# ru-wang/slam-plus-plus

Measured on AMD Instinct MI355X. Metric: Λ-solve block-nnz/sec + batch GN iters/sec, Venice BA, 1→8 MI355X, higher is better.
Workload: dtype f64; 1 GPU; venice871-shaped synthetic BA (871 cams, 530304 points, 2838740 observations, LM-damped); nnzb=3369915, n=1596138, mode=schur+dense, n_reduced=5226, schur_pairs=12875640, parallelism=single GPU

## Files before the change

### include/spp_hip.h

```cpp
#ifndef SPP_HIP_H
#define SPP_HIP_H

#include <stddef.h>
#include <stdint.h>

#ifdef __cplusplus
extern "C" {
#endif

#define SPP_OK            0
#define SPP_NOT_POSDEF    1
#define SPP_E_BADARG     -1
#define SPP_E_NOMEM      -2
#define SPP_E_HIP        -3
#define SPP_E_NO_DEVICE  -4
#define SPP_E_STATE      -5
#define SPP_E_UNSUPPORTED -6

#define SPP_MODE_AUTO     0
#define SPP_MODE_SPARSE   1
#define SPP_MODE_SCHUR    2
#define SPP_MODE_SCHUR_SPARSE 3

#define SPP_FLAG_PROFILE  1
#define SPP_FLAG_SCHUR_PARTIAL 2

typedef struct spp_ctx spp_ctx;

spp_ctx *spp_create(int device, int flags);
void spp_destroy(spp_ctx *ctx);
int spp_free_memory(spp_ctx *ctx);
int spp_last_error(const spp_ctx *ctx, char *buf, size_t buf_size);
double *spp_host_staging(spp_ctx *ctx, int64_t n_doubles);
int spp_set_stream(spp_ctx *ctx, void *hip_stream);
int spp_synchronize(spp_ctx *ctx);

int spp_analyze(spp_ctx *ctx, int64_t nb, const int64_t *h_col_ptr, const int64_t *h_row_idx,
	const int64_t *h_blk_off, const int32_t *h_dim, int mode);

int spp_set_shard(spp_ctx *ctx, int rank, int world_size);

#define SPP_MODE_SCHUR_MIS 4

#define SPP_INFO_MODE           0
#define SPP_INFO_N              1
#define SPP_INFO_NNZB           2
#define SPP_INFO_NVALS          3
#define SPP_INFO_FACTOR_NNZ     4
#define SPP_INFO_FACTOR_FLOPS   5
#define SPP_INFO_N_REDUCED      6
#define SPP_INFO_N_POSES        7
#define SPP_INFO_N_LANDMARKS    8
#define SPP_INFO_SCHUR_PAIRS    9
#define SPP_INFO_N_OBS          10
#define SPP_INFO_SOLVE_BYTES    11
#define SPP_INFO_N_SUPERNODES   12
#define SPP_INFO_N_LEVELS       13
#define SPP_INFO_S_LD           14
#define SPP_INFO_S_NNZB         15
#define SPP_INFO_DENSE_STREAMED 16
int spp_get_info(const spp_ctx *ctx, int what, int64_t *out);
int spp_get_ordering(const spp_ctx *ctx, int64_t *h_order);

#define SPP_ORDER_AMD 0
#define SPP_ORDER_ND  1
int spp_block_ordering(int64_t nb, const int64_t *col_ptr, const int64_t *row_idx, int method, int64_t *h_order);

int spp_schur_plan_host(int64_t nb, const int32_t *dim, const int64_t *col_ptr, const int64_t *row_idx, int shard_rank,
	int shard_world, int sparse_S, int64_t *out, double *seconds);

int spp_factor_solve(spp_ctx *ctx, const double *h_vals, double *h_rhs_inout);

int spp_factor_solve_device(spp_ctx *ctx, const double *d_vals, double *d_rhs_inout);

int spp_schur_buffer_size(const spp_ctx *ctx, int64_t *n_doubles);
int spp_schur_form(spp_ctx *ctx, const double *d_vals, const double *d_rhs, double *d_S_rhs);
int spp_schur_finish(spp_ctx *ctx, const double *d_vals, double *d_S_rhs, double *d_rhs_inout);
int spp_schur_packed_size(const spp_ctx *ctx, int64_t *n_doubles);
int spp_schur_pack(spp_ctx *ctx, const double *d_S_rhs, double *d_packed);
int spp_schur_unpack(spp_ctx *ctx, const double *d_packed, double *d_S_rhs);

int spp_assemble_analyze(spp_ctx *ctx, int64_t nv, const int32_t *h_dim,
	int64_t ne, const int64_t *h_v0, const int64_t *h_v1, int d0, int d1, int rd,
	int64_t unary_vertex);
int spp_assemble_get_structure(const spp_ctx *ctx, int64_t *h_col_ptr, int64_t *h_row_idx,
	int64_t *h_blk_off);
int spp_assemble_device(spp_ctx *ctx, const double *d_J0, const double *d_J1,
	const double *d_Omega, const double *d_r, double damping, double *d_vals_out, double *d_eta_out);
int spp_assemble_set_edge_weights(spp_ctx *ctx, const double *d_w);
int spp_edge_robust_weights_device(spp_ctx *ctx, int64_t n_edges, int rd, int kind, double scale, double param,
	const double *d_r, double *d_w_out);

int spp_se2_linearize_device(spp_ctx *ctx, int64_t n_edges, const int32_t *d_v0, const int32_t *d_v1,
	const double *d_poses, const double *d_measurements, double *d_J0, double *d_J1, double *d_r);
int spp_se2_update_device(spp_ctx *ctx, int64_t n_vertices, double *d_poses, const double *d_dx, int apply,
	double *h_dx_norm2);

int spp_se3_linearize_device(spp_ctx *ctx, int64_t n_edges, const int32_t *d_v0, const int32_t *d_v1,
	const double *d_poses, const double *d_measurements, double *d_J0, double *d_J1, double *d_r);
int spp_se3_update_device(spp_ctx *ctx, int64_t n_vertices, double *d_poses, const double *d_dx, int apply,
	double *h_dx_norm2);

int spp_ba_linearize_device(spp_ctx *ctx, int64_t n_obs, const int32_t *d_cam_of, const int32_t *d_pt_of,
	const double *d_cams, const double *d_intrinsics, const double *d_points, const double *d_measurements,
	double *d_J0, double *d_J1, double *d_r);
int spp_ba_update_device(spp_ctx *ctx, int64_t n_cams, double *d_cams, const int64_t *d_cam_dxoff,
	int64_t n_points, double *d_points, const int64_t *d_pt_dxoff, const double *d_dx, int64_t n_dx, int apply,
	double *h_dx_norm2);

int spp_edge_chi2_device(spp_ctx *ctx, int64_t n_edges, int rd, const double *d_r, const double *d_Omega, double *h_chi2);
int spp_edge_hessian_maxdiag_device(spp_ctx *ctx, int64_t n_edges, int rd, int d0, int d1, const double *d_J0,
	const double *d_J1, const double *d_Omega, double *h_max);
int spp_lm_gain_denominator_device(spp_ctx *ctx, int64_t n, const double *d_dx, const double *d_eta, double alpha,
	double *h_out);

int spp_device_malloc(spp_ctx *ctx, size_t bytes, void **d_ptr);
int spp_device_free(spp_ctx *ctx, void *d_ptr);
int spp_memcpy_h2d(spp_ctx *ctx, void *d_dst, const void *h_src, size_t bytes);
int spp_memcpy_d2h(spp_ctx *ctx, void *h_dst, const void *d_src, size_t bytes);
int spp_memcpy_d2d(spp_ctx *ctx, void *d_dst, const void *d_src, size_t bytes);

int spp_set_profiling(spp_ctx *ctx, int on);

#define SPP_PHASE_PERMUTE   0
#define SPP_PHASE_SCHUR_INV 1
#define SPP_PHASE_SCHUR_GEMM 2
#define SPP_PHASE_SCHUR_RHS 3
#define SPP_PHASE_FACTOR    4
#define SPP_PHASE_TRISOLVE  5
#define SPP_PHASE_BACKSUBST 6
#define SPP_PHASE_ASSEMBLE  7
#define SPP_PHASE_TOTAL     8
#define SPP_N_PHASES        9
int spp_get_phase_ms(spp_ctx *ctx, double *ms_out );
int spp_get_dominant_kernel(spp_ctx *ctx, double *ms_total, int64_t *n_launches, double *flops);

int spp_microbench_copy(spp_ctx *ctx, size_t bytes, int iters, double *gb_per_s);
int spp_microbench_mfma_f64(spp_ctx *ctx, int iters, double *tflops);
int spp_microbench_ctile(spp_ctx *ctx, int n, int iters, double *gb_per_s);
int spp_microbench_update(spp_ctx *ctx, int64_t m, int iters, double *ms_per_launch);

int spp_dense_potrf_upper(spp_ctx *ctx, double *d_A, int64_t n, int64_t ld);
int spp_dense_posv(spp_ctx *ctx, double *d_A, int64_t n, int64_t ld, double *d_b);
int spp_dense_gemm_tn_sub(spp_ctx *ctx, int64_t m, int64_t n, int64_t k,
	const double *d_A, int64_t lda, const double *d_B, int64_t ldb, double *d_C, int64_t ldc);
int spp_dense_gemm_tn_sub_upper(spp_ctx *ctx, int64_t m, int64_t n, int64_t k,
	const double *d_A, int64_t lda, const double *d_B, int64_t ldb, double *d_C, int64_t ldc);
int spp_dense_front_factor(spp_ctx *ctx, double *d_F, int64_t ld, int64_t w, int64_t h, double *d_image);

const char *spp_version(void);

#ifdef __cplusplus
}
#endif
#endif
```

### slam_plus_plus_amd/api.py

```python
import ctypes
import os

import numpy as np

_HERE = os.path.dirname(os.path.abspath(__file__))
LIB_PATH = os.environ.get("SPP_LIB") or os.path.join(_HERE, "libspp_hip.so")

SPP_OK, SPP_NOT_POSDEF = 0, 1
MODE_AUTO, MODE_SPARSE, MODE_SCHUR, MODE_SCHUR_SPARSE, MODE_SCHUR_MIS = 0, 1, 2, 3, 4
FLAG_PROFILE = 1
INFO = dict(MODE=0, N=1, NNZB=2, NVALS=3, FACTOR_NNZ=4, FACTOR_FLOPS=5, N_REDUCED=6, N_POSES=7,
            N_LANDMARKS=8, SCHUR_PAIRS=9, N_OBS=10, SOLVE_BYTES=11, N_SUPERNODES=12, N_LEVELS=13, S_LD=14, S_NNZB=15, DENSE_STREAMED=16)
PHASES = ["permute", "schur_inv", "schur_gemm", "schur_rhs", "factor", "trisolve", "backsubst", "assemble", "total"]

EXPORTS = [
    "spp_create", "spp_destroy", "spp_free_memory", "spp_last_error", "spp_host_staging", "spp_set_stream", "spp_synchronize",
    "spp_analyze", "spp_set_shard", "spp_get_info", "spp_get_ordering", "spp_factor_solve",
    "spp_factor_solve_device", "spp_schur_buffer_size", "spp_schur_form", "spp_schur_finish",
    "spp_schur_packed_size", "spp_schur_pack", "spp_schur_unpack",
    "spp_assemble_analyze", "spp_assemble_get_structure", "spp_assemble_device", "spp_assemble_set_edge_weights", "spp_device_malloc",
    "spp_device_free", "spp_memcpy_h2d", "spp_memcpy_d2h", "spp_memcpy_d2d", "spp_get_phase_ms", "spp_get_dominant_kernel",
    "spp_microbench_copy", "spp_microbench_mfma_f64", "spp_microbench_ctile", "spp_microbench_update", "spp_block_ordering", "spp_schur_plan_host", "spp_set_profiling", "spp_se2_linearize_device", "spp_se2_update_device", "spp_ba_linearize_device", "spp_ba_update_device", "spp_se3_linearize_device", "spp_se3_update_device", "spp_edge_chi2_device", "spp_edge_robust_weights_device", "spp_edge_hessian_maxdiag_device",
    "spp_lm_gain_denominator_device", "spp_dense_potrf_upper", "spp_dense_posv",
    "spp_dense_gemm_tn_sub", "spp_dense_gemm_tn_sub_upper", "spp_dense_front_factor", "spp_version",
]

_lib = None
_c_i64p = ctypes.POINTER(ctypes.c_int64)
_c_i32p = ctypes.POINTER(ctypes.c_int32)
_c_f64p = ctypes.POINTER(ctypes.c_double)


class SppError(RuntimeError):
    """std::runtime_error of the C++ adapter (reference LinearSolver_Schur_GPU.cpp:734-797)."""


def load_library():
    global _lib
    if _lib is not None:
        return _lib
    if not os.path.exists(LIB_PATH):
        raise SppError("libspp_hip.so is not built: run `python -m slam_plus_plus_amd.build` "
                       "(hipcc --offload-arch=gfx950); there is no CPU fallback")
    lib = ctypes.CDLL(LIB_PATH)
    vp, i64, i32, dbl, cint = ctypes.c_void_p, ctypes.c_int64, ctypes.c_int32, ctypes.c_double, ctypes.c_int
    sig = {
        "spp_create": (vp, [cint, cint]),
        "spp_destroy": (None, [vp]),
        "spp_free_memory": (cint, [vp]),
        "spp_last_error": (cint, [vp, ctypes.c_char_p, ctypes.c_size_t]),
        "spp_host_staging": (vp, [vp, i64]),
        "spp_set_stream": (cint, [vp, vp]),
        "spp_synchronize": (cint, [vp]),
        "spp_analyze": (cint, [vp, i64, vp, vp, vp, vp, cint]),
        "spp_set_shard": (cint, [vp, cint, cint]),
        "spp_get_info": (cint, [vp, cint, _c_i64p]),
        "spp_get_ordering": (cint, [vp, vp]),
        "spp_factor_solve": (cint, [vp, vp, vp]),
        "spp_factor_solve_device": (cint, [vp, vp, vp]),
        "spp_schur_buffer_size": (cint, [vp, _c_i64p]),
        "spp_schur_form": (cint, [vp, vp, vp, vp]),
        "spp_schur_finish": (cint, [vp, vp, vp, vp]),
        "spp_schur_packed_size": (cint, [vp, _c_i64p]),
        "spp_schur_pack": (cint, [vp, vp, vp]),
        "spp_schur_unpack": (cint, [vp, vp, vp]),
        "spp_assemble_analyze": (cint, [vp, i64, vp, i64, vp, vp, cint, cint, cint, i64]),
        "spp_assemble_get_structure": (cint, [vp, vp, vp, vp]),
        "spp_assemble_device": (cint, [vp, vp, vp, vp, vp, dbl, vp, vp]),
        "spp_assemble_set_edge_weights": (cint, [vp, vp]),
        "spp_device_malloc": (cint, [vp, ctypes.c_size_t, ctypes.POINTER(vp)]),
        "spp_device_free": (cint, [vp, vp]),
        "spp_memcpy_h2d": (cint, [vp, vp, vp, ctypes.c_size_t]),
        "spp_memcpy_d2h": (cint, [vp, vp, vp, ctypes.c_size_t]),
        "spp_memcpy_d2d": (cint, [vp, vp, vp, ctypes.c_size_t]),
        "spp_get_phase_ms": (cint, [vp, _c_f64p]),
        "spp_get_dominant_kernel": (cint, [vp, _c_f64p, _c_i64p, _c_f64p]),
        "spp_microbench_copy": (cint, [vp, ctypes.c_size_t, cint, _c_f64p]),
        "spp_microbench_mfma_f64": (cint, [vp, cint, _c_f64p]),
        "spp_microbench_ctile": (cint, [vp, cint, cint, _c_f64p]),
        "spp_microbench_update": (cint, [vp, ctypes.c_int64, cint, _c_f64p]),
        "spp_block_ordering": (cint, [ctypes.c_int64, vp, vp, cint, vp]),
        "spp_schur_plan_host": (cint, [ctypes.c_int64, vp, vp, vp, cint, cint, cint, vp, vp]),
        "spp_set_profiling": (cint, [vp, cint]),
        "spp_se2_linearize_device": (cint, [vp, ctypes.c_int64, vp, vp, vp, vp, vp, vp, vp]),
        "spp_se2_update_device": (cint, [vp, ctypes.c_int64, vp, vp, cint, _c_f64p]),
        "spp_se3_linearize_device": (cint, [vp, ctypes.c_int64, vp, vp, vp, vp, vp, vp, vp]),
        "spp_se3_update_device": (cint, [vp, ctypes.c_int64, vp, vp, cint, _c_f64p]),
        "spp_edge_chi2_device": (cint, [vp, ctypes.c_int64, cint, vp, vp, _c_f64p]),
        "spp_edge_robust_weights_device": (cint, [vp, ctypes.c_int64, cint, cint, dbl, dbl, vp, vp]),
        "spp_edge_hessian_maxdiag_device": (cint, [vp, ctypes.c_int64, cint, cint, cint, vp, vp, vp, _c_f64p]),
        "spp_lm_gain_denominator_device": (cint, [vp, ctypes.c_int64, vp, vp, ctypes.c_double, _c_f64p]),
        "spp_ba_linearize_device": (cint, [vp, ctypes.c_int64, vp, vp, vp, vp, vp, vp, vp, vp, vp]),
        "spp_ba_update_device": (cint, [vp, ctypes.c_int64, vp, vp, ctypes.c_int64, vp, vp, vp, ctypes.c_int64, cint, _c_f64p]),
        "spp_dense_potrf_upper": (cint, [vp, vp, i64, i64]),
        "spp_dense_posv": (cint, [vp, vp, i64, i64, vp]),
        "spp_dense_gemm_tn_sub": (cint, [vp, i64, i64, i64, vp, i64, vp, i64, vp, i64]),
        "spp_dense_gemm_tn_sub_upper": (cint, [vp, i64, i64, i64, vp, i64, vp, i64, vp, i64]),
        "spp_dense_front_factor": (cint, [vp, vp, i64, i64, i64, vp]),
        "spp_version": (ctypes.c_char_p, []),
    }
    for name, (res, args) in sig.items():
        fn = getattr(lib, name)
        fn.restype = res
        fn.argtypes = args
    _lib = lib
    return lib


def _ptr(a):
    return a.ctypes.data_as(ctypes.c_void_p)


ORDER_AMD, ORDER_ND = 0, 1


def block_ordering(lam, method=ORDER_AMD):
    lib = load_library()
    col_ptr = np.ascontiguousarray(lam.col_ptr, dtype=np.int64)
    row_idx = np.ascontiguousarray(lam.row_idx, dtype=np.int64)
    out = np.empty(lam.nb, dtype=np.int64)
    code = lib.spp_block_ordering(lam.nb, _ptr(col_ptr), _ptr(row_idx), method, _ptr(out))
    if code != 0:
        raise SppError("spp_block_ordering failed: %d" % code)
    return out


def schur_plan_host(lam, shard_rank=0, shard_world=1, sparse_S=False, mis=False):
    lib = load_library()
    col_ptr = np.ascontiguousarray(lam.col_ptr, dtype=np.int64)
    row_idx = np.ascontiguousarray(lam.row_idx, dtype=np.int64)
    dim = np.ascontiguousarray(lam.dim, dtype=np.int32)
    out = np.zeros(8, dtype=np.int64)
    sec = ctypes.c_double(0.0)
    code = lib.spp_schur_plan_host(lam.nb, _ptr(dim), _ptr(col_ptr), _ptr(row_idx), shard_rank, shard_world,
                                   (1 if sparse_S else 0) | (2 if mis else 0), _ptr(out), ctypes.byref(sec))
    if code != 0:
        raise SppError("spp_schur_plan_host failed: %d" % code)
    keys = ("nc", "nl", "no", "n_pairs", "n_sblk", "n_items", "n_multi", "checksum")
    d = dict(zip(keys, (int(v) for v in out)))
    d["seconds"] = sec.value
    return d


class DeviceArray:

    def __init__(self, ctx, n, dtype=np.float64):
        self.ctx, self.n, self.dtype = ctx, int(n), np.dtype(dtype)
        p = ctypes.c_void_p()
        ctx._check(ctx.lib.spp_device_malloc(ctx.h, self.n * self.dtype.itemsize, ctypes.byref(p)))
        self.ptr = p.value

    @classmethod
    def from_host(cls, ctx, arr):
        arr = np.ascontiguousarray(arr)
        d = cls(ctx, arr.size, arr.dtype)
        d.upload(arr)
        return d

    def upload(self, arr):
        arr = np.ascontiguousarray(arr, dtype=self.dtype)
        assert arr.size == self.n
        self.ctx._check(self.ctx.lib.spp_memcpy_h2d(self.ctx.h, self.ptr, _ptr(arr), arr.nbytes))

    def download(self):
        out = np.empty(self.n, dtype=self.dtype)
        self.ctx._check(self.ctx.lib.spp_memcpy_d2h(self.ctx.h, _ptr(out), self.ptr, out.nbytes))
        return out

    def copy_from(self, other):
        assert other.n * other.dtype.itemsize <= self.n * self.dtype.itemsize
        self.ctx._check(self.ctx.lib.spp_memcpy_d2d(self.ctx.h, self.ptr, other.ptr, other.n * other.dtype.itemsize))

    def free(self):
        if self.ptr:
            self.ctx.lib.spp_device_free(self.ctx.h, self.ptr)
            self.ptr = None


class Context:

    def __init__(self, device=0, flags=0):
        self.lib = load_library()
        self.h = self.lib.spp_create(int(device), int(flags))
        if not self.h:
            raise SppError("spp_create failed: no usable HIP device %d (the solver has no CPU fallback)" % device)

    def close(self):
        if getattr(self, "h", None):
            self.lib.spp_destroy(self.h)
            self.h = None

    def __del__(self):
        try:
            self.close()
        except Exception:
            pass

    def last_error(self):
        buf = ctypes.create_string_buffer(1024)
        self.lib.spp_last_error(self.h, buf, 1024)
        return buf.value.decode(errors="replace")

    def _check(self, code):
        if code < 0:
            if code == -2:
                raise MemoryError(self.last_error())
            raise SppError("spp error %d: %s" % (code, self.last_error()))
        return code

    def analyze(self, bcsc, mode=MODE_AUTO):
        self._keep = bcsc
        return self._check(self.lib.spp_analyze(self.h, bcsc.nb, _ptr(bcsc.col_ptr), _ptr(bcsc.row_idx),
                                                 _ptr(bcsc.blk_off), _ptr(bcsc.dim), mode))

    def set_shard(self, rank, world):
        return self._check(self.lib.spp_set_shard(self.h, rank, world))

    def info(self, key):
        out = ctypes.c_int64()
        self._check(self.lib.spp_get_info(self.h, INFO[key], ctypes.byref(out)))
        return out.value

    def ordering(self, nb):
        out = np.empty(nb, dtype=np.int64)
        self._check(self.lib.spp_get_ordering(self.h, _ptr(out)))
        return out

    def se2_linearize_device(self, n_edges, d_v0, d_v1, d_poses, d_meas, d_J0, d_J1, d_r):
        return self._check(self.lib.spp_se2_linearize_device(self.h, n_edges, d_v0, d_v1, d_poses, d_meas, d_J0, d_J1, d_r))

    def se2_update_device(self, n_vertices, d_poses, d_dx, apply=True):
        out = ctypes.c_double()
        self._check(self.lib.spp_se2_update_device(self.h, n_vertices, d_poses, d_dx, 1 if apply else 0, ctypes.byref(out)))
        return out.value ** 0.5

    def se3_linearize_device(self, n_edges, d_v0, d_v1, d_poses, d_meas, d_J0, d_J1, d_r):
        return self._check(self.lib.spp_se3_linearize_device(self.h, n_edges, d_v0, d_v1, d_poses, d_meas, d_J0, d_J1, d_r))

    def se3_update_device(self, n_vertices, d_poses, d_dx, apply=True):
        out = ctypes.c_double()
        self._check(self.lib.spp_se3_update_device(self.h, n_vertices, d_poses, d_dx, 1 if apply else 0, ctypes.byref(out)))
        return out.value ** 0.5

    def edge_robust_weights_device(self, n_edges, rd, d_r, d_w, scale, param=1.345, kind=0):
        return self._check(self.lib.spp_edge_robust_weights_device(self.h, n_edges, rd, kind, float(scale), float(param), d_r, d_w))

    def edge_chi2_device(self, n_edges, rd, d_r, d_Om):
        out = ctypes.c_double()
        self._check(self.lib.spp_edge_chi2_device(self.h, n_edges, rd, d_r, d_Om, ctypes.byref(out)))
        return out.value

    def edge_hessian_maxdiag_device(self, n_edges, rd, d0, d1, d_J0, d_J1, d_Om):
        out = ctypes.c_double()
        self._check(self.lib.spp_edge_hessian_maxdiag_device(self.h, n_edges, rd, d0, d1, d_J0, d_J1, d_Om, ctypes.byref(out)))
        return out.value

    def lm_gain_denominator_device(self, n, d_dx, d_eta, alpha):
        out = ctypes.c_double()
        self._check(self.lib.spp_lm_gain_denominator_device(self.h, n, d_dx, d_eta, float(alpha), ctypes.byref(out)))
        return out.value

    def ba_linearize_device(self, n_obs, d_cam_of, d_pt_of, d_cams, d_intr, d_points, d_meas, d_J0, d_J1, d_r):
        return self._check(self.lib.spp_ba_linearize_device(self.h, n_obs, d_cam_of, d_pt_of, d_cams, d_intr, d_points,
                                                            d_meas, d_J0, d_J1, d_r))

    def ba_update_device(self, n_cams, d_cams, d_cam_dxoff, n_points, d_points, d_pt_dxoff, d_dx, n_dx, apply=True):
        out = ctypes.c_double()
        self._check(self.lib.spp_ba_update_device(self.h, n_cams, d_cams, d_cam_dxoff, n_points, d_points, d_pt_dxoff,
                                                  d_dx, n_dx, 1 if apply else 0, ctypes.byref(out)))
        return out.value ** 0.5

    def set_profiling(self, on):
        return self._check(self.lib.spp_set_profiling(self.h, 1 if on else 0))

    def set_stream(self, stream_handle):
        return self._check(self.lib.spp_set_stream(self.h, ctypes.c_void_p(stream_handle)))

    def synchronize(self):
        return self._check(self.lib.spp_synchronize(self.h))

    def host_staging(self, n):
        p = self.lib.spp_host_staging(self.h, int(n))
        if not p:
            raise MemoryError(self.last_error())
        return np.ctypeslib.as_array(ctypes.cast(p, ctypes.POINTER(ctypes.c_double)), shape=(int(n),))

    def factor_solve(self, vals, rhs):
        vals = np.ascontiguousarray(vals, dtype=np.float64)
        x = np.array(rhs, dtype=np.float64, copy=True)
        code = self._check(self.lib.spp_factor_solve(self.h, _ptr(vals), _ptr(x)))
        return code, x

    def factor_solve_device(self, d_vals, d_rhs):
        return self._check(self.lib.spp_factor_solve_device(self.h, d_vals, d_rhs))

    def schur_buffer_size(self):
# ... 127 lines not shown
```

### slam_plus_plus_amd/csrc/spp_api.cpp

```cpp

#include "spp_internal.h"
#include <string.h>
#include <new>

using namespace spp;

namespace spp {

void phases_reset(spp_ctx *ctx)
{
	if(!(ctx->flags & SPP_FLAG_PROFILE))
		return;
	if(!ctx->timer.created) {
		for(int i = 0; i < 2 * SPP_N_PHASES; ++ i)
			SPP_HIP_CHECK(hipEventCreate(&ctx->timer.ev[i]));
		ctx->timer.created = true;
	}
	for(int i = 0; i < SPP_N_PHASES; ++ i) {
		ctx->timer.used[i] = false;
		ctx->phase_ms[i] = 0;
	}
	ctx->dom_used = 0;
	ctx->dom_flops = 0;
}

void phase_begin(spp_ctx *ctx, int phase)
{
	if(!(ctx->flags & SPP_FLAG_PROFILE) || !ctx->timer.created)
		return;
	SPP_HIP_CHECK(hipEventRecord(ctx->timer.ev[2 * phase], ctx->stream));
}

void phase_end(spp_ctx *ctx, int phase)
{
	if(!(ctx->flags & SPP_FLAG_PROFILE) || !ctx->timer.created)
		return;
	SPP_HIP_CHECK(hipEventRecord(ctx->timer.ev[2 * phase + 1], ctx->stream));
	ctx->timer.used[phase] = true;
}

void phases_collect(spp_ctx *ctx)
{
	if(!(ctx->flags & SPP_FLAG_PROFILE) || !ctx->timer.created)
		return;
	SPP_HIP_CHECK(hipStreamSynchronize(ctx->stream));
	for(int i = 0; i < SPP_N_PHASES; ++ i) {
		if(!ctx->timer.used[i])
			continue;
		float ms = 0;
		if(hipEventElapsedTime(&ms, ctx->timer.ev[2 * i], ctx->timer.ev[2 * i + 1]) == hipSuccess)
			ctx->phase_ms[i] = ms;
	}
}

void dom_begin(spp_ctx *ctx)
{
	if(!(ctx->flags & SPP_FLAG_PROFILE))
		return;
	if(ctx->dom_used + 2 > ctx->dom_events.size()) {
		size_t old = ctx->dom_events.size();
		ctx->dom_events.resize(old + 64);
		for(size_t i = old; i < ctx->dom_events.size(); ++ i)
			SPP_HIP_CHECK(hipEventCreate(&ctx->dom_events[i]));
	}
	SPP_HIP_CHECK(hipEventRecord(ctx->dom_events[ctx->dom_used], ctx->stream));
}

void dom_end(spp_ctx *ctx, double flops)
{
	if(!(ctx->flags & SPP_FLAG_PROFILE))
		return;
	SPP_HIP_CHECK(hipEventRecord(ctx->dom_events[ctx->dom_used + 1], ctx->stream));
	ctx->dom_used += 2;
	ctx->dom_flops += flops;
}

}

#define SPP_TRY(ctx) try {
#define SPP_CATCH(ctx) } catch(const spp::Error &e) { if(ctx) (ctx)->last_error = e.what(); return e.code; } \
	catch(const std::bad_alloc &) { if(ctx) (ctx)->last_error = "host allocation failed"; return SPP_E_NOMEM; } \
	catch(const std::exception &e) { if(ctx) (ctx)->last_error = e.what(); return SPP_E_HIP; }

extern "C" {

const char *spp_version(void)
{
	return "slam_plus_plus_amd 0.1 (gfx950, fp64)";
}

spp_ctx *spp_create(int device, int flags)
{
	int count = 0;
	if(hipGetDeviceCount(&count) != hipSuccess || count <= 0 || device < 0 || device >= count)
		return nullptr;
	if(hipSetDevice(device) != hipSuccess)
		return nullptr;
	spp_ctx *ctx = new(std::nothrow) spp_ctx;
	if(!ctx)
		return nullptr;
	ctx->device = device;
	ctx->flags = flags;
	if(hipStreamCreateWithFlags(&ctx->stream, hipStreamNonBlocking) != hipSuccess) {
		delete ctx;
		return nullptr;
	}
	ctx->own_stream = true;
	return ctx;
}

int spp_free_memory(spp_ctx *ctx)
{
	if(!ctx)
		return SPP_E_BADARG;
	SPP_TRY(ctx)
	(void)hipSetDevice(ctx->device);
	(void)hipStreamSynchronize(ctx->stream);
	ctx->schur.release_all();
	sparse_release(ctx);
	assemble_release(ctx);
	ctx->dense.tinv.release();
	ctx->dense.tinv_all.release();
	ctx->dense.xtmp.release();
	ctx->dense.la_cnt.release();
	ctx->dense.la_trace.release();
	ctx->geom_partial.release();
	ctx->dense.flags.release();
	ctx->dense.trsv_pay.release();
	ctx->dense.trsv_m.release();
	ctx->dense.tail_pub.release();
	ctx->dense.tail_order.release();
	ctx->dense.tail_order_tr = ctx->dense.tail_order_tc = 0;
	ctx->dense.tail_dinv.release();
	ctx->dense.tail_epoch = 0;
	ctx->dense.epoch = 0;
	ctx->dense.sync.release();
	ctx->dense.fuse_cnt.release();
	ctx->dense.fuse_expect.clear();
	ctx->dense.sync_epoch = 0;
	ctx->d_vals.release();
	ctx->d_rhs.release();
	ctx->mode = -1;
	return SPP_OK;
	SPP_CATCH(ctx)
}

void spp_destroy(spp_ctx *ctx)
{
	if(!ctx)
		return;
	if(ctx->plan_trash.joinable())
		ctx->plan_trash.join();
	spp_free_memory(ctx);
	ctx->dense.info.release();
	if(ctx->dense.aux) {
		dense_aux_park(ctx->device, ctx->dense.aux);
		(void)hipEventDestroy(ctx->dense.ev[0]);
		(void)hipEventDestroy(ctx->dense.ev[1]);
	}
	if(ctx->dense.chain) {
		(void)hipStreamDestroy(ctx->dense.chain);
		if(ctx->dense.ev_chain)
			(void)hipEventDestroy(ctx->dense.ev_chain);
	}
	if(ctx->dense.h_chain_err)
		(void)hipHostFree(ctx->dense.h_chain_err);
	if(ctx->h_staging)
		(void)hipHostFree(ctx->h_staging);
	if(ctx->timer.created)
		for(int i = 0; i < 2 * SPP_N_PHASES; ++ i)
			(void)hipEventDestroy(ctx->timer.ev[i]);
	for(size_t i = 0; i < ctx->dom_events.size(); ++ i)
		(void)hipEventDestroy(ctx->dom_events[i]);
	if(ctx->own_stream && ctx->stream)
		(void)hipStreamDestroy(ctx->stream);
	delete ctx;
}

int spp_last_error(const spp_ctx *ctx, char *buf, size_t buf_size)
{
	if(!ctx || !buf || !buf_size)
		return SPP_E_BADARG;
	strncpy(buf, ctx->last_error.c_str(), buf_size - 1);
	buf[buf_size - 1] = 0;
	return SPP_OK;
}

double *spp_host_staging(spp_ctx *ctx, int64_t n_doubles)
{
	if(!ctx || n_doubles < 0)
		return nullptr;
	if((size_t)n_doubles <= ctx->h_staging_cap && ctx->h_staging)
		return ctx->h_staging;
	(void)hipSetDevice(ctx->device);
	(void)hipStreamSynchronize(ctx->stream);
	if(ctx->h_staging) {
		(void)hipHostFree(ctx->h_staging);
		ctx->h_staging = nullptr;
		ctx->h_staging_cap = 0;
	}
	const size_t want = (size_t)(n_doubles > 0 ? n_doubles : 1);
	if(hipHostMalloc((void**)&ctx->h_staging, want * sizeof(double), hipHostMallocDefault) != hipSuccess) {
		(void)hipGetLastError();
		ctx->h_staging = nullptr;
		ctx->last_error = "hipHostMalloc of the staging buffer failed";
		return nullptr;
	}
	ctx->h_staging_cap = want;
	return ctx->h_staging;
}

int spp_set_stream(spp_ctx *ctx, void *hip_stream)
{
	if(!ctx)
		return SPP_E_BADARG;
	(void)hipStreamSynchronize(ctx->stream);
	if(ctx->own_stream && ctx->stream)
		(void)hipStreamDestroy(ctx->stream);
	ctx->stream = (hipStream_t)hip_stream;
	ctx->own_stream = false;
	return SPP_OK;
}

int spp_synchronize(spp_ctx *ctx)
{
	if(!ctx)
		return SPP_E_BADARG;
	SPP_TRY(ctx)
	SPP_HIP_CHECK(hipStreamSynchronize(ctx->stream));
	dense_chain_check(ctx);
	return SPP_OK;
	SPP_CATCH(ctx)
}

int spp_set_profiling(spp_ctx *ctx, int on)
{
	if(!ctx)
		return SPP_E_BADARG;
	ctx->flags = on ? (ctx->flags | SPP_FLAG_PROFILE) : (ctx->flags & ~SPP_FLAG_PROFILE);
	return SPP_OK;
}

int spp_set_shard(spp_ctx *ctx, int rank, int world_size)
{
	if(!ctx || world_size < 1 || rank < 0 || rank >= world_size)
		return SPP_E_BADARG;
	ctx->shard_rank = rank;
	ctx->shard_world = world_size;
	return SPP_OK;
}

int spp_analyze(spp_ctx *ctx, int64_t nb, const int64_t *col_ptr, const int64_t *row_idx,
	const int64_t *blk_off, const int32_t *dim, int mode)
{
	if(!ctx)
		return SPP_E_BADARG;
	SPP_TRY(ctx)
	SPP_REQUIRE(nb > 0 && col_ptr && row_idx && blk_off && dim, SPP_E_BADARG, "spp_analyze: null or empty structure");
	SPP_REQUIRE(col_ptr[0] == 0 && col_ptr[nb] >= nb, SPP_E_BADARG, "spp_analyze: column pointers must start at 0 and hold every diagonal block");
	SPP_HIP_CHECK(hipSetDevice(ctx->device));
	ctx->mode = -1;
	VClock clk("spp_analyze");
	Structure st;
	st.nb = nb;
	st.nnzb = col_ptr[nb];
	st.col_ptr.assign(col_ptr, col_ptr + nb + 1);
	SPP_REQUIRE(st.nnzb >= nb, SPP_E_BADARG, "spp_analyze: fewer blocks than block columns");
	for(int64_t j = 0; j < nb; ++ j)
		SPP_REQUIRE(col_ptr[j + 1] > col_ptr[j], SPP_E_BADARG, "every block column needs its diagonal block");
	st.dim.assign(dim, dim + nb);
	st.base.resize(nb + 1);
	st.base[0] = 0;
	for(int64_t j = 0; j < nb; ++ j) {
		SPP_REQUIRE(dim[j] > 0 && dim[j] <= 8, SPP_E_BADARG, "block widths must be in 1..8");
		st.base[j + 1] = st.base[j] + dim[j];
	}
	st.n = st.base[nb];
	st.row_idx.resize(st.nnzb);
	st.blk_off.resize(st.nnzb);
	{
		const int nt = plan_threads(st.nnzb);
		std::vector<int64_t> jcut, nvals_t(nt, 0);
		balanced_cuts(st.col_ptr, nt, jcut);
		run_threads(nt, [&](int t) {
			const int64_t p0 = col_ptr[jcut[t]], p1 = col_ptr[jcut[t + 1]];
			if(p1 > p0) {
				memcpy(st.row_idx.data() + p0, row_idx + p0, (size_t)(p1 - p0) * sizeof(int64_t));
				memcpy(st.blk_off.data() + p0, blk_off + p0, (size_t)(p1 - p0) * sizeof(int64_t));
			}
			int64_t nv = 0;
			for(int64_t j = jcut[t]; j < jcut[t + 1]; ++ j) {
				for(int64_t p = col_ptr[j]; p < col_ptr[j + 1]; ++ p) {
					const int64_t i = row_idx[p];
					SPP_REQUIRE(i >= 0 && i <= j, SPP_E_BADARG, "only the upper triangle may be stored");
					SPP_REQUIRE(p == col_ptr[j] || row_idx[p - 1] < i, SPP_E_BADARG, "rows must ascend within a column");
					SPP_REQUIRE(blk_off[p] >= 0, SPP_E_BADARG, "negative block offset");
					nv = std::max<int64_t>(nv, blk_off[p] + (int64_t)dim[i] * dim[j]);
				}
				SPP_REQUIRE(row_idx[col_ptr[j + 1] - 1] == j, SPP_E_BADARG, "diagonal block missing (must be last in its column)");
			}
			nvals_t[t] = nv;
		});
		st.nvals = 0;
		for(int t = 0; t < nt; ++ t)
			st.nvals = std::max(st.nvals, nvals_t[t]);
	}
	ctx->st = std::move(st);
	Structure &st_ref = ctx->st;
	clk.lap("structure copied + validated");
	ctx->schur.release_all();
	sparse_release(ctx);
	clk.lap("old plans released");
	int dp, dl;
	int chosen = mode;
	if(mode == SPP_MODE_AUTO) {
		chosen = SPP_MODE_SPARSE;
		if(schur_applicable(st_ref, &dp, &dl)) {
			int64_t n_red = 0;
			for(int64_t j = 0; j < nb; ++ j)
				n_red += (dim[j] == dp) ? dp : 0;
			chosen = (n_red <= 16384) ? SPP_MODE_SCHUR : SPP_MODE_SCHUR_SPARSE;
		}
	}
	SPP_REQUIRE(chosen == SPP_MODE_SCHUR || chosen == SPP_MODE_SPARSE || chosen == SPP_MODE_SCHUR_SPARSE ||
		chosen == SPP_MODE_SCHUR_MIS, SPP_E_BADARG, "unknown mode");
	SPP_REQUIRE((chosen != SPP_MODE_SPARSE && chosen != SPP_MODE_SCHUR_MIS) || ctx->shard_world == 1, SPP_E_UNSUPPORTED,
		"only the Schur modes shard (over landmarks); pose graphs run as replicas (DESIGN.md, multi-GPU)");
	ctx->mode = -1;
	if(chosen == SPP_MODE_SCHUR || chosen == SPP_MODE_SCHUR_SPARSE || chosen == SPP_MODE_SCHUR_MIS) {
		const bool mis = chosen == SPP_MODE_SCHUR_MIS;
		const bool sparse_S = chosen != SPP_MODE_SCHUR;
		build_schur_plan(ctx, sparse_S, mis);
		clk.lap("schur plan (all of it)");
		ctx->schur.mis = mis;
		ctx->order.clear();
		ctx->order.reserve((size_t)st_ref.nb);
		if(sparse_S) {
			sparse_analyze(ctx, ctx->schur.s_st);
			std::vector<int64_t> red = ctx->order;
			ctx->order.clear();
			for(size_t i = 0; i < red.size(); ++ i)
				ctx->order.push_back(ctx->schur.pose_block[red[i]]);
			chosen = SPP_MODE_SCHUR;
		} else
		for(size_t i = 0; i < ctx->schur.pose_block.size(); ++ i)
			ctx->order.push_back(ctx->schur.pose_block[i]);
		for(int64_t j = 0; j < st_ref.nb; ++ j)
			if(ctx->schur.is_lm[j])
				ctx->order.push_back(j);
	} else
		sparse_analyze(ctx, ctx->st);
	ctx->mode = chosen;
	clk.lap("plan + ordering");
	return SPP_OK;
	SPP_CATCH(ctx)
}

int spp_get_info(const spp_ctx *ctx, int what, int64_t *out)
{
	if(!ctx || !out)
		return SPP_E_BADARG;
	if(ctx->mode < 0 && what != SPP_INFO_NNZB && what != SPP_INFO_NVALS && what != SPP_INFO_N && what != SPP_INFO_DENSE_STREAMED)
		return SPP_E_STATE;
	switch(what) {
	case SPP_INFO_MODE: *out = (ctx->mode != SPP_MODE_SCHUR) ? ctx->mode : ctx->schur.mis ? SPP_MODE_SCHUR_MIS :
		ctx->schur.sparse_S ? SPP_MODE_SCHUR_SPARSE : SPP_MODE_SCHUR; break;
	case SPP_INFO_N: *out = ctx->st.n; break;
	case SPP_INFO_NNZB: *out = ctx->st.nnzb; break;
	case SPP_INFO_NVALS: *out = ctx->st.nvals; break;
	case SPP_INFO_FACTOR_NNZ: *out = ctx->factor_nnz; break;
	case SPP_INFO_FACTOR_FLOPS: *out = ctx->factor_flops; break;
	case SPP_INFO_N_REDUCED: *out = (ctx->mode == SPP_MODE_SCHUR) ? ctx->schur.n_red : 0; break;
	case SPP_INFO_N_POSES: *out = (ctx->mode == SPP_MODE_SCHUR) ? ctx->schur.nc : ctx->st.nb; break;
	case SPP_INFO_N_LANDMARKS: *out = (ctx->mode == SPP_MODE_SCHUR) ? ctx->schur.nl : 0; break;
	case SPP_INFO_SCHUR_PAIRS: *out = (ctx->mode == SPP_MODE_SCHUR) ? ctx->schur.n_pairs : 0; break;
	case SPP_INFO_N_OBS: *out = (ctx->mode == SPP_MODE_SCHUR) ? ctx->schur.no : 0; break;
	case SPP_INFO_SOLVE_BYTES: *out = ctx->solve_bytes; break;
	case SPP_INFO_N_SUPERNODES: *out = ctx->sparse ? sparse_info(ctx, what) : 0; break;
	case SPP_INFO_N_LEVELS: *out = ctx->sparse ? sparse_info(ctx, what) : 0; break;
	case SPP_INFO_S_LD: *out = (ctx->mode == SPP_MODE_SCHUR && !ctx->schur.sparse_S) ? ctx->schur.ld : 0; break;
	case SPP_INFO_S_NNZB: *out = (ctx->mode == SPP_MODE_SCHUR) ? ctx->schur.n_sblk : 0; break;
	case SPP_INFO_DENSE_STREAMED: *out = ctx->dense.tail_rows_last; break;
	default: return SPP_E_BADARG;
	}
	return SPP_OK;
}

int spp_get_ordering(const spp_ctx *ctx, int64_t *h_order)
{
	if(!ctx || !h_order)
		return SPP_E_BADARG;
	if(ctx->mode < 0)
		return SPP_E_STATE;
	for(size_t i = 0; i < ctx->order.size(); ++ i)
		h_order[i] = ctx->order[i];
	return SPP_OK;
}

int spp_block_ordering(int64_t nb, const int64_t *col_ptr, const int64_t *row_idx, int method, int64_t *h_order)
{
	if(nb <= 0 || !col_ptr || !row_idx || !h_order || (method != SPP_ORDER_AMD && method != SPP_ORDER_ND))
		return SPP_E_BADARG;
	try {
		for(int64_t j = 0; j < nb; ++ j)
			for(int64_t p = col_ptr[j]; p < col_ptr[j + 1]; ++ p)
				if(row_idx[p] < 0 || row_idx[p] > j)
					return SPP_E_BADARG;
		std::vector<int64_t> order;
		if(method == SPP_ORDER_AMD)
			min_degree_order(nb, col_ptr, row_idx, order);
		else
			nested_dissection_order(nb, col_ptr, row_idx, order);
		for(int64_t k = 0; k < nb; ++ k)
			h_order[k] = order[k];
		return SPP_OK;
	} catch(const std::bad_alloc &) {
		return SPP_E_NOMEM;
	} catch(...) {
		return SPP_E_HIP;
	}
}

int spp_schur_plan_host(int64_t nb, const int32_t *dim, const int64_t *col_ptr, const int64_t *row_idx, int shard_rank,
	int shard_world, int sparse_S, int64_t *out, double *seconds)
{
	if(nb <= 0 || !dim || !col_ptr || !row_idx || !out || shard_world < 1 || shard_rank < 0 || shard_rank >= shard_world)
		return SPP_E_BADARG;
	try {
		Structure st;
		st.nb = nb;
		st.nnzb = col_ptr[nb];
		st.col_ptr.assign(col_ptr, col_ptr + nb + 1);
		st.row_idx.assign(row_idx, row_idx + st.nnzb);
		st.dim.assign(dim, dim + nb);
		st.base.resize(nb + 1);
		st.base[0] = 0;
		for(int64_t j = 0; j < nb; ++ j)
			st.base[j + 1] = st.base[j] + dim[j];
		st.n = st.base[nb];
		st.blk_off.resize(st.nnzb);
		int64_t off = 0;
		for(int64_t j = 0; j < nb; ++ j)
			for(int64_t p = col_ptr[j]; p < col_ptr[j + 1]; ++ p) {
				if(row_idx[p] < 0 || row_idx[p] > j)
					return SPP_E_BADARG;
				st.blk_off[p] = off;
				off += (int64_t)dim[row_idx[p]] * dim[j];
			}
		st.nvals = off;
		const double sec = schur_plan_host_probe(st, shard_rank, shard_world, (sparse_S & 1) != 0, (sparse_S & 2) != 0, out);
		if(seconds)
			*seconds = sec;
		return SPP_OK;
	} catch(const Error &e) {
		return e.code;
	} catch(const std::bad_alloc &) {
		return SPP_E_NOMEM;
	} catch(...) {
		return SPP_E_HIP;
	}
}

int spp_schur_buffer_size(const spp_ctx *ctx, int64_t *n_doubles)
{
	if(!ctx || !n_doubles)
		return SPP_E_BADARG;
	if(ctx->mode != SPP_MODE_SCHUR)
		return SPP_E_STATE;
	*n_doubles = schur_buffer_doubles(ctx);
	return SPP_OK;
}

int spp_schur_form(spp_ctx *ctx, const double *d_vals, const double *d_rhs, double *d_S_rhs)
{
	if(!ctx || !d_vals || !d_rhs || !d_S_rhs)
		return SPP_E_BADARG;
	SPP_TRY(ctx)
	SPP_REQUIRE(ctx->mode == SPP_MODE_SCHUR, SPP_E_STATE, "spp_schur_form: analyze in Schur mode first");
	SPP_HIP_CHECK(hipSetDevice(ctx->device));
	phases_reset(ctx);
	phase_begin(ctx, SPP_PHASE_TOTAL);
	schur_form(ctx, d_vals, d_rhs, d_S_rhs);
	return SPP_OK;
	SPP_CATCH(ctx)
}

int spp_schur_packed_size(const spp_ctx *ctx, int64_t *n_doubles)
{
	if(!ctx || !n_doubles)
		return SPP_E_BADARG;
	if(ctx->mode != SPP_MODE_SCHUR)
		return SPP_E_STATE;
	if(ctx->schur.sparse_S) {
		*n_doubles = schur_buffer_doubles(ctx);
		return SPP_OK;
	}
	const int64_t nblk = ctx->schur.ld / DENSE_NB;
	*n_doubles = (int64_t)DENSE_NB * DENSE_NB * (nblk * (nblk + 1) / 2);
	return SPP_OK;
}

int spp_schur_pack(spp_ctx *ctx, const double *d_S_rhs, double *d_packed)
{
	if(!ctx || !d_S_rhs || !d_packed)
		return SPP_E_BADARG;
	SPP_TRY(ctx)
	SPP_REQUIRE(ctx->mode == SPP_MODE_SCHUR, SPP_E_STATE, "spp_schur_pack: analyze in Schur mode first");
	SPP_HIP_CHECK(hipSetDevice(ctx->device));
	if(ctx->schur.sparse_S)
		SPP_HIP_CHECK(hipMemcpyAsync(d_packed, d_S_rhs, (size_t)schur_buffer_doubles(ctx) * sizeof(double),
			hipMemcpyDeviceToDevice, ctx->stream));
	else
		schur_pack(ctx, const_cast<double*>(d_S_rhs), d_packed, true);
	return SPP_OK;
	SPP_CATCH(ctx)
}

int spp_schur_unpack(spp_ctx *ctx, const double *d_packed, double *d_S_rhs)
{
	if(!ctx || !d_S_rhs || !d_packed)
		return SPP_E_BADARG;
	SPP_TRY(ctx)
	SPP_REQUIRE(ctx->mode == SPP_MODE_SCHUR, SPP_E_STATE, "spp_schur_unpack: analyze in Schur mode first");
	SPP_HIP_CHECK(hipSetDevice(ctx->device));
	if(ctx->schur.sparse_S)
		SPP_HIP_CHECK(hipMemcpyAsync(d_S_rhs, d_packed, (size_t)schur_buffer_doubles(ctx) * sizeof(double),
			hipMemcpyDeviceToDevice, ctx->stream));
	else
		schur_pack(ctx, d_S_rhs, const_cast<double*>(d_packed), false);
	return SPP_OK;
	SPP_CATCH(ctx)
}

int spp_schur_finish(spp_ctx *ctx, const double *d_vals, double *d_S_rhs, double *d_rhs_inout)
{
	if(!ctx || !d_vals || !d_rhs_inout || !d_S_rhs)
		return SPP_E_BADARG;
	SPP_TRY(ctx)
	SPP_REQUIRE(ctx->mode == SPP_MODE_SCHUR, SPP_E_STATE, "spp_schur_finish: analyze in Schur mode first");
	SPP_HIP_CHECK(hipSetDevice(ctx->device));
	int ret = schur_finish(ctx, d_vals, d_S_rhs, d_rhs_inout);
	phase_end(ctx, SPP_PHASE_TOTAL);
	phases_collect(ctx);
	dense_chain_check(ctx);
	return ret;
	SPP_CATCH(ctx)
}

int spp_factor_solve_device(spp_ctx *ctx, const double *d_vals, double *d_rhs)
{
	if(!ctx || !d_vals || !d_rhs)
		return SPP_E_BADARG;
	SPP_TRY(ctx)
	SPP_REQUIRE(ctx->mode >= 0, SPP_E_STATE, "spp_factor_solve: call spp_analyze first");
	SPP_HIP_CHECK(hipSetDevice(ctx->device));
	phases_reset(ctx);
	phase_begin(ctx, SPP_PHASE_TOTAL);
	int ret;
	if(ctx->mode == SPP_MODE_SCHUR) {
		SPP_REQUIRE(ctx->shard_world == 1, SPP_E_STATE,
			"sharded ctx: use spp_schur_form / all-reduce / spp_schur_finish");
		ctx->schur.S.reserve((size_t)schur_buffer_doubles(ctx));
		schur_form(ctx, d_vals, d_rhs, ctx->schur.S.p);
		ret = schur_finish(ctx, d_vals, ctx->schur.S.p, d_rhs);
	} else
		ret = sparse_factor_solve(ctx, d_vals, d_rhs);
	phase_end(ctx, SPP_PHASE_TOTAL);
	phases_collect(ctx);
	SPP_HIP_CHECK(hipStreamSynchronize(ctx->stream));
	dense_chain_check(ctx);
	return ret;
	SPP_CATCH(ctx)
}

int spp_factor_solve(spp_ctx *ctx, const double *h_vals, double *h_rhs)
{
	if(!ctx || !h_vals || !h_rhs)
		return SPP_E_BADARG;
	SPP_TRY(ctx)
	SPP_REQUIRE(ctx->mode >= 0, SPP_E_STATE, "spp_factor_solve: call spp_analyze first");
	SPP_HIP_CHECK(hipSetDevice(ctx->device));
	ctx->d_vals.reserve((size_t)ctx->st.nvals);
	ctx->d_rhs.reserve((size_t)ctx->st.n);
	SPP_HIP_CHECK(hipMemcpyAsync(ctx->d_vals.p, h_vals, ctx->st.nvals * sizeof(double), hipMemcpyHostToDevice, ctx->stream));
	SPP_HIP_CHECK(hipMemcpyAsync(ctx->d_rhs.p, h_rhs, ctx->st.n * sizeof(double), hipMemcpyHostToDevice, ctx->stream));
	int ret = spp_factor_solve_device(ctx, ctx->d_vals.p, ctx->d_rhs.p);
	if(ret != SPP_OK)
		return ret;
	SPP_HIP_CHECK(hipMemcpyAsync(h_rhs, ctx->d_rhs.p, ctx->st.n * sizeof(double), hipMemcpyDeviceToHost, ctx->stream));
	SPP_HIP_CHECK(hipStreamSynchronize(ctx->stream));
	return SPP_OK;
	SPP_CATCH(ctx)
}

int spp_assemble_analyze(spp_ctx *ctx, int64_t nv, const int32_t *h_dim, int64_t ne, const int64_t *h_v0,
	const int64_t *h_v1, int d0, int d1, int rd, int64_t unary_vertex)
{
	if(!ctx || !h_dim || !h_v0 || !h_v1 || nv <= 0 || ne <= 0)
		return SPP_E_BADARG;
	SPP_TRY(ctx)
	SPP_HIP_CHECK(hipSetDevice(ctx->device));
	assemble_analyze(ctx, nv, h_dim, ne, h_v0, h_v1, d0, d1, rd, unary_vertex);
	return SPP_OK;
	SPP_CATCH(ctx)
}

// ... 163 lines not shown
}

int spp_device_malloc(spp_ctx *ctx, size_t bytes, void **d_ptr)
{
	if(!ctx || !d_ptr)
		return SPP_E_BADARG;
	(void)hipSetDevice(ctx->device);
	if(hipMalloc(d_ptr, bytes ? bytes : 8) != hipSuccess) {
		ctx->last_error = "hipMalloc failed";
		return SPP_E_NOMEM;
	}
	return SPP_OK;
}

int spp_device_free(spp_ctx *ctx, void *d_ptr)
{
	if(!ctx)
		return SPP_E_BADARG;
	(void)hipSetDevice(ctx->device);
	(void)hipStreamSynchronize(ctx->stream);
	return hipFree(d_ptr) == hipSuccess ? SPP_OK : SPP_E_HIP;
}

int spp_memcpy_h2d(spp_ctx *ctx, void *d_dst, const void *h_src, size_t bytes)
{
	if(!ctx)
		return SPP_E_BADARG;
	SPP_TRY(ctx)
	SPP_HIP_CHECK(hipSetDevice(ctx->device));
	SPP_HIP_CHECK(hipMemcpyAsync(d_dst, h_src, bytes, hipMemcpyHostToDevice, ctx->stream));
	SPP_HIP_CHECK(hipStreamSynchronize(ctx->stream));
	return SPP_OK;
	SPP_CATCH(ctx)
}

int spp_memcpy_d2h(spp_ctx *ctx, void *h_dst, const void *d_src, size_t bytes)
{
	if(!ctx)
		return SPP_E_BADARG;
	SPP_TRY(ctx)
	SPP_HIP_CHECK(hipSetDevice(ctx->device));
	SPP_HIP_CHECK(hipMemcpyAsync(h_dst, d_src, bytes, hipMemcpyDeviceToHost, ctx->stream));
	SPP_HIP_CHECK(hipStreamSynchronize(ctx->stream));
	return SPP_OK;
	SPP_CATCH(ctx)
}

int spp_memcpy_d2d(spp_ctx *ctx, void *d_dst, const void *d_src, size_t bytes)
{
	if(!ctx)
		return SPP_E_BADARG;
	SPP_TRY(ctx)
	SPP_HIP_CHECK(hipSetDevice(ctx->device));
	SPP_HIP_CHECK(hipMemcpyAsync(d_dst, d_src, bytes, hipMemcpyDeviceToDevice, ctx->stream));
	return SPP_OK;
	SPP_CATCH(ctx)
}

int spp_get_phase_ms(spp_ctx *ctx, double *ms_out)
{
	if(!ctx || !ms_out)
		return SPP_E_BADARG;
	for(int i = 0; i < SPP_N_PHASES; ++ i)
		ms_out[i] = ctx->phase_ms[i];
	return SPP_OK;
}

int spp_get_dominant_kernel(spp_ctx *ctx, double *ms_total, int64_t *n_launches, double *flops)
{
	if(!ctx || !ms_total || !n_launches || !flops)
		return SPP_E_BADARG;
	SPP_TRY(ctx)
	SPP_HIP_CHECK(hipStreamSynchronize(ctx->stream));
	double total = 0;
	for(size_t i = 0; i + 1 < ctx->dom_used; i += 2) {
		float ms = 0;
		SPP_HIP_CHECK(hipEventElapsedTime(&ms, ctx->dom_events[i], ctx->dom_events[i + 1]));
		total += ms;
	}
	*ms_total = total;
	*n_launches = (int64_t)(ctx->dom_used / 2);
	*flops = ctx->dom_flops;
	return SPP_OK;
	SPP_CATCH(ctx)
}

int spp_microbench_copy(spp_ctx *ctx, size_t bytes, int iters, double *gb_per_s)
{
	if(!ctx || !gb_per_s)
		return SPP_E_BADARG;
	SPP_TRY(ctx)
	SPP_HIP_CHECK(hipSetDevice(ctx->device));
	*gb_per_s = microbench_copy(ctx, bytes, iters);
	return SPP_OK;
	SPP_CATCH(ctx)
}

int spp_microbench_ctile(spp_ctx *ctx, int n, int iters, double *gb_per_s)
{
	if(!ctx || !gb_per_s)
		return SPP_E_BADARG;
	SPP_TRY(ctx)
	SPP_HIP_CHECK(hipSetDevice(ctx->device));
	*gb_per_s = microbench_ctile(ctx, n, iters);
	return SPP_OK;
	SPP_CATCH(ctx)
}

int spp_microbench_update(spp_ctx *ctx, int64_t m, int iters, double *ms_per_launch)
{
	if(!ctx || !ms_per_launch || m < 128 || iters < 1)
		return SPP_E_BADARG;
	SPP_TRY(ctx)
	SPP_HIP_CHECK(hipSetDevice(ctx->device));
	*ms_per_launch = microbench_update(ctx, m, iters);
	return SPP_OK;
	SPP_CATCH(ctx)
}

int spp_microbench_mfma_f64(spp_ctx *ctx, int iters, double *tflops)
{
	if(!ctx || !tflops)
		return SPP_E_BADARG;
	SPP_TRY(ctx)
	SPP_HIP_CHECK(hipSetDevice(ctx->device));
	*tflops = microbench_mfma_f64(ctx, iters);
	return SPP_OK;
	SPP_CATCH(ctx)
}

int spp_dense_potrf_upper(spp_ctx *ctx, double *d_A, int64_t n, int64_t ld)
{
	if(!ctx || !d_A || n <= 0 || ld < n)
		return SPP_E_BADARG;
	SPP_TRY(ctx)
	SPP_HIP_CHECK(hipSetDevice(ctx->device));
	const int64_t ldp = ((n + 1 + DENSE_NB - 1) / DENSE_NB) * DENSE_NB;
	DevBuf<double> tmp;
	tmp.reserve((size_t)ldp * ldp);
	SPP_HIP_CHECK(hipMemsetAsync(tmp.p, 0, (size_t)ldp * ldp * sizeof(double), ctx->stream));
	SPP_HIP_CHECK(hipMemcpy2DAsync(tmp.p, ldp * sizeof(double), d_A, ld * sizeof(double), n * sizeof(double), n,
		hipMemcpyDeviceToDevice, ctx->stream));
	dense_set_padding(ctx, tmp.p, ldp, n);
	int ret = dense_potrf_upper(ctx, tmp.p, n, ldp, true);
	SPP_HIP_CHECK(hipMemcpy2DAsync(d_A, ld * sizeof(double), tmp.p, ldp * sizeof(double), n * sizeof(double), n,
		hipMemcpyDeviceToDevice, ctx->stream));
	SPP_HIP_CHECK(hipStreamSynchronize(ctx->stream));
	return ret;
	SPP_CATCH(ctx)
}

int spp_dense_posv(spp_ctx *ctx, double *d_A, int64_t n, int64_t ld, double *d_b)
{
	if(!ctx || !d_A || !d_b || n <= 0 || ld < n)
		return SPP_E_BADARG;
	SPP_TRY(ctx)
	SPP_HIP_CHECK(hipSetDevice(ctx->device));
	const int64_t ldp = ((n + 1 + DENSE_NB - 1) / DENSE_NB) * DENSE_NB;
	DevBuf<double> tmp;
	tmp.reserve((size_t)ldp * ldp);
	SPP_HIP_CHECK(hipMemsetAsync(tmp.p, 0, (size_t)ldp * ldp * sizeof(double), ctx->stream));
	SPP_HIP_CHECK(hipMemcpy2DAsync(tmp.p, ldp * sizeof(double), d_A, ld * sizeof(double), n * sizeof(double), n,
		hipMemcpyDeviceToDevice, ctx->stream));
	dense_set_padding(ctx, tmp.p, ldp, n);
	SPP_HIP_CHECK(hipMemcpyAsync(tmp.p + n * ldp, d_b, n * sizeof(double), hipMemcpyDeviceToDevice, ctx->stream));
	int ret = dense_potrf_upper(ctx, tmp.p, n, ldp, true);
	if(ret == SPP_OK) {
		dense_potrs_upper(ctx, tmp.p, n, ldp, tmp.p + n * ldp);
		SPP_HIP_CHECK(hipMemcpyAsync(d_b, tmp.p + n * ldp, n * sizeof(double), hipMemcpyDeviceToDevice, ctx->stream));
		SPP_HIP_CHECK(hipMemcpy2DAsync(d_A, ld * sizeof(double), tmp.p, ldp * sizeof(double), n * sizeof(double), n,
			hipMemcpyDeviceToDevice, ctx->stream));
	}
	SPP_HIP_CHECK(hipStreamSynchronize(ctx->stream));
	dense_chain_check(ctx);
	return ret;
	SPP_CATCH(ctx)
}

int spp_dense_gemm_tn_sub(spp_ctx *ctx, int64_t m, int64_t n, int64_t k, const double *d_A, int64_t lda,
	const double *d_B, int64_t ldb, double *d_C, int64_t ldc)
{
	if(!ctx || !d_A || !d_B || !d_C)
		return SPP_E_BADARG;
	SPP_TRY(ctx)
	SPP_REQUIRE((lda % 2) == 0 && (ldb % 2) == 0, SPP_E_BADARG, "gemm_tn_sub: lda/ldb must be even (16-byte loads)");
	SPP_HIP_CHECK(hipSetDevice(ctx->device));
	dense_gemm_tn_sub(ctx, m, n, k, d_A, lda, d_B, ldb, d_C, ldc, false);
	SPP_HIP_CHECK(hipStreamSynchronize(ctx->stream));
	return SPP_OK;
	SPP_CATCH(ctx)
}

int spp_dense_gemm_tn_sub_upper(spp_ctx *ctx, int64_t m, int64_t n, int64_t k, const double *d_A, int64_t lda,
	const double *d_B, int64_t ldb, double *d_C, int64_t ldc)
{
	if(!ctx || !d_A || !d_B || !d_C)
		return SPP_E_BADARG;
	SPP_TRY(ctx)
	SPP_REQUIRE((lda % 2) == 0 && (ldb % 2) == 0, SPP_E_BADARG, "gemm_tn_sub: lda/ldb must be even (16-byte loads)");
	SPP_HIP_CHECK(hipSetDevice(ctx->device));
	dense_gemm_tn_sub(ctx, m, n, k, d_A, lda, d_B, ldb, d_C, ldc, true);
	SPP_HIP_CHECK(hipStreamSynchronize(ctx->stream));
	return SPP_OK;
	SPP_CATCH(ctx)
}

int spp_dense_front_factor(spp_ctx *ctx, double *d_F, int64_t ld, int64_t w, int64_t h, double *d_image)
{
	if(!ctx || !d_F)
		return SPP_E_BADARG;
	SPP_TRY(ctx)
	SPP_HIP_CHECK(hipSetDevice(ctx->device));
	return dense_front_factor(ctx, d_F, ld, w, h, d_image);
	SPP_CATCH(ctx)
}

}
```

### slam_plus_plus_amd/csrc/spp_dense.hip

```cpp

#include "spp_internal.h"
#include "spp_tiles.h"
#include "spp_dense_dev.h"
#include <stdio.h>
#include <stdlib.h>
#include <string.h>
#include <algorithm>
#include <vector>
#include <mutex>

namespace spp {


constexpr int BK = 16;
constexpr int LDS_STRIDE = 18;

template <int BM, int BN, int WM, int WN, int MODE, int DEPTH, int BKT, int SC1 = 0>
__device__ __forceinline__ void gemm_tn_tile(const int64_t m0, const int64_t n0, int64_t M, int64_t N, int K,
	const double *__restrict__ A, int64_t lda, const double *B, int64_t ldb, double *C, int64_t ldc, double *gemm_lds)
{
	constexpr int NWM = BM / WM, NWN = BN / WN, NT = NWM * NWN * 64;
	constexpr int TA = WM / 16, TB = WN / 16;
	constexpr int PPC = BKT / 2, LSTR = BKT + 2;
	constexpr int PA = (BM * PPC) / NT, PB = (BN * PPC) / NT;
// ... 1148 lines not shown
		dw.la_trace.reserve(nw);
		std::vector<long long> init(nw, 0);
		for(int64_t k = 0; k < nsteps; ++ k)
			init[8 * nsteps + 8 + 4 * k] = (long long)((~0ull) >> 1);
		SPP_HIP_CHECK(hipMemcpyAsync(dw.la_trace.p, init.data(), nw * sizeof(long long), hipMemcpyHostToDevice, s));
		SPP_HIP_CHECK(hipStreamSynchronize(s));
		a.trace = dw.la_trace.p;
	}
	SPP_HIP_CHECK(hipMemsetAsync(a.cnt, 0, nints * sizeof(int), s));
	SPP_HIP_CHECK(hipEventRecord(dw.ev[0], s));
	SPP_HIP_CHECK(hipStreamWaitEvent(sc, dw.ev[0], 0));
	SPP_HIP_CHECK(hipStreamWaitEvent(sb, dw.ev[0], 0));
	hipLaunchKernelGGL(la_chain_kernel, dim3((unsigned)(1 + LA_G1 + a.g2)), dim3(LA_THREADS), LA_LDS_DOUBLES * sizeof(double), sc, a);
	const int64_t slots = slots_env > 0 ? slots_env : 512;
	for(int k = 0; k < a.nsteps; ++ k) {
		const int64_t c1 = (int64_t)NB * (k + 1);
		if(c1 >= ncols || rows - c1 <= 0)
			break;
		const int nr = (int)((rows - c1 + NB - 1) / NB), nc = (int)((ncols - c1 + NB - 1) / NB);
		const int npri = (nc > 2) ? (nc - 2) + std::min(2, nr - 1) : 0;
		const int64_t ntr = nr - 1, ntc = nc - 1;
		const int64_t T = ntr > 0 ? ntr * (ntr + 1) / 2 + (ntc - ntr) * ntr : 0;
		const int64_t n128 = (T / slots) * slots;
		const int64_t grid = 4 * (int64_t)npri + n128 + 4 * (T - n128);
		if(grid > 0)
			hipLaunchKernelGGL(la_bulk_kernel, dim3((unsigned)grid), dim3(1024), LA_BULK_LDS_DOUBLES * sizeof(double), sb,
				a, k, nr, nc, npri, n128);
	}
	SPP_HIP_CHECK(hipEventRecord(dw.ev[1], sb));
	SPP_HIP_CHECK(hipEventRecord(dw.ev_chain, sc));
	SPP_HIP_CHECK(hipStreamWaitEvent(s, dw.ev[1], 0));
	SPP_HIP_CHECK(hipStreamWaitEvent(s, dw.ev_chain, 0));
	SPP_HIP_CHECK(hipGetLastError());
	if(tracing) {
		std::vector<long long> h((size_t)12 * nsteps + 16);
		SPP_HIP_CHECK(hipMemcpyAsync(h.data(), dw.la_trace.p, h.size() * sizeof(long long), hipMemcpyDeviceToHost, s));
		SPP_HIP_CHECK(hipStreamSynchronize(s));
		fprintf(stderr, "[spp] lookahead factorization, %d steps: potrf start / duration / gap to the next start (us)\n", a.nsteps);
		for(int k = 0; k < a.nsteps; ++ k)
			fprintf(stderr, "  k %2d  start %8.1f  potrf %5.1f  publish %4.1f | b1 seen +%4.1f  done +%4.1f | c1 seen +%4.1f  done +%4.1f | step %5.1f\n", k,
				(h[8 * k] - h[0]) * 0.01, (h[8 * k + 2] - h[8 * k]) * 0.01, (h[8 * k + 1] - h[8 * k + 2]) * 0.01,
				(h[8 * k + 3] - h[8 * k + 1]) * 0.01, (h[8 * k + 4] - h[8 * k + 1]) * 0.01, (h[8 * k + 5] - h[8 * k + 1]) * 0.01,
				(h[8 * k + 6] - h[8 * k + 1]) * 0.01, k + 1 < a.nsteps ? (h[8 * (k + 1)] - h[8 * k]) * 0.01 : 0.0);
		fprintf(stderr, "[spp] per step: panel (rest) done / bulk launch: first tile starts, priority tiles done, last tile done, busy workgroup-us (all relative to potrf(0) start)\n");
		for(int k = 0; k < a.nsteps; ++ k) {
			const long long *b = h.data() + 8 * nsteps + 8 + 4 * k;
			fprintf(stderr, "  k %2d  panel done %8.1f | bulk start %8.1f  pri done %8.1f  end %8.1f  busy %9.1f\n", k, h[8 * k + 7] ? (h[8 * k + 7] - h[0]) * 0.01 : 0.0,
				b[1] ? (b[0] - h[0]) * 0.01 : 0.0, b[3] ? (b[3] - h[0]) * 0.01 : 0.0, b[1] ? (b[1] - h[0]) * 0.01 : 0.0, b[2] * 0.01);
		}
	}
}

void dense_factor_steps(spp_ctx *ctx, double *d_A, int64_t ld, int64_t n, int64_t rows, int64_t ncols,
	int64_t nsteps, bool has_rhs)
{
	ensure_dense_work(ctx, nsteps);
	ctx->dense.tail_rows_last = 0;
	hipStreamCaptureStatus cs = hipStreamCaptureStatusNone;
	const bool capturing = hipStreamIsCapturing(ctx->stream, &cs) != hipSuccess || cs != hipStreamCaptureStatusNone;
	if(!capturing && la_usable(ctx, nsteps)) {
		dense_factor_lookahead(ctx, d_A, ld, n, rows, ncols, nsteps, has_rhs);
		ctx->dense.tinv_half = 0;
		return;
	}
	ctx->dense.tinv_half = nsteps;
	const bool flags = !capturing && nsteps >= 4 && flag_schedule_usable(ctx);
	dense_factor_steps_enqueue(ctx, d_A, ld, n, rows, ncols, nsteps, has_rhs, flags, !capturing);
}

static void flag_signal(hipStream_t st, int *flag, int value)
{
	hipLaunchKernelGGL(flag_signal_kernel, dim3(1), dim3(64), 0, st, flag, value);
}

static FlagWait make_flag_wait(spp_ctx *ctx, const int *flag, int value, double timeout_ms = 500.0)
{
	return FlagWait{flag, value, ctx->dense.info.p + 2, (long long)(timeout_ms * 1e5)};
}

static void flag_wait(spp_ctx *ctx, hipStream_t st, const int *flag, int value, double timeout_ms)
{
	hipLaunchKernelGGL(flag_wait_kernel, dim3(1), dim3(64), 0, st, make_flag_wait(ctx, flag, value, timeout_ms));
}

static bool flag_schedule_selftest(spp_ctx *ctx)
{
	DenseWork &dw = ctx->dense;
	hipStream_t st[2] = {ctx->stream, dw.aux};
	dw.sync.reserve(16);
	SPP_HIP_CHECK(hipMemsetAsync(dw.sync.p, 0, 16 * sizeof(int), ctx->stream));
	SPP_HIP_CHECK(hipStreamSynchronize(ctx->stream));
	for(int p = 0; p < 2; ++ p) {
		flag_wait(ctx, st[p], dw.sync.p + p, 1, 20.0);
		flag_signal(st[1 - p], dw.sync.p + p, 1);
	}
	for(int i = 0; i < 2; ++ i)
		SPP_HIP_CHECK(hipStreamSynchronize(st[i]));
	int h_abort = 0;
	SPP_HIP_CHECK(hipMemcpy(&h_abort, dw.info.p + 2, sizeof(int), hipMemcpyDeviceToHost));
	if(h_abort) {
		SPP_HIP_CHECK(hipMemset(dw.info.p + 2, 0, sizeof(int)));
		return false;
	}
	return true;
}

static bool flag_schedule_usable(spp_ctx *ctx)
{
	static int sched = -1;
	if(sched < 0) {
		const char *e = getenv("SPP_DENSE_SCHED");
		sched = e ? atoi(e) : 1;
	}
	if(!sched)
		return false;
	DenseWork &dw = ctx->dense;
	if(dw.sync_state == 0 || dw.sync_stream != ctx->stream) {
		hipStreamCaptureStatus cs = hipStreamCaptureStatusNone;
		if(hipStreamIsCapturing(ctx->stream, &cs) != hipSuccess || cs != hipStreamCaptureStatusNone)
			return false;
		dw.sync_state = flag_schedule_selftest(ctx) ? 1 : -1;
		dw.sync_stream = ctx->stream;
	}
	return dw.sync_state == 1;
}

static int dense_tail_rows()
{
	static int v = -1;
	if(v < 0) {
		const char *e = getenv("SPP_TAIL_ROWS"), *on = getenv("SPP_DENSE_TAIL");
		v = (on && !atoi(on)) ? 0 : (e ? atoi(e) : 44);
	}
	return v;
}

static bool dense_tail_applies(spp_ctx *ctx, int64_t rows, int64_t nsteps)
{
	return !ctx->dense.tail_disabled && nsteps * NB >= rows && !(ctx->dense.ident_from >= 0 && ctx->dense.ident_from < rows);
}

static bool launch_dense_tail(spp_ctx *ctx, double *d_A, int64_t ld, int64_t rows, int64_t ncols, int64_t nsteps, int64_t k, bool has_rhs)
{
	static int enabled = -1;
	if(enabled < 0) {
		const char *e = getenv("SPP_DENSE_TAIL");
		enabled = e ? atoi(e) : 1;
	}
	DenseWork &dw = ctx->dense;
	const int64_t c1 = (k + 1) * NB;
	if(!enabled || dw.tail_disabled || k + 1 >= nsteps || nsteps * NB < rows || (dw.ident_from >= 0 && dw.ident_from < rows))
		return false;
	const int Tr = (int)(nsteps - (k + 1)), Tc = (int)((ncols - c1 + NB - 1) / NB);
	if(Tr < 1 || Tc < Tr || Tc > Tr + 1)
		return false;
	const int ntile = Tr * Tc - Tr * (Tr - 1) / 2;
	static int max_rows = -1;
	if(max_rows < 0) {
		const char *e = getenv("SPP_TAIL_ROWS");
		max_rows = e ? atoi(e) : 44;
	}
	if(Tr > max_rows)
		return false;
	hipStream_t s = ctx->stream;
	static uint64_t attr_seen = 0;
	if(first_on_this_device(attr_seen))
		SPP_HIP_CHECK(hipFuncSetAttribute((const void*)dense_tail_kernel, hipFuncAttributeMaxDynamicSharedMemorySize,
			TAIL_LDS_DOUBLES * (int)sizeof(double)));
	if(dw.tail_pub.cap < (size_t)Tr * Tc) {
		dw.tail_pub.reserve(std::max<size_t>((size_t)Tr * Tc, 24 * 25));
		SPP_HIP_CHECK(hipMemsetAsync(dw.tail_pub.p, 0, dw.tail_pub.cap * sizeof(int), s));
		dw.tail_epoch = 0;
	}
	if(dw.tail_dinv.cap < (size_t)Tr * 8 * 256)
		dw.tail_dinv.reserve(std::max<size_t>((size_t)Tr * 8 * 256, (size_t)24 * 8 * 256));
	if(++ dw.tail_epoch >= (1 << 26)) {
		SPP_HIP_CHECK(hipMemsetAsync(dw.tail_pub.p, 0, dw.tail_pub.cap * sizeof(int), s));
		dw.tail_epoch = 1;
	}
	if(dw.tail_order_tr != Tr || dw.tail_order_tc != Tc) {
		static double beta = -1;
		if(beta < 0) {
			const char *e = getenv("SPP_TAIL_ORDER_BETA");
			beta = e ? atof(e) : 0.0;
		}
		std::vector<std::pair<double, int> > key;
		for(int i = 0; i < Tr; ++ i)
			for(int j = i; j < Tc; ++ j)
				key.push_back(std::make_pair((double)i + beta * (double)j, (i << 16) | j));
		std::stable_sort(key.begin(), key.end(), [](const std::pair<double, int> &x, const std::pair<double, int> &y) { return x.first < y.first; });
		std::vector<int> &order = dw.tail_order_host;
		order.resize(key.size());
		for(size_t q = 0; q < key.size(); ++ q)
			order[q] = key[q].second;
		dw.tail_order.upload(order, s);
		dw.tail_order_tr = Tr;
		dw.tail_order_tc = Tc;
	}
	TailArgs a;
	a.order = dw.tail_order.p;
	a.A = d_A;
	a.ld = ld;
	a.rows = rows;
	a.ncols = ncols;
	a.c0 = c1;
	a.have_pre = (k >= 0) ? 1 : 0;
	a.Tr = Tr;
	a.Tc = Tc;
	a.has_rhs = has_rhs ? 1 : 0;
	a.tinv = dw.tinv_all.p + (size_t)(k + 1) * NB * NB;
	a.dbuf = dw.tail_dinv.p;
	a.pub = dw.tail_pub.p;
	a.epoch = dw.tail_epoch;
	a.info = dw.info.p;
	a.abort = dw.info.p + 2;
	static long long tail_timeout = -1;
	if(tail_timeout < 0) {
		const char *e = getenv("SPP_TAIL_TIMEOUT_TICKS");
		tail_timeout = e ? atoll(e) : (long long)(500.0 * 1e5);
	}
	a.timeout_ticks = tail_timeout;
	static int trace_env = -1;
	if(trace_env < 0) {
		const char *e = getenv("SPP_TAIL_TRACE");
		trace_env = e ? atoi(e) : 0;
	}
	static int launches = 0;
	DevBuf<long long> trace;
	a.trace = nullptr;
	if(trace_env && ++ launches == trace_env) {
		trace.reserve((size_t)Tr * 8);
		SPP_HIP_CHECK(hipMemsetAsync(trace.p, 0, (size_t)Tr * 8 * sizeof(long long), s));
		a.trace = trace.p;
	}
	dom_begin(ctx);
	hipLaunchKernelGGL(dense_tail_kernel, dim3((unsigned)ntile), dim3(POTRF_THREADS), TAIL_LDS_DOUBLES * sizeof(double), s, a);
	{
		const double m = (double)(rows - c1);
		dom_end(ctx, m * m * m / 3.0 + (a.have_pre ? (double)NB * m * (m + 1.0) : 0.0) + 2.0 * m * m);
	}
	dw.tail_rows_last = Tr;
	SPP_HIP_CHECK(hipGetLastError());
	if(a.trace) {
		std::vector<long long> h((size_t)Tr * 8);
		SPP_HIP_CHECK(hipStreamSynchronize(s));
		SPP_HIP_CHECK(hipMemcpy(h.data(), trace.p, h.size() * sizeof(long long), hipMemcpyDeviceToHost));
		fprintf(stderr, "[spp] streamed tail, %d tile rows (us from the launch's first stamp): diagonal tile: updates complete / factored+inverted | first panel tile: first row tile seen / last seen / last published\n", Tr);
		const long long t0 = h[0];
		for(int i = 0; i < Tr; ++ i)
			fprintf(stderr, "  row %2d  start %7.1f  updated %7.1f  done %7.1f | %7.1f %7.1f %7.1f\n", i, (h[8 * i] - t0) * 0.01, (h[8 * i + 1] - t0) * 0.01,
				(h[8 * i + 2] - t0) * 0.01, h[8 * i + 3] ? (h[8 * i + 3] - t0) * 0.01 : 0.0, h[8 * i + 4] ? (h[8 * i + 4] - t0) * 0.01 : 0.0, h[8 * i + 5] ? (h[8 * i + 5] - t0) * 0.01 : 0.0);
	}
	return true;
}

static void dense_factor_steps_enqueue(spp_ctx *ctx, double *d_A, int64_t ld, int64_t n, int64_t rows, int64_t ncols,
	int64_t nsteps, bool has_rhs, bool use_flags, bool allow_fused)
{
	hipStream_t s = ctx->stream, s2 = ctx->dense.aux;
	hipEvent_t evA = ctx->dense.ev[0], evB = ctx->dense.ev[1];
	DenseWork &dw = ctx->dense;
	const int64_t n_id = (dw.ident_from >= 0 && dw.ident_from < n) ? dw.ident_from : n;
	int ep = 0;
	int64_t step_a = -1, step_b = -1;
	int64_t need_wait_b = -1;
	if(use_flags) {
		if(dw.sync.cap < (size_t)(2 * nsteps + 16)) {
			dw.sync.reserve((size_t)(2 * nsteps + 16));
			SPP_HIP_CHECK(hipMemsetAsync(dw.sync.p, 0, dw.sync.cap * sizeof(int), s));
			dw.sync_epoch = 1;
		}
		ep = ++ dw.sync_epoch;
		SPP_HIP_CHECK(hipEventRecord(evA, s));
		SPP_HIP_CHECK(hipStreamWaitEvent(s2, evA, 0));
	}
	int64_t pend_sig = -1;
	auto record_a = [&](int64_t k) {
		step_a = k;
		if(use_flags)
			pend_sig = k;
		else
			SPP_HIP_CHECK(hipEventRecord(evA, s));
	};
	int64_t pend_sig_b = -1;
	auto wait_a_on_bulk = [&]() {
		if(use_flags && pend_sig_b >= 0) {
			hipLaunchKernelGGL(flag_signal_wait_kernel, dim3(1), dim3(64), 0, s2, dw.sync.p + 2 * pend_sig_b + 1, ep,
				make_flag_wait(ctx, dw.sync.p + 2 * step_a, ep));
			pend_sig_b = -1;
		} else if(use_flags)
			flag_wait(ctx, s2, dw.sync.p + 2 * step_a, ep);
		else
			SPP_HIP_CHECK(hipStreamWaitEvent(s2, evA, 0));
	};
	auto flush_sig_b = [&]() {
		if(pend_sig_b >= 0)
			flag_signal(s2, dw.sync.p + 2 * pend_sig_b + 1, ep);
		pend_sig_b = -1;
	};
	auto record_b = [&](int64_t k) {
		step_b = k;
		if(use_flags)
			pend_sig_b = k;
		else
			SPP_HIP_CHECK(hipEventRecord(evB, s2));
	};
	auto wait_b_now = [&]() {
		if(use_flags && pend_sig_b == step_b)
			flush_sig_b();
		if(use_flags && pend_sig >= 0) {
			flag_signal(s, dw.sync.p + 2 * pend_sig, ep);
			pend_sig = -1;
		}
		if(use_flags)
			flag_wait(ctx, s, dw.sync.p + 2 * step_b + 1, ep);
		else
			SPP_HIP_CHECK(hipStreamWaitEvent(s, evB, 0));
	};
	auto wait_b_deferred = [&]() {
		if(use_flags)
			need_wait_b = step_b;
		else
			SPP_HIP_CHECK(hipStreamWaitEvent(s, evB, 0));
	};
	auto flush_wait_b = [&]() {
		if(need_wait_b >= 0 && pend_sig_b == need_wait_b)
			flush_sig_b();
		if(need_wait_b >= 0 && pend_sig >= 0)
			hipLaunchKernelGGL(flag_signal_wait_kernel, dim3(1), dim3(64), 0, s, dw.sync.p + 2 * pend_sig, ep,
				make_flag_wait(ctx, dw.sync.p + 2 * need_wait_b + 1, ep));
		else if(need_wait_b >= 0)
			flag_wait(ctx, s, dw.sync.p + 2 * need_wait_b + 1, ep);
		else if(pend_sig >= 0)
			flag_signal(s, dw.sync.p + 2 * pend_sig, ep);
		need_wait_b = pend_sig = -1;
	};
	bool bulk_pending = false;
	static int fused_env = -1;
	if(fused_env < 0) {
		const char *e = getenv("SPP_FUSED");
		fused_env = e ? atoi(e) : 1;
	}
	const int fused = allow_fused ? fused_env : 0;
	if(fused) {
		static uint64_t fattr_seen = 0;
		if(first_on_this_device(fattr_seen)) {
			SPP_HIP_CHECK(hipFuncSetAttribute((const void*)update_potrf_kernel, hipFuncAttributeMaxDynamicSharedMemorySize,
				POTRF_LDS_DOUBLES * (int)sizeof(double)));
		}
		if(dw.fuse_cnt.cap < (size_t)(nsteps + 2) || dw.fuse_dirty) {
			dw.fuse_cnt.reserve(std::max<size_t>((size_t)(nsteps + 2), 64));
			SPP_HIP_CHECK(hipMemsetAsync(dw.fuse_cnt.p, 0, dw.fuse_cnt.cap * sizeof(int), s));
			dw.fuse_expect.assign(dw.fuse_cnt.cap, 0);
			dw.fuse_dirty = false;
		}
	}
	static_assert(POTRF_LDS_DOUBLES >= (64 + 64) * FS_STRIDE, "the fused kernel's LDS is sized by the factorization");
	auto fused_update_potrf = [&](int64_t r0, int64_t m, int64_t kp0, int64_t kn) {
		const int64_t N = ncols - r0;
		if(m <= 0 || N <= 0)
			return false;
		const int64_t md = std::min<int64_t>(NB, m), nd = std::min<int64_t>(NB, N);
		const int ti = (int)((md + 31) / 32), tj = (int)((nd + 31) / 32);
		int nA = 0;
		for(int j = 0; j < tj; ++ j)
			nA += std::min(j, ti - 1) + 1;
		const int64_t nbi = (m + 63) / 64, nbj = (N + 63) / 64;
		const int do_potrf = kn >= 0 ? 1 : 0;
		const int64_t kn0 = (kn >= 0 ? kn : 0) * NB;
		const int n_valid = (int)std::max<int64_t>(0, std::min<int64_t>(NB, n_id - kn0));
		const size_t slot = (size_t)(kn >= 0 ? kn : nsteps + 1);
		dw.fuse_expect[slot] += nA;
		hipLaunchKernelGGL(update_potrf_kernel, dim3((unsigned)(nA + do_potrf + nbi * nbj)), dim3(POTRF_THREADS),
			POTRF_LDS_DOUBLES * sizeof(double), s, m, N, d_A + kp0 + r0 * ld, ld, d_A + r0 + r0 * ld, nA, dw.fuse_expect[slot], do_potrf,
			n_valid, (has_rhs && n_valid < NB) ? 1 : 0, dw.tinv_all.p + (size_t)(kn >= 0 ? kn : 0) * NB * NB, dw.info.p, kn0,
			dw.fuse_cnt.p + slot, dw.info.p + 2, (long long)(500.0 * 1e5));
		return true;
	};
	auto potrf_and_panel = [&](int64_t k, bool potrf_done = false) {
		const int64_t k0 = k * NB;
		const int n_valid = (int)std::max<int64_t>(0, std::min<int64_t>(NB, n_id - k0));
		double *tinv = ctx->dense.tinv_all.p + (size_t)k * NB * NB;
		if(!potrf_done)
			hipLaunchKernelGGL(potrf_diag_kernel, dim3(1), dim3(POTRF_THREADS), POTRF_LDS_DOUBLES * sizeof(double), s,
				d_A + k0 + k0 * ld, ld, n_valid, (has_rhs && n_valid < NB) ? 1 : 0, tinv, ctx->dense.info.p, k0);
		const int64_t c1 = k0 + NB;
		if(c1 < ncols)
			launch_panel_solve(s, ncols - c1, tinv, d_A + k0 + c1 * ld, ld);
	};
	auto tile_row = [&](int64_t r0, int64_t kp0) {
		const int64_t m = std::min<int64_t>(NB, rows - r0);
		if(m <= 0 || r0 >= ncols)
			return;
		const double *P = d_A + kp0 + r0 * ld;
		flush_wait_b();
		launch_gemm_staged<32, 32, 16, 16, 0>(s, m, ncols - r0, NB, P, ld, P, ld, d_A + r0 + r0 * ld, ld, true);
	};
	if(allow_fused && nsteps >= 2 && dense_tail_rows() * NB >= rows && dense_tail_applies(ctx, rows, nsteps) &&
		launch_dense_tail(ctx, d_A, ld, rows, ncols, nsteps, -1, has_rhs)) {
		dw.tinv_half = 0;
// ... 435 lines not shown
```

### slam_plus_plus_amd/csrc/spp_dense_tail.h

```cpp
#pragma once
#include "spp_dense_dev.h"

namespace spp {

struct TailArgs {
	double *A;
	int64_t ld;
	int64_t rows;
	int64_t ncols;
	int64_t c0;
	int have_pre;
	int Tr, Tc;
	int has_rhs;
	double *tinv;
	double *dbuf;
	int *pub;
	int epoch;
	int *info, *abort;
	long long timeout_ticks;
	long long *trace;
	const int *order;
};

constexpr int TAIL_ABORT_TIMEOUT = 2;

constexpr int TAIL_LDS_DOUBLES = POTRF_LDS_DOUBLES_INV2 + 16;

#ifndef SPP_TAIL_PLAIN_LD
#define SPP_TAIL_PLAIN_LD 0
#endif
__device__ __forceinline__ double tail_ld(const double *p)
{
#if SPP_TAIL_PLAIN_LD
	return __hip_atomic_load(p, __ATOMIC_RELAXED, __HIP_MEMORY_SCOPE_WORKGROUP);
#else
	return __hip_atomic_load(p, __ATOMIC_RELAXED, __HIP_MEMORY_SCOPE_AGENT);
#endif
}

__device__ __noinline__ void tail_first_tile(double *sm, const v4f64 t00, const int lane, int *info, const int64_t k0)
{
	const int l15 = lane & 15, l4 = lane >> 4;
#pragma unroll
	for(int r = 0; r < 4; ++ r)
		sm[(l4 + 4 * r) + l15 * TS] = t00[r];
	if(lane == 0)
		potrf_lds2_fail(sm)[0] = 0;
	__builtin_amdgcn_fence(__ATOMIC_ACQ_REL, "wavefront");
	__builtin_amdgcn_wave_barrier();
	diag_tile_factor<TS>(sm, potrf_lds2_dv(sm), potrf_lds2_gd0(sm), potrf_lds2_dinv(sm), 0, lane, potrf_lds2_fail(sm), info, k0);
}

__global__ __launch_bounds__(POTRF_THREADS)
void dense_tail_kernel(const TailArgs a)
{
	extern __shared__ double sm[];
	const int tid = threadIdx.x, lane = tid & 63, wave = __builtin_amdgcn_readfirstlane(tid >> 6);
	const int l15 = lane & 15, l4 = lane >> 4;
	int *st = (int*)(sm + POTRF_LDS_DOUBLES_INV2);
	const int ord = a.order[blockIdx.x];
	const int ti = ord >> 16, tj = ord & 0xffff;
	const bool diag = ti == tj;
	const int64_t i0 = a.c0 + (int64_t)NB * ti, j0 = a.c0 + (int64_t)NB * tj;
	const int tag = a.epoch << 4;
	auto stamp = [&](int slot) { if(a.trace && tid == 0) a.trace[ti * 8 + slot] = wall_clock64(); };
	if(diag) stamp(0);
	auto pub_count = [&](const int v, const int w) -> int {
		const int cv = ((v >> 4) == a.epoch) ? (v & 15) : 0, cw = ((w >> 4) == a.epoch) ? (w & 15) : 0;
		return cv < cw ? cv : cw;
	};
	auto wait_pub = [&](const int *p, const int *q, const int need) -> int {
		if(tid == 0) {
			const long long t0 = wall_clock64();
			int got = -1;
			for(;;) {
				const int v = __hip_atomic_load(p, __ATOMIC_RELAXED, __HIP_MEMORY_SCOPE_AGENT);
				const int w = q ? __hip_atomic_load(q, __ATOMIC_RELAXED, __HIP_MEMORY_SCOPE_AGENT) : v;
				const int cv = ((v >> 4) == a.epoch) ? (v & 15) : 0, cw = ((w >> 4) == a.epoch) ? (w & 15) : 0;
				const int c = cv < cw ? cv : cw;
				if(c >= need) {
					got = c;
					break;
				}
				if(__hip_atomic_load(a.abort, __ATOMIC_RELAXED, __HIP_MEMORY_SCOPE_AGENT))
					break;
				if(wall_clock64() - t0 > a.timeout_ticks) {
					__hip_atomic_store(a.abort, TAIL_ABORT_TIMEOUT, __ATOMIC_RELAXED, __HIP_MEMORY_SCOPE_AGENT);
					break;
				}
				__builtin_amdgcn_s_sleep(1);
			}
			st[1] = got;
		}
		lds_barrier();
		const int got = st[1];
		lds_barrier();
		return got;
	};
	int ra[4], cb[4];
#pragma unroll
	for(int u = 0; u < 4; ++ u) {
		if(!diag) {
			ra[u] = wave & 7;
			cb[u] = 4 * (wave >> 3) + u;
		} else {
			int q = (wave == 0) ? (u == 0 ? 0 : 36) : wave + 15 * u, c = 0;
			if(q >= 36)
				ra[u] = cb[u] = -1;
			else {
				while(q > c) {
					q -= c + 1;
					++ c;
				}
				ra[u] = q;
				cb[u] = c;
			}
		}
	}
	v4f64 acc[4];
	{
		double *img = sm;
#pragma unroll 4
		for(int q = 0; q < NB * NB / POTRF_THREADS; ++ q) {
			const int e = tid + q * POTRF_THREADS, r = e & (NB - 1), c = e >> 7;
			const int64_t row = i0 + r, col = j0 + c;
			img[r + c * TS] = (col < a.ncols) ? a.A[row + col * a.ld] : ((diag && row == col) ? 1.0 : 0.0);
		}
		lds_barrier();
#pragma unroll
		for(int u = 0; u < 4; ++ u)
#pragma unroll
			for(int r = 0; r < 4; ++ r)
				acc[u][r] = (ra[u] < 0) ? 0.0 : img[(16 * ra[u] + l4 + 4 * r) + (16 * cb[u] + l15) * TS];
		lds_barrier();
	}
	bool pre_first = false;
	{
		const int ek = tid & 15, ec = tid >> 4;
		constexpr int PS = 18;
		const int ekp = 4 * (ek & 3) + (ek >> 2);
		const int kfirst = a.have_pre ? -1 : 0, nst = 8 * (ti - kfirst);
		double va[2], vb[2];
		auto fetch = [&](const int sidx) {
			const int k = kfirst + (sidx >> 3), J = sidx & 7;
			const double *rowp = a.A + (a.c0 + (int64_t)NB * k) + 16 * J + ek;
#pragma unroll
			for(int h = 0; h < 2; ++ h) {
				const int64_t ca = i0 + ec + 64 * h, cb = j0 + ec + 64 * h;
				va[h] = (ca < (diag ? a.ncols : a.rows)) ? tail_ld(rowp + ca * a.ld) : 0.0;
				vb[h] = (!diag && cb < a.ncols) ? tail_ld(rowp + cb * a.ld) : 0.0;
			}
		};
		int avail = a.have_pre ? 8 : 0;
		pre_first = diag && nst > 0 && (nst & 1) == 0 && a.rows - i0 >= 16;
		bool inflight = false;
		for(int sidx = 0; sidx < nst; ++ sidx) {
			const int k = kfirst + (sidx >> 3), J = sidx & 7;
			if(J == 0 && k >= 0)
				avail = 0;
			if(!inflight) {
				if(J >= avail) {
					avail = wait_pub(a.pub + k * a.Tc + ti, a.pub + k * a.Tc + tj, J + 1);
					if(avail < 0)
						return;
				}
				fetch(sidx);
			}
			int pk = -1;
			if(tid == 0 && k >= 0 && J + 1 < 8 && J + 1 >= avail)
				pk = pub_count(__hip_atomic_load(a.pub + k * a.Tc + ti, __ATOMIC_RELAXED, __HIP_MEMORY_SCOPE_AGENT),
					__hip_atomic_load(a.pub + k * a.Tc + tj, __ATOMIC_RELAXED, __HIP_MEMORY_SCOPE_AGENT));
			double *sa = sm + (sidx & 1) * 2 * NB * PS, *sb = diag ? sa : sa + NB * PS;
#pragma unroll
			for(int h = 0; h < 2; ++ h) {
				sa[ekp + (ec + 64 * h) * PS] = va[h];
				if(!diag)
					sb[ekp + (ec + 64 * h) * PS] = vb[h];
			}
			if(tid == 0)
				st[2 + (sidx & 1)] = pk;
			lds_barrier();
			{
				const int seen = st[2 + (sidx & 1)];
				if(seen > avail)
					avail = seen;
			}
			inflight = (sidx + 1 < nst) && (J + 1 < 8) && (J + 1 < avail);
			if(inflight)
				fetch(sidx + 1);
			double fa[4];
#pragma unroll
			for(int u = 0; u < 4; ++ u) {
				if(ra[u] < 0)
					continue;
				double fb[4];
				if(u == 0 || diag) {
					const bool row_live = i0 + 16 * ra[u] + l15 < a.rows;
					const double2 a01 = *(const double2*)(sa + 4 * l4 + (16 * ra[u] + l15) * PS), a23 = *(const double2*)(sa + 4 * l4 + 2 + (16 * ra[u] + l15) * PS);
					fa[0] = row_live ? -a01.x : 0.0;
					fa[1] = row_live ? -a01.y : 0.0;
					fa[2] = row_live ? -a23.x : 0.0;
					fa[3] = row_live ? -a23.y : 0.0;
				}
				{
					const double2 b01 = *(const double2*)(sb + 4 * l4 + (16 * cb[u] + l15) * PS), b23 = *(const double2*)(sb + 4 * l4 + 2 + (16 * cb[u] + l15) * PS);
					fb[0] = b01.x;
					fb[1] = b01.y;
					fb[2] = b23.x;
					fb[3] = b23.y;
				}
#pragma unroll
				for(int kk = 0; kk < 4; ++ kk)
					acc[u] = __builtin_amdgcn_mfma_f64_16x16x4f64(fa[kk], fb[kk], acc[u], 0, 0, 0);
				if(u == 0 && pre_first && sidx == nst - 1 && wave == 0) {
					tail_first_tile(sm, acc[0], lane, a.info, i0);
				}
			}
		}
		lds_barrier();
	}
	if(diag) stamp(1);
	double *T = sm;
#pragma unroll
	for(int u = 0; u < 4; ++ u)
#pragma unroll
		for(int r = 0; r < 4; ++ r)
			if(ra[u] >= 0 && !(pre_first && wave == 0 && u == 0))
				T[(16 * ra[u] + l4 + 4 * r) + (16 * cb[u] + l15) * TS] = acc[u][r];
	lds_barrier();
	if(diag) {
		const int64_t nv = a.rows - i0;
		const int n_valid = (int)(nv < 0 ? 0 : (nv > NB ? NB : nv));
		PotrfPub pb;
		pb.flag = a.pub + ti * a.Tc + ti;
		pb.base = tag;
		pb.dbuf = a.dbuf + (size_t)ti * 8 * 256;
		pb.abort = a.abort;
		potrf_diag_body<false, 1, 2, true>(a.A + i0 + i0 * a.ld, a.ld, n_valid, (a.has_rhs && n_valid < NB) ? 1 : 0,
			a.tinv + (size_t)ti * NB * NB, a.info, i0, sm, pb, pre_first ? 1 : 0);
		stamp(2);
		return;
	}
	double *Dv = T + NB * TS;
	double *Rr = Dv + 16 * PT;
	const double *Rii = a.A + i0 + i0 * a.ld;
	int avail = 0;
	bool inflight = false;
	double dvr = 0, rr[2] = {0, 0};
	auto fetch_panel = [&](const int J) {
		if(tid < 256)
			dvr = tail_ld(a.dbuf + ((size_t)ti * 8 + J) * 256 + tid);
#pragma unroll
		for(int h = 0; h < 2; ++ h) {
			const int e = tid + POTRF_THREADS * h, k = e & 15, c = e >> 4;
			if(e < 16 * (NB - 16 * (J + 1)))
				rr[h] = tail_ld(Rii + (16 * J + k) + (int64_t)(16 * (J + 1) + c) * a.ld);
		}
	};
	for(int J = 0; J < 8; ++ J) {
		if(!inflight) {
			if(J >= avail) {
				avail = wait_pub(a.pub + ti * a.Tc + ti, nullptr, J + 1);
				if(avail < 0)
					return;
			}
			fetch_panel(J);
		}
		if(tj == ti + 1 && J == 0) stamp(3);
		if(tj == ti + 1 && J == 7) stamp(4);
		int pk = -1;
		if(tid == 0 && J + 1 < 8 && J + 1 >= avail) {
			const int v = __hip_atomic_load(a.pub + ti * a.Tc + ti, __ATOMIC_RELAXED, __HIP_MEMORY_SCOPE_AGENT);
			pk = pub_count(v, v);
		}
		if(tid < 256)
			Dv[(tid & 15) + (tid >> 4) * PT] = dvr;
#pragma unroll
		for(int h = 0; h < 2; ++ h) {
			const int e = tid + POTRF_THREADS * h;
			if(e < 16 * (NB - 16 * (J + 1)))
				Rr[(e & 15) + (e >> 4) * PT] = rr[h];
		}
		if(tid == 0)
			st[2 + (J & 1)] = pk;
		lds_barrier();
		{
			const int seen = st[2 + (J & 1)];
			if(seen > avail)
				avail = seen;
		}
		inflight = (J + 1 < 8) && (J + 1 < avail);
		if(inflight)
			fetch_panel(J + 1);
		if(wave < 8) {
			double *Y = T + 16 * J + (16 * wave) * TS;
			const v4f64 x = tile_atb(Dv, 1, PT, Y, 1, TS, lane);
			__builtin_amdgcn_fence(__ATOMIC_ACQ_REL, "wavefront");
			__builtin_amdgcn_wave_barrier();
			const int64_t col = j0 + 16 * wave + l15;
#pragma unroll
			for(int r = 0; r < 4; ++ r) {
				Y[(l4 + 4 * r) + l15 * TS] = x[r];
				if(col < a.ncols)
					__hip_atomic_store(&a.A[(i0 + 16 * J + l4 + 4 * r) + col * a.ld], x[r], __ATOMIC_RELAXED, __HIP_MEMORY_SCOPE_AGENT);
			}
		}
		lds_barrier();
		{
			const int b = wave & 7;
			double xb[4];
#pragma unroll
			for(int kk = 0; kk < 4; ++ kk)
				xb[kk] = T[16 * J + (4 * kk + l4) + (16 * b + l15) * TS];
			auto row_update = [&](const int I) {
				const double *Ra = Rr + 16 * (I - J - 1) * PT;
				v4f64 d = (v4f64){0, 0, 0, 0};
#pragma unroll
				for(int kk = 0; kk < 4; ++ kk)
					d = __builtin_amdgcn_mfma_f64_16x16x4f64(Ra[(4 * kk + l4) + l15 * PT], xb[kk], d, 0, 0, 0);
				double *D = T + 16 * I + (16 * b) * TS;
#pragma unroll
				for(int r = 0; r < 4; ++ r)
					D[(l4 + 4 * r) + l15 * TS] -= d[r];
			};
			{
				const int I = J + 1 + (wave >> 3);
				if(I < 8)
					row_update(I);
			}
			if(wave < 8)
				asm volatile("s_waitcnt vmcnt(0)" ::: "memory");
			lds_barrier();
			if(tid == 0)
				__hip_atomic_store(a.pub + ti * a.Tc + tj, tag | (J + 1), __ATOMIC_RELAXED, __HIP_MEMORY_SCOPE_AGENT);
			for(int I = J + 3 + (wave >> 3); I < 8; I += 2)
				row_update(I);
			lds_barrier();
		}
		if(tj == ti + 1 && J == 7) stamp(5);
	}
}

// ... 2 lines not shown
```

### slam_plus_plus_amd/csrc/spp_internal.h

```cpp
#pragma once

#include <hip/hip_runtime.h>
#include <stdint.h>
#include <string>
#include <vector>
#include <sys/mman.h>
#include <utility>
#include <new>
#include <exception>
#include <thread>
#include <stdexcept>
#include <algorithm>
#include <string.h>
#include <chrono>
#include <stdio.h>
#include <stdlib.h>
#include "../../include/spp_hip.h"

namespace spp {

struct Error : std::runtime_error {
	int code;
	Error(int c, const std::string &what) : std::runtime_error(what), code(c) {}
};
// ... 23 lines not shown
		if(!on)
			return;
		const std::chrono::steady_clock::time_point n = std::chrono::steady_clock::now();
		fprintf(stderr, "[spp] %s: %-34s %8.2f ms\n", who, what, std::chrono::duration<double>(n - t).count() * 1e3);
		t = n;
	}
};

template <class T>
struct HugeAlloc {
	typedef T value_type;
	HugeAlloc() {}
	template <class U> HugeAlloc(const HugeAlloc<U>&) {}
	T *allocate(size_t n)
	{
		const size_t bytes = n * sizeof(T), huge = (size_t)2 << 20;
		void *q = nullptr;
		if(bytes >= ((size_t)4 << 20)) {
			if(posix_memalign(&q, huge, (bytes + huge - 1) & ~(huge - 1)) != 0)
				q = nullptr;
#ifdef MADV_HUGEPAGE
			if(q)
				madvise(q, bytes, MADV_HUGEPAGE);
#endif
		}
		if(!q)
			q = malloc(bytes ? bytes : 1);
		if(!q)
			throw std::bad_alloc();
		return (T*)q;
	}
	void deallocate(T *p, size_t) { free(p); }
	template <class U> void construct(U *p) { ::new((void*)p) U; }
	template <class U, class A0, class... A> void construct(U *p, A0 &&a0, A &&... a) { ::new((void*)p) U(std::forward<A0>(a0), std::forward<A>(a)...); }
	template <class U> bool operator==(const HugeAlloc<U>&) const { return true; }
	template <class U> bool operator!=(const HugeAlloc<U>&) const { return false; }
};
template <class T> using HVec = std::vector<T, HugeAlloc<T> >;

template <class T>
struct DevBuf {
	T *p = nullptr;
	size_t cap = 0;
	bool owned = true;
	DevBuf() {}
	DevBuf(const DevBuf&) = delete;
	DevBuf &operator=(const DevBuf&) = delete;
	~DevBuf() { release(); }
	void release()
	{
		if(p && owned)
			(void)hipFree(p);
		p = nullptr;
		cap = 0;
		owned = true;
	}
	void view(T *ptr, size_t n)
	{
		release();
		p = ptr;
		cap = n;
		owned = false;
	}
	void reserve(size_t n)
	{
		if(n <= cap && owned)
			return;
		release();
		size_t want = n;
		hipError_t e = hipMalloc((void**)&p, want * sizeof(T));
		if(e != hipSuccess) {
			p = nullptr;
			throw Error(SPP_E_NOMEM, "hipMalloc of " + std::to_string(want * sizeof(T)) + " bytes failed");
		}
		cap = want;
	}
	template <class A>
	void upload(const std::vector<T, A> &h, hipStream_t s)
	{
		reserve(h.size() ? h.size() : 1);
		if(!h.empty())
			SPP_HIP_CHECK(hipMemcpyAsync(p, h.data(), h.size() * sizeof(T), hipMemcpyHostToDevice, s));
	}
};

struct UploadArena {
	hipStream_t stream;
	std::vector<unsigned char> host;
	struct Item { void **pp; size_t *pcap; bool *powned; size_t off, n; };
	std::vector<Item> items;
	explicit UploadArena(hipStream_t s) : stream(s) { host.reserve(size_t(1) << 20); }
	template <class T, class A>
	void add(DevBuf<T> &b, const std::vector<T, A> &v)
	{
		if(v.size() * sizeof(T) > (size_t(256) << 10)) {
			b.upload(v, stream);
			return;
		}
		b.release();
		const size_t off = (host.size() + 255) & ~(size_t)255, bytes = std::max<size_t>(v.size(), 1) * sizeof(T);
		host.resize(off + bytes);
		if(!v.empty())
			memcpy(host.data() + off, v.data(), v.size() * sizeof(T));
		Item it = {(void**)&b.p, &b.cap, &b.owned, off, std::max<size_t>(v.size(), 1)};
		items.push_back(it);
	}
	void commit(DevBuf<unsigned char> &store)
	{
		store.release();
		store.reserve(std::max<size_t>(host.size(), 256));
		if(!host.empty())
			SPP_HIP_CHECK(hipMemcpyAsync(store.p, host.data(), host.size(), hipMemcpyHostToDevice, stream));
		for(size_t i = 0; i < items.size(); ++ i) {
			*items[i].pp = store.p + items[i].off;
			*items[i].pcap = items[i].n;
			*items[i].powned = false;
		}
	}
};

struct Structure {
	int64_t nb = 0, n = 0, nnzb = 0, nvals = 0;
	HVec<int64_t> col_ptr, row_idx, blk_off, base;
	HVec<int32_t> dim;
};

struct SaccItem {
	int32_t beg, end;
	int32_t kind;
	int32_t pad;
	int64_t dst;
	int64_t aoff;
};

struct SchurPlan {
	int dp = 0, dl = 0;
	int64_t nc = 0, nl = 0;
	int64_t nl_total = 0;
	int64_t no = 0;
	int64_t n_red = 0, ld = 0;
	int64_t n_sblk = 0;
	int64_t n_pairs = 0;
	int64_t n_items = 0, n_multi = 0;
	bool add_A = true;
	bool u_landmark_major = true;
	bool factored = true;
	bool sparse_S = false;
	bool mis = false;
	Structure s_st;
	DevBuf<int64_t> sblk_voff;
	std::vector<int64_t> pose_block;
	std::vector<int64_t> lm_block;
	std::vector<uint8_t> is_lm;
	DevBuf<int32_t> lm_ptr;
	DevBuf<int32_t> bs_ptr;
	int64_t n_bs = 0;
	DevBuf<int64_t> lm_coff;
	DevBuf<int64_t> lm_rbase;
	DevBuf<int32_t> obs_pose;
	DevBuf<int32_t> obs_lm;
	DevBuf<int64_t> obs_off;
	DevBuf<int64_t> pose_rbase;
	DevBuf<int32_t> cam_ptr;
	DevBuf<int32_t> cam_obs;
	DevBuf<int32_t> obs_wpos;
	DevBuf<SaccItem> items;
	DevBuf<int32_t> xcd_beg;
	int32_t xcd_max_items = 0;
	DevBuf<int32_t> sblk_i1, sblk_i2;
	DevBuf<int64_t> sblk_aoff;
	DevBuf<int32_t> pair_a, pair_b;
	DevBuf<int32_t> multi_blk;
	DevBuf<int32_t> multi_ptr;
	DevBuf<double> cinv;
	DevBuf<double> lfac;
	DevBuf<double> W;
	DevBuf<double> Up;
	DevBuf<double> xw;
	DevBuf<double> partial;
	DevBuf<double> S;
	void release_all();
};

struct DenseWork {
	DevBuf<double> tinv;
	DevBuf<int> info;
	DevBuf<double> tinv_all;
	int64_t tinv_half = 0;
	DevBuf<double> xtmp;
	DevBuf<int> flags;
	DevBuf<int> tail_pub;
	DevBuf<double> tail_dinv;
	int tail_epoch = 0;
	DevBuf<int> tail_order;
	std::vector<int> tail_order_host;
	int tail_order_tr = 0, tail_order_tc = 0;
	int tail_rows_last = 0;
	bool tail_disabled = false;
	DevBuf<double> trsv_m;
	DevBuf<double> trsv_pay;
	uint64_t epoch = 0;
	int *h_chain_err = nullptr;
	hipStream_t aux = nullptr;
	hipEvent_t ev[2] = {nullptr, nullptr};
	DevBuf<int> sync;
	DevBuf<int> fuse_cnt;
	std::vector<int> fuse_expect;
	bool fuse_dirty = false;
	int64_t ident_from = -1;
	hipStream_t chain = nullptr;
	hipEvent_t ev_chain = nullptr;
	DevBuf<int> la_cnt;
	DevBuf<long long> la_trace;
	int la_state = 0;
	int la_reserve = 0;
	int la_ncu = 0;
	int sync_epoch = 0;
	int sync_state = 0;
	hipStream_t sync_stream = nullptr;
};

struct SparsePlan;

struct AssemblePlan;

struct PhaseTimer {
	hipEvent_t ev[2 * SPP_N_PHASES];
	bool used[SPP_N_PHASES];
	bool created = false;
};

}

struct spp_ctx {
	int device = 0;
	int flags = 0;
	hipStream_t stream = nullptr;
	bool own_stream = false;
	std::string last_error;
	int mode = -1;
	int shard_rank = 0, shard_world = 1;
	spp::Structure st;
	std::vector<int64_t> order;
	std::thread plan_trash;
	spp::SchurPlan schur;
	spp::DenseWork dense;
	spp::SparsePlan *sparse = nullptr;
	spp::AssemblePlan *assemble = nullptr;
	spp::DevBuf<double> d_vals, d_rhs;
	double *h_staging = nullptr;
	size_t h_staging_cap = 0;
	spp::DevBuf<double> geom_partial;
	spp::PhaseTimer timer;
	double phase_ms[SPP_N_PHASES] = {0};
	std::vector<hipEvent_t> dom_events;
	size_t dom_used = 0;
	double dom_flops = 0;
	int64_t factor_flops = 0, solve_bytes = 0, factor_nnz = 0;
};

namespace spp {

void se2_linearize(spp_ctx *ctx, int64_t ne, const int32_t *d_v0, const int32_t *d_v1, const double *d_poses,
	const double *d_meas, double *d_J0, double *d_J1, double *d_r);
double se2_update(spp_ctx *ctx, int64_t nv, double *d_poses, const double *d_dx, bool apply);
double edge_chi2(spp_ctx *ctx, int64_t ne, int rd, const double *d_r, const double *d_Om);
void edge_robust_weights(spp_ctx *ctx, int64_t ne, int rd, int kind, double scale, double param, const double *d_r, double *d_w);
double edge_hessian_maxdiag(spp_ctx *ctx, int64_t ne, int rd, int d0, int d1, const double *d_J0, const double *d_J1,
	const double *d_Om);
double lm_gain_denominator(spp_ctx *ctx, int64_t n, const double *d_dx, const double *d_rhs, double alpha);
void se3_linearize(spp_ctx *ctx, int64_t ne, const int32_t *d_v0, const int32_t *d_v1, const double *d_poses,
	const double *d_meas, double *d_J0, double *d_J1, double *d_r);
double se3_update(spp_ctx *ctx, int64_t nv, double *d_poses, const double *d_dx, bool apply);
void ba_linearize(spp_ctx *ctx, int64_t no, const int32_t *d_cam_of, const int32_t *d_pt_of, const double *d_cams,
	const double *d_intr, const double *d_pts, const double *d_meas, double *d_J0, double *d_J1, double *d_r);
double ba_update(spp_ctx *ctx, int64_t nc, double *d_cams, const int64_t *d_cam_dxoff, int64_t np, double *d_pts,
	const int64_t *d_pt_dxoff, const double *d_dx, int64_t n_dx, bool apply);

void min_degree_order(int64_t nb, const int64_t *col_ptr, const int64_t *row_idx, std::vector<int64_t> &order);
void nested_dissection_order(int64_t nb, const int64_t *col_ptr, const int64_t *row_idx, std::vector<int64_t> &order);
void build_schur_plan(spp_ctx *ctx, bool sparse_S, bool mis = false);
int64_t schur_buffer_doubles(const spp_ctx *ctx);
bool schur_applicable(const Structure &st, int *dp, int *dl);
double schur_plan_host_probe(const Structure &st, int shard_rank, int shard_world, bool sparse_S, bool mis, int64_t *out);

void sparse_analyze(spp_ctx *ctx, const Structure &st);
int sparse_factor_solve(spp_ctx *ctx, const double *d_vals, double *d_rhs);
void sparse_release(spp_ctx *ctx);
void sparse_dag_disable(spp_ctx *ctx);
int64_t sparse_info(const spp_ctx *ctx, int what);

void schur_form(spp_ctx *ctx, const double *d_vals, const double *d_rhs, double *d_S_rhs);
int schur_finish(spp_ctx *ctx, const double *d_vals, double *d_S_rhs, double *d_rhs);
void schur_pack(spp_ctx *ctx, double *S, double *packed, bool pack);

constexpr int DENSE_NB = 128;
int dense_potrf_upper(spp_ctx *ctx, double *d_A, int64_t n, int64_t ld, bool keep_inverses);
void dense_potrf_upper_enqueue(spp_ctx *ctx, double *d_A, int64_t n, int64_t ld);
int dense_info_fetch(spp_ctx *ctx, bool *dag_aborted = nullptr);
void dense_potrs_upper(spp_ctx *ctx, const double *d_R, int64_t n, int64_t ld, double *d_b);
void dense_aux_park(int device, hipStream_t s);
void dense_factor_steps(spp_ctx *ctx, double *d_A, int64_t ld, int64_t n, int64_t rows, int64_t ncols,
	int64_t nsteps, bool has_rhs);
void dense_info_reset(spp_ctx *ctx);
void dense_reserve(spp_ctx *ctx, int64_t nblk);

void dense_chain_check(spp_ctx *ctx);
void dense_set_padding(spp_ctx *ctx, double *d_A, int64_t ld, int64_t n);
int dense_front_factor(spp_ctx *ctx, double *d_F, int64_t ld, int64_t w, int64_t h, double *d_image);
bool dense_gemm_tn_sub(spp_ctx *ctx, int64_t m, int64_t n, int64_t k, const double *A, int64_t lda,
	const double *B, int64_t ldb, double *C, int64_t ldc, bool upper_only);
double microbench_copy(spp_ctx *ctx, size_t bytes, int iters);
double microbench_mfma_f64(spp_ctx *ctx, int iters);
double microbench_ctile(spp_ctx *ctx, int n, int iters);
double microbench_update(spp_ctx *ctx, int64_t m, int iters);

void assemble_analyze(spp_ctx *ctx, int64_t nv, const int32_t *dim, int64_t ne, const int64_t *v0,
	const int64_t *v1, int d0, int d1, int rd, int64_t unary_vertex);
void assemble_run(spp_ctx *ctx, const double *J0, const double *J1, const double *Om, const double *r,
	double damping, double *vals, double *eta);
void assemble_set_edge_weights(spp_ctx *ctx, const double *d_w);
void assemble_release(spp_ctx *ctx);
void assemble_get_structure(const spp_ctx *ctx, int64_t *col_ptr, int64_t *row_idx, int64_t *blk_off);

void phase_begin(spp_ctx *ctx, int phase);
void phase_end(spp_ctx *ctx, int phase);
void phases_reset(spp_ctx *ctx);
void phases_collect(spp_ctx *ctx);
void dom_begin(spp_ctx *ctx);
void dom_end(spp_ctx *ctx, double flops);

template <class F>
inline void run_threads(int nt, F fn)
{
	if(nt <= 1) {
		fn(0);
		return;
	}
	std::vector<std::thread> th;
	std::exception_ptr err[64];
	for(int t = 1; t < nt; ++ t)
		th.emplace_back([&, t]() { try { fn(t); } catch(...) { err[t] = std::current_exception(); } });
	try { fn(0); } catch(...) { err[0] = std::current_exception(); }
	for(size_t t = 0; t < th.size(); ++ t)
		th[t].join();
	for(int t = 0; t < nt; ++ t)
		if(err[t])
			std::rethrow_exception(err[t]);
}

inline int plan_threads(int64_t work)
{
	static int env = -1;
	if(env < 0) {
		const char *e = getenv("SPP_PLAN_THREADS");
		env = e ? std::max(1, atoi(e)) : 0;
	}
	static int64_t min_work = -1;
	if(min_work < 0) {
		const char *e = getenv("SPP_PLAN_MIN_WORK");
		min_work = e ? std::max<int64_t>(1, atoll(e)) : (int64_t(1) << 18);
	}
	int nt = env ? env : (int)std::min<unsigned>(16u, std::max(1u, std::thread::hardware_concurrency()));
	if(work < min_work)
		nt = 1;
	return std::min(nt, 64);
}

template <class V>
inline void balanced_cuts(const V &w_prefix, int nt, std::vector<int64_t> &cut)
{
	const int64_t n = (int64_t)w_prefix.size() - 1, total = w_prefix[n];
	cut.assign(nt + 1, n);
	cut[0] = 0;
	for(int t = 1; t < nt; ++ t)
		cut[t] = std::lower_bound(w_prefix.begin(), w_prefix.end(), total * t / nt) - w_prefix.begin();
	for(int t = 1; t <= nt; ++ t)
		cut[t] = std::max(cut[t], cut[t - 1]);
	cut[nt] = n;
}


}
```

### slam_plus_plus_amd/csrc/spp_schur.hip

```cpp

#include "spp_internal.h"

namespace spp {

template <int DL>
__device__ __forceinline__ void cinv_block(const double *__restrict__ m, double *o)
{
	if(DL == 3) {
#define M_(i, j) m[(i) + 3 * (j)]
#define COF_(i, j) (M_(((i) + 1) % 3, ((j) + 1) % 3) * M_(((i) + 2) % 3, ((j) + 2) % 3) - \
	M_(((i) + 1) % 3, ((j) + 2) % 3) * M_(((i) + 2) % 3, ((j) + 1) % 3))
		const double c00 = COF_(0, 0), c10 = COF_(1, 0), c20 = COF_(2, 0);
		const double det = c00 * M_(0, 0) + c10 * M_(1, 0) + c20 * M_(2, 0);
		const double id = -1.0 / det;
		o[0] = c00 * id; o[3] = c10 * id; o[6] = c20 * id;
		o[1] = COF_(0, 1) * id; o[4] = COF_(1, 1) * id; o[7] = COF_(2, 1) * id;
		o[2] = COF_(0, 2) * id; o[5] = COF_(1, 2) * id; o[8] = COF_(2, 2) * id;
#undef COF_
#undef M_
	} else if(DL == 2) {
		const double det = m[0] * m[3] - m[2] * m[1];
		const double id = -1.0 / det;
		o[0] = m[3] * id; o[2] = -m[2] * id;
		o[1] = -m[1] * id; o[3] = m[0] * id;
// ... 684 lines not shown
#pragma unroll
	for(int q = 0; q < DL; ++ q) {
		double sum = 0;
#pragma unroll
		for(int u = 0; u < DL; ++ u)
			sum += Ci[q + DL * u] * t[u];
		rhs[rb + q] = sum;
	}
}

template <int DP, int DL>
__global__ __launch_bounds__(256)
void backsubst_fused_kernel(const int32_t *__restrict__ bs_ptr, const int32_t *__restrict__ lm_ptr, const int32_t *__restrict__ obs_pose,
	const int64_t *__restrict__ obs_off, const int64_t *__restrict__ lm_rbase, const double *__restrict__ cinv,
	const int64_t *__restrict__ lm_coff, const double *__restrict__ vals, const double *__restrict__ dx, double *__restrict__ rhs)
{
	__shared__ double tq[256 * DL];
	const int32_t l0 = bs_ptr[blockIdx.x], l1 = bs_ptr[blockIdx.x + 1];
	const int32_t a0 = lm_ptr[l0], na = lm_ptr[l1] - a0;
	const int t = threadIdx.x;
	if(t < na) {
		const int64_t a = (int64_t)a0 + t;
		double u[DP * DL];
		load_U<DP, DL>(vals, obs_off[a], u);
		double dv[DP];
		const double *d = dx + (int64_t)obs_pose[a] * DP;
#pragma unroll
		for(int r = 0; r < DP; ++ r)
			dv[r] = d[r];
#pragma unroll
		for(int q = 0; q < DL; ++ q) {
			double sum = 0;
#pragma unroll
			for(int r = 0; r < DP; ++ r)
				sum += dv[r] * u[r + DP * q];
			tq[t * DL + q] = sum;
		}
	}
	__syncthreads();
	if(t >= l1 - l0)
		return;
	const int64_t l = (int64_t)l0 + t;
	double tv[DL];
	const int64_t rb = lm_rbase[l];
#pragma unroll
	for(int q = 0; q < DL; ++ q)
		tv[q] = -rhs[rb + q];
	for(int32_t a = lm_ptr[l] - a0, e = lm_ptr[l + 1] - a0; a < e; ++ a) {
#pragma unroll
		for(int q = 0; q < DL; ++ q)
			tv[q] += tq[a * DL + q];
	}
	double Ci[DL * DL];
	if(cinv) {
#pragma unroll
		for(int e = 0; e < DL * DL; ++ e)
			Ci[e] = cinv[l * DL * DL + e];
	} else
		cinv_block<DL>(vals + lm_coff[l], Ci);
#pragma unroll
	for(int q = 0; q < DL; ++ q) {
		double sum = 0;
#pragma unroll
		for(int u = 0; u < DL; ++ u)
			sum += Ci[q + DL * u] * tv[u];
		rhs[rb + q] = sum;
	}
}

template <int DP>
__global__ __launch_bounds__(256)
void scatter_dx_kernel(int64_t nc, const int64_t *__restrict__ pose_rbase, const double *__restrict__ dx,
	double *__restrict__ rhs)
{
	const int64_t e = (int64_t)blockIdx.x * blockDim.x + threadIdx.x;
	if(e >= nc * DP)
		return;
	rhs[pose_rbase[e / DP] + e % DP] = dx[e];
}

template <int DP, int DL>
static void schur_form_t(spp_ctx *ctx, const double *d_vals, const double *d_rhs, double *S)
{
	SchurPlan &sp = ctx->schur;
	hipStream_t s = ctx->stream;
	const int64_t ld = sp.ld;
	const int64_t *voff = sp.sparse_S ? sp.sblk_voff.p : nullptr;
	double *xcol = sp.sparse_S ? S + sp.s_st.nvals : S + sp.n_red * ld;
	phase_begin(ctx, SPP_PHASE_SCHUR_INV);
	if(S == sp.S.p && !sp.sparse_S && ctx->shard_world == 1 && sp.n_sblk == sp.nc * (sp.nc + 1) / 2 && sp.n_red == sp.nc * DP)
		SPP_HIP_CHECK(hipMemsetAsync(S + sp.n_red * ld, 0, (size_t)(schur_buffer_doubles(ctx) - sp.n_red * ld) * sizeof(double), s));
	else
		SPP_HIP_CHECK(hipMemsetAsync(S, 0, (size_t)schur_buffer_doubles(ctx) * sizeof(double), s));
	constexpr int VIL = VSplit<DP * DL>::IL;
	double *Vm = sp.W.p, *Vs = sp.W.p + sp.no * VIL;
	const bool onfly = sp.factored && DL <= 3;
	if(sp.nl && !onfly)
		hipLaunchKernelGGL((cinv_kernel<DL>), dim3((unsigned)((sp.nl + 255) / 256)), dim3(256), 0, s,
			sp.nl, sp.lm_coff.p, d_vals, sp.cinv.p, sp.factored ? sp.lfac.p : nullptr);
	if(sp.no && sp.factored)
		hipLaunchKernelGGL((obs_fact_kernel<DP, DL>), dim3((unsigned)((sp.no + 255) / 256)), dim3(256), 0, s,
			sp.no, sp.obs_lm.p, sp.obs_off.p, sp.lm_rbase.p, d_vals, d_rhs, onfly ? (const double*)nullptr : (const double*)sp.lfac.p, sp.lm_coff.p,
			sp.obs_wpos.p, Vm, Vs, sp.xw.p);
	else if(sp.no)
		hipLaunchKernelGGL((obs_kernel<DP, DL>), dim3((unsigned)((sp.no + 255) / 256)), dim3(256), 0, s,
			sp.no, sp.obs_lm.p, sp.obs_off.p, sp.lm_rbase.p, d_vals, d_rhs, sp.cinv.p, sp.obs_wpos.p, sp.W.p, sp.Up.p, sp.xw.p, sp.u_landmark_major ? 1 : 0);
	phase_end(ctx, SPP_PHASE_SCHUR_INV);
	phase_begin(ctx, SPP_PHASE_SCHUR_GEMM);
	if(sp.n_items) {
		static int chunk_env = -1;
		if(chunk_env < 0) {
			const char *e = getenv("SPP_SACC_CHUNK");
			chunk_env = e ? atoi(e) : 1;
		}
		int chunk = chunk_env;
		if(chunk <= 0)
			chunk = (int)((sp.xcd_max_items + SACC_WAVES * 64 - 1) / (SACC_WAVES * 64));
		const int64_t per = (int64_t)SACC_WAVES * chunk;
		if(sp.factored)
			hipLaunchKernelGGL((s_accum_kernel<DP, DL, true>), dim3((unsigned)(8 * ((sp.xcd_max_items + per - 1) / per))), dim3(SACC_WAVES * 64), 0, s,
				sp.items.p, sp.xcd_beg.p, chunk, sp.pair_a.p, sp.pair_b.p, Vm, Vs, d_vals, S, ld, sp.partial.p);
		else
			hipLaunchKernelGGL((s_accum_kernel<DP, DL, false>), dim3((unsigned)(8 * ((sp.xcd_max_items + per - 1) / per))), dim3(SACC_WAVES * 64), 0, s,
				sp.items.p, sp.xcd_beg.p, chunk, sp.pair_a.p, sp.pair_b.p, sp.W.p, sp.Up.p, d_vals, S, ld, sp.partial.p);
	}
	if(sp.n_multi)
		hipLaunchKernelGGL((s_multi_kernel<DP>), dim3((unsigned)((sp.n_multi + 3) / 4)), dim3(256), 0, s,
			sp.n_multi, sp.multi_blk.p, sp.multi_ptr.p, sp.sblk_i1.p, sp.sblk_i2.p, sp.sblk_aoff.p,
			sp.partial.p, d_vals, sp.add_A ? 1 : 0, S, ld, voff);
	phase_end(ctx, SPP_PHASE_SCHUR_GEMM);
	phase_begin(ctx, SPP_PHASE_SCHUR_RHS);
	if(sp.nc)
		hipLaunchKernelGGL((rhs_kernel<DP>), dim3((unsigned)((sp.nc + 3) / 4)), dim3(256), 0, s,
			sp.nc, sp.cam_ptr.p, sp.cam_obs.p, sp.pose_rbase.p, sp.xw.p, d_rhs, sp.add_A ? 1 : 0, xcol);
	phase_end(ctx, SPP_PHASE_SCHUR_RHS);
	SPP_HIP_CHECK(hipGetLastError());
}

template <int DP, int DL>
static int schur_finish_t(spp_ctx *ctx, const double *d_vals, double *S, double *d_rhs)
{
	SchurPlan &sp = ctx->schur;
	hipStream_t s = ctx->stream;
	const int64_t ld = sp.ld;
	double *xcol;
	if(sp.sparse_S) {
		xcol = S + sp.s_st.nvals;
		const int ret = sparse_factor_solve(ctx, S, xcol);
		if(ret != SPP_OK)
			return ret;
	} else {
		phase_begin(ctx, SPP_PHASE_FACTOR);
		dense_set_padding(ctx, S, ld, sp.n_red);
		dense_potrf_upper_enqueue(ctx, S, sp.n_red, ld);
		phase_end(ctx, SPP_PHASE_FACTOR);
		xcol = S + sp.n_red * ld;
		phase_begin(ctx, SPP_PHASE_TRISOLVE);
		dense_potrs_upper(ctx, S, sp.n_red, ld, xcol);
		phase_end(ctx, SPP_PHASE_TRISOLVE);
	}
	phase_begin(ctx, SPP_PHASE_BACKSUBST);
	static_assert(DL <= DP, "the products U^T dx reuse the W l buffer (DP doubles per observation)");
	static int bs_fused = -1;
	if(bs_fused < 0) {
		const char *e = getenv("SPP_BACKSUBST_FUSED");
		bs_fused = e ? atoi(e) : 1;
	}
	const double *cinv_arg = (sp.factored && DL <= 3) ? (const double*)nullptr : (const double*)sp.cinv.p;
	if(bs_fused && sp.n_bs > 0)
		hipLaunchKernelGGL((backsubst_fused_kernel<DP, DL>), dim3((unsigned)sp.n_bs), dim3(256), 0, s,
			sp.bs_ptr.p, sp.lm_ptr.p, sp.obs_pose.p, sp.obs_off.p, sp.lm_rbase.p, cinv_arg, sp.lm_coff.p, d_vals, xcol, d_rhs);
	else {
		if(sp.no)
			hipLaunchKernelGGL((backsubst_obs_kernel<DP, DL>), dim3((unsigned)((sp.no + 255) / 256)), dim3(256), 0, s,
				sp.no, sp.obs_pose.p, sp.obs_off.p, d_vals, xcol, sp.xw.p);
		if(sp.nl)
			hipLaunchKernelGGL((backsubst_lm_kernel<DL>), dim3((unsigned)((sp.nl + 255) / 256)), dim3(256), 0, s,
				sp.nl, sp.lm_ptr.p, sp.lm_rbase.p, sp.xw.p, cinv_arg, sp.lm_coff.p, d_vals, d_rhs);
	}
	if(sp.nc)
		hipLaunchKernelGGL((scatter_dx_kernel<DP>), dim3((unsigned)((sp.nc * DP + 255) / 256)), dim3(256), 0, s,
			sp.nc, sp.pose_rbase.p, xcol, d_rhs);
	phase_end(ctx, SPP_PHASE_BACKSUBST);
	SPP_HIP_CHECK(hipGetLastError());
	if(!sp.sparse_S && dense_info_fetch(ctx))
		return SPP_NOT_POSDEF;
	return SPP_OK;
}

template <bool PACK>
__global__ __launch_bounds__(256)
void schur_pack_kernel(double *__restrict__ S, int64_t ld, double *__restrict__ packed)
{
	const int64_t k = blockIdx.y;
	const int64_t rows = 128 * (k + 1);
	const int64_t e = (int64_t)blockIdx.x * 256 + threadIdx.x;
	if(e >= rows * 128)
		return;
	const int64_t r = e % rows, c = e / rows;
	double *ps = S + r + (128 * k + c) * ld;
	double *pp = packed + 128 * 128 * (k * (k + 1) / 2) + e;
	if(PACK)
		*pp = *ps;
	else
		*ps = *pp;
}

void schur_pack(spp_ctx *ctx, double *S, double *packed, bool pack)
{
	const int64_t ld = ctx->schur.ld, nblk = ld / 128;
	dim3 grid((unsigned)((ld * 128 + 255) / 256), (unsigned)nblk);
	if(pack)
		hipLaunchKernelGGL((schur_pack_kernel<true>), grid, dim3(256), 0, ctx->stream, S, ld, packed);
	else
		hipLaunchKernelGGL((schur_pack_kernel<false>), grid, dim3(256), 0, ctx->stream, S, ld, packed);
	SPP_HIP_CHECK(hipGetLastError());
}

void schur_form(spp_ctx *ctx, const double *d_vals, const double *d_rhs, double *d_S_rhs)
{
	const int dp = ctx->schur.dp, dl = ctx->schur.dl;
	if(dp == 6 && dl == 3) schur_form_t<6, 3>(ctx, d_vals, d_rhs, d_S_rhs);
	else if(dp == 3 && dl == 2) schur_form_t<3, 2>(ctx, d_vals, d_rhs, d_S_rhs);
	else if(dp == 3 && dl == 3) schur_form_t<3, 3>(ctx, d_vals, d_rhs, d_S_rhs);
	else if(dp == 6 && dl == 6) schur_form_t<6, 6>(ctx, d_vals, d_rhs, d_S_rhs);
	else throw Error(SPP_E_UNSUPPORTED, "Schur kernels: block widths not instantiated");
}

int schur_finish(spp_ctx *ctx, const double *d_vals, double *d_S_rhs, double *d_rhs)
{
	const int dp = ctx->schur.dp, dl = ctx->schur.dl;
	if(dp == 6 && dl == 3) return schur_finish_t<6, 3>(ctx, d_vals, d_S_rhs, d_rhs);
	if(dp == 3 && dl == 2) return schur_finish_t<3, 2>(ctx, d_vals, d_S_rhs, d_rhs);
	if(dp == 3 && dl == 3) return schur_finish_t<3, 3>(ctx, d_vals, d_S_rhs, d_rhs);
	if(dp == 6 && dl == 6) return schur_finish_t<6, 6>(ctx, d_vals, d_S_rhs, d_rhs);
	throw Error(SPP_E_UNSUPPORTED, "Schur kernels: block widths not instantiated");
}

}
```

### slam_plus_plus_amd/csrc/spp_symbolic.cpp

```cpp

#include "spp_internal.h"
#include <sys/mman.h>
#include <stdlib.h>
#include <algorithm>
#include <numeric>
#include <string.h>
#include <stdlib.h>
#include <stdio.h>
#include <thread>
#include <memory>
#include <chrono>
#include <exception>

namespace spp {

void SchurPlan::release_all()
{
	lm_ptr.release(); bs_ptr.release(); n_bs = 0; lm_coff.release(); lm_rbase.release(); obs_pose.release(); obs_lm.release();
	obs_off.release(); pose_rbase.release(); cam_ptr.release(); cam_obs.release(); items.release();
	obs_wpos.release(); xcd_beg.release(); sblk_i1.release(); sblk_i2.release(); sblk_aoff.release();
	sblk_voff.release(); s_st = Structure(); sparse_S = false; mis = false;
	pair_a.release(); pair_b.release(); multi_blk.release(); multi_ptr.release(); cinv.release(); lfac.release();
	W.release(); Up.release(); xw.release(); partial.release(); S.release();
	pose_block.clear(); lm_block.clear(); is_lm.clear();
}

bool schur_applicable(const Structure &st, int *dp_out, int *dl_out)
{
	int d_a = -1, d_b = -1;
	for(int64_t j = 0; j < st.nb; ++ j) {
		int d = st.dim[j];
		if(d_a < 0 || d == d_a) d_a = d;
		else if(d_b < 0 || d == d_b) d_b = d;
		else return false;
	}
	if(d_a < 0 || d_b < 0)
		return false;
	int dp = std::max(d_a, d_b), dl = std::min(d_a, d_b);
	if(!((dp == 6 && dl == 3) || (dp == 3 && dl == 2)))
		return false;
	int64_t n_lm = 0;
	for(int64_t j = 0; j < st.nb; ++ j) {
		if(st.dim[j] == dl)
			++ n_lm;
		for(int64_t p = st.col_ptr[j]; p < st.col_ptr[j + 1]; ++ p) {
			int64_t i = st.row_idx[p];
			if(i != j && st.dim[i] == dl && st.dim[j] == dl)
				return false;
		}
	}
	if(n_lm == 0)
		return false;
	*dp_out = dp;
	*dl_out = dl;
	return true;
}

static const int PAIR_CHUNK = 2048;

int64_t schur_buffer_doubles(const spp_ctx *ctx)
{
	const SchurPlan &sp = ctx->schur;
	return sp.sparse_S ? sp.s_st.nvals + sp.n_red : sp.ld * sp.ld;
}

static bool mis_partition(const Structure &st, std::vector<uint8_t> &is_lm, int *d_out)
{
	const int d = st.dim[0];
	for(int64_t j = 0; j < st.nb; ++ j)
		if(st.dim[j] != d)
			return false;
	if(d != 3 && d != 6)
		return false;
	std::vector<std::vector<int32_t> > adj(st.nb);
	for(int64_t j = 0; j < st.nb; ++ j)
		for(int64_t p = st.col_ptr[j]; p < st.col_ptr[j + 1]; ++ p) {
			const int64_t i = st.row_idx[p];
			if(i != j) {
				adj[i].push_back((int32_t)j);
				adj[j].push_back((int32_t)i);
			}
		}
	std::vector<int32_t> order(st.nb);
	for(int64_t j = 0; j < st.nb; ++ j)
		order[j] = (int32_t)j;
	std::stable_sort(order.begin(), order.end(), [&](int32_t a, int32_t b) { return adj[a].size() < adj[b].size(); });
	is_lm.assign(st.nb, 0);
	std::vector<uint8_t> blocked(st.nb, 0);
	int64_t n_lm = 0;
	for(int64_t q = 0; q < st.nb; ++ q) {
		const int32_t v = order[q];
		if(blocked[v])
			continue;
		is_lm[v] = 1;
		++ n_lm;
		for(size_t e = 0; e < adj[v].size(); ++ e)
			blocked[adj[v][e]] = 1;
	}
	*d_out = d;
	return n_lm > 0 && n_lm < st.nb;
}

template <class T>
struct RawBuf {
	T *p = nullptr;
	size_t n = 0;
	RawBuf() {}
	RawBuf(const RawBuf&) = delete;
	RawBuf &operator=(const RawBuf&) = delete;
	~RawBuf() { free(p); }
	void resize(size_t m)
	{
		free(p);
		p = nullptr;
		if(m) {
			const size_t bytes = m * sizeof(T);
			if(bytes >= ((size_t)8 << 20)) {
				void *q = nullptr;
				if(posix_memalign(&q, (size_t)2 << 20, (bytes + (((size_t)2 << 20) - 1)) & ~(((size_t)2 << 20) - 1)) == 0) {
					p = (T*)q;
#ifdef MADV_HUGEPAGE
					madvise(q, bytes, MADV_HUGEPAGE);
#endif
				}
			}
			if(!p)
				p = (T*)malloc(bytes);
			if(!p)
				throw std::bad_alloc();
		}
		n = m;
	}
	size_t size() const { return n; }
	T &operator[](size_t i) { return p[i]; }
	const T &operator[](size_t i) const { return p[i]; }
};

struct SchurPlanHost {
	int dp = 0, dl = 0;
	int64_t nc = 0, nl = 0, nl_total = 0, no = 0, n_red = 0, ld = 0, n_sblk = 0, n_pairs = 0, n_items = 0, n_multi = 0, n_ablk = 0;
	int32_t n_slots = 0, xcd_max_items = 0;
	bool u_landmark_major = true, factored = true;
	std::vector<int64_t> pose_block, lm_block;
	std::vector<uint8_t> is_lm;
	HVec<int32_t> lm_ptr, obs_pose, obs_lm, cam_obs, wpos;
	std::vector<int32_t> bs_ptr;
	std::vector<int32_t> cam_ptr, sblk_i1, sblk_i2, multi_blk, multi_ptr, xb;
	RawBuf<int32_t> pair_a, pair_b;
	HVec<int64_t> lm_coff, obs_off, lm_rbase;
	std::vector<int64_t> sblk_aoff, sblk_voff, pose_rbase;
	std::vector<SaccItem> recs;
	Structure s_st;
};

static void schur_plan_host(const Structure &st, int shard_rank, int shard_world, bool sparse_S, bool mis, SchurPlanHost &h)
{
	VClock clk("schur plan");
	int dp, dl;
	std::vector<uint8_t> &is_lm = h.is_lm;
	if(mis) {
		SPP_REQUIRE(mis_partition(st, is_lm, &dp), SPP_E_UNSUPPORTED,
			"MIS Schur mode needs a graph of one block width (3 or 6) with at least one edge");
		dl = dp;
	} else {
		SPP_REQUIRE(schur_applicable(st, &dp, &dl), SPP_E_UNSUPPORTED,
			"Schur mode needs exactly two block widths ({6,3} or {3,2}) and a block-diagonal landmark part");
		is_lm.assign(st.nb, 0);
		for(int64_t j = 0; j < st.nb; ++ j)
			is_lm[j] = st.dim[j] == dl;
	}
	h.dp = dp;
	h.dl = dl;

	std::vector<int32_t> pose_of(st.nb, -1), lm_of(st.nb, -1);
	int64_t nc = 0, nl_total = 0, nl = 0;
	for(int64_t j = 0; j < st.nb; ++ j) {
		if(!is_lm[j]) {
			pose_of[j] = (int32_t)nc ++;
			h.pose_block.push_back(j);
		} else {
			if(nl_total % shard_world == shard_rank) {
				lm_of[j] = (int32_t)nl ++;
				h.lm_block.push_back(j);
			}
			++ nl_total;
		}
	}
	h.nc = nc;
	h.nl = nl;
	h.nl_total = nl_total;
	const bool add_A = (shard_rank == 0);
	h.n_red = nc * dp;
	h.ld = ((h.n_red + 1 + DENSE_NB - 1) / DENSE_NB) * DENSE_NB;
	SPP_REQUIRE(sparse_S || h.ld <= 65536, SPP_E_UNSUPPORTED,
		"reduced camera system too large for the dense path (use SPP_MODE_SCHUR_SPARSE)");

	struct Obs { int32_t lm, pose; int64_t off; };
	HVec<int64_t> &lm_coff = h.lm_coff;
	lm_coff.assign(nl, -1);
	struct ABlk { int32_t i1, i2; int64_t off; };
	std::vector<ABlk> ablk;
	HVec<int32_t> &lm_ptr = h.lm_ptr, &obs_pose = h.obs_pose, &obs_lm = h.obs_lm;
	HVec<int64_t> &obs_off = h.obs_off;
	bool obs_sorted = true;
	const int nts = plan_threads(st.nnzb);
	std::vector<int64_t> jcut;
	balanced_cuts(st.col_ptr, nts, jcut);
	{
		std::vector<int64_t> n_obs_t(nts + 1, 0), n_ab_t(nts + 1, 0);
		auto classify = [&](int64_t j, int64_t p, Obs &o) -> int {
			const int64_t i = st.row_idx[p];
			const bool pi = !is_lm[i], pj = !is_lm[j];
			if(pi && pj)
				return 0;
			if(!pi && !pj)
				return 1;
			if(pi) {
				if(lm_of[j] < 0)
					return 3;
				o = {lm_of[j], pose_of[i], st.blk_off[p] << 1};
			} else {
				if(lm_of[i] < 0)
					return 3;
				o = {lm_of[i], pose_of[j], (st.blk_off[p] << 1) | 1};
			}
			return 2;
		};
		run_threads(nts, [&](int t) {
			int64_t n_o = 0, n_a = 0;
			Obs o;
			for(int64_t j = jcut[t]; j < jcut[t + 1]; ++ j)
				for(int64_t p = st.col_ptr[j]; p < st.col_ptr[j + 1]; ++ p) {
					const int k = classify(j, p, o);
					n_o += k == 2;
					n_a += k == 0;
				}
			n_obs_t[t + 1] = n_o;
			n_ab_t[t + 1] = n_a;
		});
		for(int t = 0; t < nts; ++ t) {
			n_obs_t[t + 1] += n_obs_t[t];
			n_ab_t[t + 1] += n_ab_t[t];
		}
		const int64_t no_all = n_obs_t[nts];
		SPP_REQUIRE(no_all < (int64_t(1) << 31), SPP_E_UNSUPPORTED, "too many observations for 32-bit obs indices");
		obs_pose.resize(no_all);
		obs_lm.resize(no_all);
		obs_off.resize(no_all);
		ablk.resize(n_ab_t[nts]);
		std::vector<char> sorted_t(nts, 1);
		run_threads(nts, [&](int t) {
			int64_t a = n_obs_t[t], q = n_ab_t[t];
			Obs o, prev = {-1, -1, 0};
			bool sorted = true;
			for(int64_t j = jcut[t]; j < jcut[t + 1]; ++ j)
				for(int64_t p = st.col_ptr[j]; p < st.col_ptr[j + 1]; ++ p) {
					const int k = classify(j, p, o);
					if(k == 0)
						ablk[q ++] = {pose_of[st.row_idx[p]], pose_of[j], st.blk_off[p]};
					else if(k == 1) {
						if(lm_of[j] >= 0)
							lm_coff[lm_of[j]] = st.blk_off[p];
					} else if(k == 2) {
						if(o.lm < prev.lm || (o.lm == prev.lm && o.pose < prev.pose))
							sorted = false;
						prev = o;
						obs_lm[a] = o.lm;
						obs_pose[a] = o.pose;
						obs_off[a] = o.off;
						++ a;
					}
				}
			sorted_t[t] = sorted;
		});
		for(int t = 0; t < nts; ++ t)
			obs_sorted = obs_sorted && sorted_t[t];
		for(int t = 1; t < nts && obs_sorted; ++ t) {
			const int64_t a = n_obs_t[t];
			if(a > 0 && a < no_all && (obs_lm[a] < obs_lm[a - 1] || (obs_lm[a] == obs_lm[a - 1] && obs_pose[a] < obs_pose[a - 1])))
				obs_sorted = false;
		}
	}
	h.n_ablk = (int64_t)ablk.size();
	clk.lap("partition + observation scan");
	for(int64_t l = 0; l < nl; ++ l)
		SPP_REQUIRE(lm_coff[l] >= 0, SPP_E_BADARG, "landmark without a diagonal block");
	std::vector<std::vector<int32_t> > foreign_cols;
	if(sparse_S && shard_world > 1) {
		std::vector<int64_t> lm_gidx(st.nb, -1);
		int64_t g = 0;
		for(int64_t j = 0; j < st.nb; ++ j)
			if(is_lm[j])
				lm_gidx[j] = g ++;
		std::vector<std::vector<int32_t> > poses_of(g);
		for(int64_t j = 0; j < st.nb; ++ j)
			for(int64_t p = st.col_ptr[j]; p < st.col_ptr[j + 1]; ++ p) {
				const int64_t i = st.row_idx[p];
				const bool pi = !is_lm[i], pj = !is_lm[j];
				if(pi && !pj && lm_of[j] < 0)
					poses_of[lm_gidx[j]].push_back(pose_of[i]);
				else if(!pi && pj && lm_of[i] < 0)
					poses_of[lm_gidx[i]].push_back(pose_of[j]);
			}
		foreign_cols.resize(nc);
		for(int64_t l = 0; l < g; ++ l) {
			std::vector<int32_t> &ps = poses_of[l];
			std::sort(ps.begin(), ps.end());
			for(size_t a = 0; a < ps.size(); ++ a)
				for(size_t b = a + 1; b < ps.size(); ++ b)
					foreign_cols[ps[a]].push_back(ps[b]);
		}
		for(int64_t c = 0; c < nc; ++ c) {
			std::sort(foreign_cols[c].begin(), foreign_cols[c].end());
			foreign_cols[c].erase(std::unique(foreign_cols[c].begin(), foreign_cols[c].end()), foreign_cols[c].end());
		}
	}
	const int64_t no = (int64_t)obs_pose.size();
	h.no = no;
	if(!obs_sorted) {
		std::vector<Obs> obs(no);
		for(int64_t a = 0; a < no; ++ a)
			obs[a] = {obs_lm[a], obs_pose[a], obs_off[a]};
		std::sort(obs.begin(), obs.end(), [](const Obs &a, const Obs &b) {
			return a.lm != b.lm ? a.lm < b.lm : a.pose < b.pose; });
		for(int64_t a = 0; a < no; ++ a) {
			obs_lm[a] = obs[a].lm;
			obs_pose[a] = obs[a].pose;
			obs_off[a] = obs[a].off;
		}
	}
	lm_ptr.resize(nl + 1);
	const int nto = plan_threads(no);
	run_threads(nto, [&](int t) {
		const int64_t a0 = no * t / nto, a1 = no * (t + 1) / nto;
		for(int64_t a = a0; a < a1; ++ a) {
			const int32_t lp = a ? obs_lm[a - 1] : -1, lc = obs_lm[a];
			for(int32_t l = lp + 1; l <= lc; ++ l)
				lm_ptr[l] = (int32_t)a;
		}
	});
	for(int64_t l = (no ? obs_lm[no - 1] : -1) + 1; l <= nl; ++ l)
		lm_ptr[l] = (int32_t)no;

	{
		const int32_t BS_OBS = 256;
		std::vector<int32_t> &bp = h.bs_ptr;
		bp.clear();
		bp.reserve((size_t)(no / 160 + 2));
// ... 242 lines not shown
		if(tb_env < 0) {
			const char *e = getenv("SPP_SACC_TILE");
			tb_env = e ? std::max<int64_t>(1, atol(e)) : 4;
		}
		static int64_t tbc_env = -1;
		if(tbc_env < 0) {
			const char *e = getenv("SPP_SACC_TILE_COLS");
			tbc_env = e ? atol(e) : -2;
		}
		const int64_t TB = tb_env, TBC = (tbc_env == -2) ? TB : (tbc_env <= 0 ? nc : tbc_env), ntile = (nc + TBC - 1) / TBC;
		std::vector<int32_t> perm(item_blk.size());
		for(size_t q = 0; q < perm.size(); ++ q)
			perm[q] = (int32_t)q;
		static int il_env = -1;
		if(il_env < 0) {
			const char *e = getenv("SPP_SACC_XCD");
			il_env = e ? atoi(e) : 1;
		}
		interleave = il_env != 0;
		std::vector<int64_t> tile_of_item(item_blk.size());
		for(size_t q = 0; q < tile_of_item.size(); ++ q)
			tile_of_item[q] = (sblk_i1[item_blk[q]] / TB) * ntile + sblk_i2[item_blk[q]] / TBC;
		auto tile_of = [&](int32_t q) { return tile_of_item[q]; };
		auto stable_by_key = [&](std::vector<int32_t> &pm, int64_t n_keys, auto key_of) {
			if(n_keys > 8 * (int64_t)pm.size() + 1024) {
				std::stable_sort(pm.begin(), pm.end(), [&](int32_t x, int32_t y) { return key_of(x) < key_of(y); });
				return;
			}
			std::vector<int32_t> start((size_t)n_keys + 1, 0), out(pm.size());
			for(size_t q = 0; q < pm.size(); ++ q)
				++ start[key_of(pm[q]) + 1];
			for(int64_t k = 0; k < n_keys; ++ k)
				start[k + 1] += start[k];
			for(size_t q = 0; q < pm.size(); ++ q)
				out[start[key_of(pm[q])] ++] = pm[q];
			pm.swap(out);
		};
		stable_by_key(perm, ((nc + TB - 1) / TB) * ntile, tile_of);
		if(interleave) {
			std::vector<int32_t> xcd_of(perm.size());
			int64_t load[8] = {0, 0, 0, 0, 0, 0, 0, 0};
			for(size_t q = 0; q < perm.size();) {
				const int64_t t = tile_of(perm[q]);
				size_t e = q;
				int64_t cost = 0;
				for(; e < perm.size() && tile_of(perm[e]) == t; ++ e)
					cost += 2 + (item_end[perm[e]] - item_beg[perm[e]] + 63) / 64;
				int x = 0;
				for(int y = 1; y < 8; ++ y)
					if(load[y] < load[x])
						x = y;
				load[x] += cost;
				for(size_t i = q; i < e; ++ i)
					xcd_of[perm[i]] = x;
				q = e;
			}
			stable_by_key(perm, 8, [&](int32_t x) { return (int64_t)xcd_of[x]; });
			xb_il.assign(9, 0);
			for(size_t q = 0; q < perm.size(); ++ q)
				++ xb_il[xcd_of[q] + 1];
			for(int x = 0; x < 8; ++ x)
				xb_il[x + 1] += xb_il[x];
		}
		std::vector<int32_t> t_blk(perm.size()), t_beg(perm.size()), t_end(perm.size()), t_slot(perm.size());
		for(size_t q = 0; q < perm.size(); ++ q) {
			t_blk[q] = item_blk[perm[q]];
			t_beg[q] = item_beg[perm[q]];
			t_end[q] = item_end[perm[q]];
			t_slot[q] = item_slot[perm[q]];
		}
		item_blk.swap(t_blk); item_beg.swap(t_beg); item_end.swap(t_end); item_slot.swap(t_slot);
	}
	h.n_items = (int64_t)item_blk.size();
	{
		std::vector<int32_t> &xb = h.xb;
		xb.assign(9, 0);
		if(interleave)
			xb = xb_il;
		else {
			std::vector<int64_t> cost(h.n_items + 1, 0);
			for(int64_t q = 0; q < h.n_items; ++ q)
				cost[q + 1] = cost[q] + 2 + (item_end[q] - item_beg[q] + 63) / 64;
			for(int x = 1; x < 8; ++ x)
				xb[x] = (int32_t)(std::lower_bound(cost.begin(), cost.end(), cost[h.n_items] * x / 8) - cost.begin());
			xb[8] = (int32_t)h.n_items;
		}
		h.xcd_max_items = 0;
		for(int x = 0; x < 8; ++ x) {
			xb[x + 1] = std::max(xb[x + 1], xb[x]);
			h.xcd_max_items = std::max(h.xcd_max_items, xb[x + 1] - xb[x]);
		}
	}
	h.n_multi = (int64_t)multi_blk.size();

	h.pose_rbase.resize(nc);
	h.lm_rbase.resize(nl);
	for(int64_t c = 0; c < nc; ++ c)
		h.pose_rbase[c] = st.base[h.pose_block[c]];
	for(int64_t l = 0; l < nl; ++ l)
		h.lm_rbase[l] = st.base[h.lm_block[l]];

	clk.lap("work items");
	h.recs.resize(item_blk.size());
	for(size_t q = 0; q < h.recs.size(); ++ q) {
		const int32_t b = item_blk[q];
		SaccItem &r = h.recs[q];
		r.beg = item_beg[q];
		r.end = item_end[q];
		r.pad = 0;
		r.aoff = -1;
		if(item_slot[q] >= 0) {
			r.kind = 2;
			r.dst = (int64_t)item_slot[q] * dp * dp;
		} else {
			r.aoff = add_A ? sblk_aoff[b] : -1;
			if(sparse_S) {
				r.kind = 1;
				r.dst = h.sblk_voff[b];
			} else {
				r.kind = 0;
				r.dst = (int64_t)sblk_i1[b] * dp + (int64_t)sblk_i2[b] * dp * h.ld;
			}
		}
	}
	clk.lap("item records");
}

void build_schur_plan(spp_ctx *ctx, bool sparse_S, bool mis)
{
	const Structure &st = ctx->st;
	SchurPlan &sp = ctx->schur;
	sp.release_all();
	sp.sparse_S = sparse_S;
	hipStream_t s = ctx->stream;
	VClock clk0("schur plan (device)");
	std::unique_ptr<SchurPlanHost> hp(new SchurPlanHost);
	SchurPlanHost &h = *hp;
	clk0.lap("old plan released");
	schur_plan_host(st, ctx->shard_rank, ctx->shard_world, sparse_S, mis, h);
	VClock clk("schur plan (device)");
	const int dp = h.dp, dl = h.dl;
	const int64_t nc = h.nc, nl = h.nl, no = h.no;
	sp.dp = dp;
	sp.dl = dl;
	sp.pose_block.swap(h.pose_block);
	sp.lm_block.swap(h.lm_block);
	sp.is_lm.swap(h.is_lm);
	sp.nc = nc;
	sp.nl = nl;
	sp.nl_total = h.nl_total;
	sp.add_A = (ctx->shard_rank == 0);
	sp.n_red = h.n_red;
	sp.ld = h.ld;
	sp.no = no;
	sp.n_pairs = h.n_pairs;
	sp.n_sblk = h.n_sblk;
	sp.u_landmark_major = h.u_landmark_major;
	sp.factored = h.factored;
	sp.n_items = h.n_items;
	sp.n_multi = h.n_multi;
	sp.xcd_max_items = h.xcd_max_items;
	if(sparse_S) {
		sp.s_st = h.s_st;
		sp.sblk_voff.upload(h.sblk_voff, s);
	}

	sp.xcd_beg.upload(h.xb, s);
	sp.lm_ptr.upload(h.lm_ptr, s);
	sp.n_bs = h.bs_ptr.empty() ? 0 : (int64_t)h.bs_ptr.size() - 1;
	sp.bs_ptr.upload(h.bs_ptr, s);
	sp.lm_coff.upload(h.lm_coff, s);
	sp.lm_rbase.upload(h.lm_rbase, s);
	sp.obs_pose.upload(h.obs_pose, s);
	sp.obs_lm.upload(h.obs_lm, s);
	sp.obs_off.upload(h.obs_off, s);
	sp.pose_rbase.upload(h.pose_rbase, s);
	sp.cam_ptr.upload(h.cam_ptr, s);
	sp.cam_obs.upload(h.cam_obs, s);
	sp.items.upload(h.recs, s);
	sp.obs_wpos.upload(h.wpos, s);
	sp.sblk_i1.upload(h.sblk_i1, s);
	sp.sblk_i2.upload(h.sblk_i2, s);
	sp.sblk_aoff.upload(h.sblk_aoff, s);
	sp.pair_a.reserve(std::max<size_t>(1, h.pair_a.size()));
	sp.pair_b.reserve(std::max<size_t>(1, h.pair_b.size()));
	if(h.pair_a.size()) {
		SPP_HIP_CHECK(hipMemcpyAsync(sp.pair_a.p, h.pair_a.p, h.pair_a.size() * sizeof(int32_t), hipMemcpyHostToDevice, s));
		SPP_HIP_CHECK(hipMemcpyAsync(sp.pair_b.p, h.pair_b.p, h.pair_b.size() * sizeof(int32_t), hipMemcpyHostToDevice, s));
	}
	sp.multi_blk.upload(h.multi_blk, s);
	sp.multi_ptr.upload(h.multi_ptr, s);
	clk.lap("uploads enqueued");
	sp.cinv.reserve((size_t)std::max<int64_t>(1, nl) * dl * dl);
	sp.W.reserve((size_t)std::max<int64_t>(1, no) * dp * dl);
	if(sp.factored)
		sp.lfac.reserve((size_t)std::max<int64_t>(1, nl) * dl * dl);
	else
		sp.Up.reserve((size_t)std::max<int64_t>(1, no) * dp * dl);
	sp.xw.reserve((size_t)std::max<int64_t>(1, no) * dp);
	sp.partial.reserve((size_t)std::max<int32_t>(1, h.n_slots) * dp * dp);
	clk.lap("workspaces allocated");
	SPP_HIP_CHECK(hipStreamSynchronize(s));
	clk.lap("uploads done");

	if(!sparse_S)
		dense_reserve(ctx, (sp.n_red + DENSE_NB - 1) / DENSE_NB);
	clk.lap("dense workspaces");

	const double n = (double)sp.n_red;
	ctx->factor_flops = (int64_t)(n * n * n / 3.0 + 2.0 * n * n);
	ctx->factor_nnz = sp.ld * sp.ld;
	const int64_t blk_pl = 8 * dp * dl, blk_pp = 8 * dp * dp, blk_ll = 8 * dl * dl;
	ctx->solve_bytes = blk_pl * no + blk_ll * nl + blk_pp * h.n_ablk + 8 * st.n
		+ blk_pp * sp.n_sblk + 8 * st.n
		+ 8 * sp.n_red * sp.n_red ;
	if(ctx->plan_trash.joinable())
		ctx->plan_trash.join();
	{
		SchurPlanHost *raw = hp.release();
		try {
			ctx->plan_trash = std::thread([raw]() { delete raw; });
		} catch(...) {
			delete raw;
		}
	}
	clk.lap("host plan handed to the releasing thread");
}

double schur_plan_host_probe(const Structure &st, int shard_rank, int shard_world, bool sparse_S, bool mis, int64_t *out)
{
	const auto t0 = std::chrono::steady_clock::now();
	SchurPlanHost h;
	schur_plan_host(st, shard_rank, shard_world, sparse_S || mis, mis, h);
	const double sec = std::chrono::duration<double>(std::chrono::steady_clock::now() - t0).count();
	uint64_t sum = 1469598103934665603ull;
	auto mix = [&](uint64_t v) { sum = (sum ^ v) * 1099511628211ull; };
	for(size_t q = 0; q < h.pair_a.size(); ++ q)
		mix(((uint64_t)(uint32_t)h.pair_a[q] << 32) | (uint32_t)h.pair_b[q]);
	for(size_t q = 0; q < h.sblk_i1.size(); ++ q) {
		mix(((uint64_t)(uint32_t)h.sblk_i1[q] << 32) | (uint32_t)h.sblk_i2[q]);
		mix((uint64_t)h.sblk_aoff[q]);
	}
	for(size_t q = 0; q < h.recs.size(); ++ q) {
		mix(((uint64_t)(uint32_t)h.recs[q].beg << 32) | (uint32_t)h.recs[q].end);
		mix((uint64_t)h.recs[q].dst);
		mix((uint64_t)h.recs[q].aoff + (uint64_t)h.recs[q].kind);
	}
	for(size_t q = 0; q < h.xb.size(); ++ q)
		mix((uint64_t)h.xb[q]);
	out[0] = h.nc; out[1] = h.nl; out[2] = h.no; out[3] = h.n_pairs; out[4] = h.n_sblk; out[5] = h.n_items; out[6] = h.n_multi;
	out[7] = (int64_t)sum;
	return sec;
}

void min_degree_order(int64_t nb, const int64_t *col_ptr, const int64_t *row_idx, std::vector<int64_t> &order)
{
	order.clear();
	order.reserve(nb);
	if(nb == 0)
		return;
	std::vector<std::vector<int32_t> > adj(nb), elems(nb);
	for(int64_t j = 0; j < nb; ++ j)
		for(int64_t p = col_ptr[j]; p < col_ptr[j + 1]; ++ p) {
			int64_t i = row_idx[p];
			if(i != j) {
				adj[i].push_back((int32_t)j);
				adj[j].push_back((int32_t)i);
			}
		}
	for(int64_t i = 0; i < nb; ++ i) {
		std::sort(adj[i].begin(), adj[i].end());
		adj[i].erase(std::unique(adj[i].begin(), adj[i].end()), adj[i].end());
	}
	std::vector<std::vector<int32_t> > elem_vars(nb);
	std::vector<uint8_t> state(nb, 0);
	std::vector<int64_t> degree(nb);
	std::vector<int64_t> w(nb, -1);
	std::vector<int64_t> mark(nb, -1);
	std::vector<int32_t> head(nb + 1, -1), next(nb, -1), prev(nb, -1);
	auto bucket_insert = [&](int32_t v) {
		int64_t d = std::min<int64_t>(degree[v], nb);
		next[v] = head[d];
		prev[v] = -1;
		if(head[d] >= 0) prev[head[d]] = v;
		head[d] = v;
	};
	auto bucket_remove = [&](int32_t v) {
		int64_t d = std::min<int64_t>(degree[v], nb);
		if(prev[v] >= 0) next[prev[v]] = next[v]; else head[d] = next[v];
		if(next[v] >= 0) prev[next[v]] = prev[v];
	};
	for(int64_t i = 0; i < nb; ++ i) {
		degree[i] = (int64_t)adj[i].size();
		bucket_insert((int32_t)i);
	}
	int64_t mindeg = 0;
	std::vector<int32_t> Lp;
	for(int64_t step = 0; step < nb; ++ step) {
		while(mindeg <= nb && head[mindeg] < 0)
			++ mindeg;
		const int32_t p = head[mindeg];
		bucket_remove(p);
		order.push_back(p);
		Lp.clear();
		mark[p] = step;
		for(size_t q = 0; q < adj[p].size(); ++ q) {
			int32_t v = adj[p][q];
			if(state[v] == 0 && mark[v] != step) {
				mark[v] = step;
				Lp.push_back(v);
			}
		}
		for(size_t q = 0; q < elems[p].size(); ++ q) {
			int32_t e = elems[p][q];
			if(state[e] != 1)
				continue;
			for(size_t t = 0; t < elem_vars[e].size(); ++ t) {
				int32_t v = elem_vars[e][t];
				if(state[v] == 0 && mark[v] != step) {
					mark[v] = step;
					Lp.push_back(v);
				}
			}
			state[e] = 2;
			std::vector<int32_t>().swap(elem_vars[e]);
		}
		state[p] = 1;
		std::vector<int32_t>().swap(adj[p]);
		std::vector<int32_t>().swap(elems[p]);
		elem_vars[p] = Lp;
		const int64_t lp = (int64_t)Lp.size();
		for(size_t q = 0; q < Lp.size(); ++ q) {
			int32_t v = Lp[q];
			for(size_t t = 0; t < elems[v].size(); ++ t) {
				int32_t e = elems[v][t];
				if(state[e] != 1)
					continue;
				if(w[e] < step * (nb + 1)) {
					int64_t sz = 0;
					for(size_t u = 0; u < elem_vars[e].size(); ++ u)
						if(state[elem_vars[e][u]] == 0)
							++ sz;
					w[e] = step * (nb + 1) + sz;
				}
				-- w[e];
			}
		}
		for(size_t q = 0; q < Lp.size(); ++ q) {
			const int32_t v = Lp[q];
			bucket_remove(v);
			{
				std::vector<int32_t> &a = adj[v];
				size_t o = 0;
				for(size_t t = 0; t < a.size(); ++ t)
					if(state[a[t]] == 0 && mark[a[t]] != step)
						a[o ++] = a[t];
				a.resize(o);
			}
			int64_t d = (int64_t)adj[v].size() + (lp - 1);
			{
				std::vector<int32_t> &el = elems[v];
				size_t o = 0;
				for(size_t t = 0; t < el.size(); ++ t) {
					int32_t e = el[t];
					if(state[e] != 1)
						continue;
					int64_t we = w[e] - step * (nb + 1);
					if(we <= 0) {
						continue;
					}
					d += we;
					el[o ++] = e;
				}
				el.resize(o);
				el.push_back(p);
			}
			degree[v] = std::min<int64_t>(std::min<int64_t>(d, nb - step - 1), degree[v] + lp - 1);
			if(degree[v] < 0) degree[v] = 0;
			bucket_insert(v);
			if(degree[v] < mindeg)
				mindeg = degree[v];
		}
	}
}


static const int ND_LEAF = 48;

void nested_dissection_order(int64_t nb, const int64_t *col_ptr, const int64_t *row_idx, std::vector<int64_t> &order)
{
	order.assign(nb, -1);
	if(nb == 0)
		return;
	std::vector<std::vector<int32_t> > adj(nb);
	for(int64_t j = 0; j < nb; ++ j)
		for(int64_t p = col_ptr[j]; p < col_ptr[j + 1]; ++ p) {
			const int64_t i = row_idx[p];
			if(i != j) {
				adj[i].push_back((int32_t)j);
				adj[j].push_back((int32_t)i);
			}
		}
	std::vector<int32_t> part(nb, 0), level(nb, -1), local(nb, -1);
	struct Task { std::vector<int32_t> verts; int64_t lo; };
	std::vector<Task> stack;
	{
		Task t;
// ... 169 lines not shown
```

Baseline: 1.116 billion block-nnz/s.

## Skip structurally zero tiles in streamed dense Cholesky tail via tile sparsity mask

Computes a 128-wide tile-level sparsity mask of the reduced camera matrix from the Schur structure, closed under Cholesky fill, and passes it to the streamed tail factorization. The tail kernel launches only the tiles marked nonzero and, per tile, skips update steps whose source panel tiles are structurally zero. Because the tile order can now change with the mask, the order is rebuilt (with a stream sync) when the mask changes. The mask is limited to at most 64 tile rows, and for venice-sized systems with dense camera coupling it may be nearly full, leaving little to skip.

```diff
diff --git a/include/spp_hip.h b/include/spp_hip.h
--- a/include/spp_hip.h
+++ b/include/spp_hip.h
@@ -142,6 +142,11 @@
 
 int spp_dense_potrf_upper(spp_ctx *ctx, double *d_A, int64_t n, int64_t ld);
 int spp_dense_posv(spp_ctx *ctx, double *d_A, int64_t n, int64_t ld, double *d_b);
+int spp_dense_posv_masked(spp_ctx *ctx, double *d_A, int64_t n, int64_t ld, double *d_b, const uint64_t *words, int64_t nwords);
+int spp_tile_mask_host(int64_t n, int bs, int64_t nblk, const int32_t *i1, const int32_t *i2, int has_rhs, int fill,
+	uint64_t *words, int64_t *n_updates);
+int spp_schur_tile_mask_host(int64_t nb, const int32_t *dim, const int64_t *col_ptr, const int64_t *row_idx, int shard_rank,
+	int shard_world, uint64_t *words);
 int spp_dense_gemm_tn_sub(spp_ctx *ctx, int64_t m, int64_t n, int64_t k,
 	const double *d_A, int64_t lda, const double *d_B, int64_t ldb, double *d_C, int64_t ldc);
 int spp_dense_gemm_tn_sub_upper(spp_ctx *ctx, int64_t m, int64_t n, int64_t k,
diff --git a/slam_plus_plus_amd/api.py b/slam_plus_plus_amd/api.py
--- a/slam_plus_plus_amd/api.py
+++ b/slam_plus_plus_amd/api.py
@@ -22,6 +22,7 @@
     "spp_device_free", "spp_memcpy_h2d", "spp_memcpy_d2h", "spp_memcpy_d2d", "spp_get_phase_ms", "spp_get_dominant_kernel",
     "spp_microbench_copy", "spp_microbench_mfma_f64", "spp_microbench_ctile", "spp_microbench_update", "spp_block_ordering", "spp_schur_plan_host", "spp_set_profiling", "spp_se2_linearize_device", "spp_se2_update_device", "spp_ba_linearize_device", "spp_ba_update_device", "spp_se3_linearize_device", "spp_se3_update_device", "spp_edge_chi2_device", "spp_edge_robust_weights_device", "spp_edge_hessian_maxdiag_device",
     "spp_lm_gain_denominator_device", "spp_dense_potrf_upper", "spp_dense_posv",
+    "spp_dense_posv_masked", "spp_tile_mask_host", "spp_schur_tile_mask_host",
     "spp_dense_gemm_tn_sub", "spp_dense_gemm_tn_sub_upper", "spp_dense_front_factor", "spp_version",
 ]
 
@@ -94,6 +95,9 @@
         "spp_ba_update_device": (cint, [vp, ctypes.c_int64, vp, vp, ctypes.c_int64, vp, vp, vp, ctypes.c_int64, cint, _c_f64p]),
         "spp_dense_potrf_upper": (cint, [vp, vp, i64, i64]),
         "spp_dense_posv": (cint, [vp, vp, i64, i64, vp]),
+        "spp_dense_posv_masked": (cint, [vp, vp, i64, i64, vp, vp, i64]),
+        "spp_tile_mask_host": (cint, [i64, cint, i64, vp, vp, cint, cint, vp, vp]),
+        "spp_schur_tile_mask_host": (cint, [i64, vp, vp, vp, cint, cint, vp]),
         "spp_dense_gemm_tn_sub": (cint, [vp, i64, i64, i64, vp, i64, vp, i64, vp, i64]),
         "spp_dense_gemm_tn_sub_upper": (cint, [vp, i64, i64, i64, vp, i64, vp, i64, vp, i64]),
         "spp_dense_front_factor": (cint, [vp, vp, i64, i64, i64, vp]),
@@ -142,6 +146,31 @@
     return d
 
 
+def tile_mask_host(n, bs, i1, i2, has_rhs=True, fill=True):
+    lib = load_library()
+    i1 = np.ascontiguousarray(i1, dtype=np.int32)
+    i2 = np.ascontiguousarray(i2, dtype=np.int32)
+    words = np.zeros(64, dtype=np.uint64)
+    upd = ctypes.c_int64(0)
+    code = lib.spp_tile_mask_host(n, bs, i1.size, _ptr(i1), _ptr(i2), 1 if has_rhs else 0, 1 if fill else 0, _ptr(words),
+                                  ctypes.byref(upd))
+    if code < 0:
+        raise SppError("spp_tile_mask_host failed: %d" % code)
+    return words[:code].copy(), upd.value
+
+
+def schur_tile_mask_host(lam, shard_rank=0, shard_world=1):
+    lib = load_library()
+    col_ptr = np.ascontiguousarray(lam.col_ptr, dtype=np.int64)
+    row_idx = np.ascontiguousarray(lam.row_idx, dtype=np.int64)
+    dim = np.ascontiguousarray(lam.dim, dtype=np.int32)
+    words = np.zeros(64, dtype=np.uint64)
+    code = lib.spp_schur_tile_mask_host(lam.nb, _ptr(dim), _ptr(col_ptr), _ptr(row_idx), shard_rank, shard_world, _ptr(words))
+    if code < 0:
+        raise SppError("spp_schur_tile_mask_host failed: %d" % code)
+    return words[:code].copy()
+
+
 class DeviceArray:
 
     def __init__(self, ctx, n, dtype=np.float64):
diff --git a/slam_plus_plus_amd/csrc/spp_api.cpp b/slam_plus_plus_amd/csrc/spp_api.cpp
--- a/slam_plus_plus_amd/csrc/spp_api.cpp
+++ b/slam_plus_plus_amd/csrc/spp_api.cpp
@@ -131,6 +131,7 @@
 	ctx->dense.tail_pub.release();
 	ctx->dense.tail_order.release();
 	ctx->dense.tail_order_tr = ctx->dense.tail_order_tc = 0;
+	ctx->dense.tail_order_bits.clear();
 	ctx->dense.tail_dinv.release();
 	ctx->dense.tail_epoch = 0;
 	ctx->dense.epoch = 0;
@@ -421,6 +422,31 @@
 	}
 }
 
+static bool structure_of_pattern(int64_t nb, const int32_t *dim, const int64_t *col_ptr, const int64_t *row_idx, Structure &st)
+{
+	st.nb = nb;
+	st.nnzb = col_ptr[nb];
+	st.col_ptr.assign(col_ptr, col_ptr + nb + 1);
+	st.row_idx.assign(row_idx, row_idx + st.nnzb);
+	st.dim.assign(dim, dim + nb);
+	st.base.resize(nb + 1);
+	st.base[0] = 0;
+	for(int64_t j = 0; j < nb; ++ j)
+		st.base[j + 1] = st.base[j] + dim[j];
+	st.n = st.base[nb];
+	st.blk_off.resize(st.nnzb);
+	int64_t off = 0;
+	for(int64_t j = 0; j < nb; ++ j)
+		for(int64_t p = col_ptr[j]; p < col_ptr[j + 1]; ++ p) {
+			if(row_idx[p] < 0 || row_idx[p] > j)
+				return false;
+			st.blk_off[p] = off;
+			off += (int64_t)dim[row_idx[p]] * dim[j];
+		}
+	st.nvals = off;
+	return true;
+}
+
 int spp_schur_plan_host(int64_t nb, const int32_t *dim, const int64_t *col_ptr, const int64_t *row_idx, int shard_rank,
 	int shard_world, int sparse_S, int64_t *out, double *seconds)
 {
@@ -428,30 +454,35 @@
 		return SPP_E_BADARG;
 	try {
 		Structure st;
-		st.nb = nb;
-		st.nnzb = col_ptr[nb];
-		st.col_ptr.assign(col_ptr, col_ptr + nb + 1);
-		st.row_idx.assign(row_idx, row_idx + st.nnzb);
-		st.dim.assign(dim, dim + nb);
-		st.base.resize(nb + 1);
-		st.base[0] = 0;
-		for(int64_t j = 0; j < nb; ++ j)
-			st.base[j + 1] = st.base[j] + dim[j];
-		st.n = st.base[nb];
-		st.blk_off.resize(st.nnzb);
-		int64_t off = 0;
-		for(int64_t j = 0; j < nb; ++ j)
-			for(int64_t p = col_ptr[j]; p < col_ptr[j + 1]; ++ p) {
-				if(row_idx[p] < 0 || row_idx[p] > j)
-					return SPP_E_BADARG;
-				st.blk_off[p] = off;
-				off += (int64_t)dim[row_idx[p]] * dim[j];
-			}
-		st.nvals = off;
+		if(!structure_of_pattern(nb, dim, col_ptr, row_idx, st))
+			return SPP_E_BADARG;
 		const double sec = schur_plan_host_probe(st, shard_rank, shard_world, (sparse_S & 1) != 0, (sparse_S & 2) != 0, out);
 		if(seconds)
 			*seconds = sec;
 		return SPP_OK;
+	} catch(const Error &e) {
+		return e.code;
+	} catch(const std::bad_alloc &) {
+		return SPP_E_NOMEM;
+	} catch(...) {
+		return SPP_E_HIP;
+	}
+}
+
+int spp_schur_tile_mask_host(int64_t nb, const int32_t *dim, const int64_t *col_ptr, const int64_t *row_idx, int shard_rank,
+	int shard_world, uint64_t *words)
+{
+	if(nb <= 0 || !dim || !col_ptr || !row_idx || !words || shard_world < 1 || shard_rank < 0 || shard_rank >= shard_world)
+		return SPP_E_BADARG;
+	try {
+		Structure st;
+		if(!structure_of_pattern(nb, dim, col_ptr, row_idx, st))
+			return SPP_E_BADARG;
+		std::vector<uint64_t> w;
+		schur_tile_mask_host_probe(st, shard_rank, shard_world, w);
+		for(size_t q = 0; q < w.size(); ++ q)
+			words[q] = w[q];
+		return (int)w.size();
 	} catch(const Error &e) {
 		return e.code;
 	} catch(const std::bad_alloc &) {
@@ -921,10 +952,40 @@
 
 int spp_dense_posv(spp_ctx *ctx, double *d_A, int64_t n, int64_t ld, double *d_b)
 {
-	if(!ctx || !d_A || !d_b || n <= 0 || ld < n)
-		return SPP_E_BADARG;
-	SPP_TRY(ctx)
-	SPP_HIP_CHECK(hipSetDevice(ctx->device));
+	return spp_dense_posv_masked(ctx, d_A, n, ld, d_b, nullptr, 0);
+}
+
+int spp_tile_mask_host(int64_t n, int bs, int64_t nblk, const int32_t *i1, const int32_t *i2, int has_rhs, int fill,
+	uint64_t *words, int64_t *n_updates)
+{
+	if(n <= 0 || bs <= 0 || nblk < 0 || (nblk && (!i1 || !i2)) || !words)
+		return SPP_E_BADARG;
+	try {
+		std::vector<uint64_t> w;
+		tile_mask_mark(n, bs, nblk, i1, i2, w);
+		const int64_t upd = tile_mask_close(n, has_rhs != 0, fill != 0, w);
+		if(n_updates)
+			*n_updates = upd;
+		for(size_t q = 0; q < w.size(); ++ q)
+			words[q] = w[q];
+		return (int)w.size();
+	} catch(...) {
+		return SPP_E_NOMEM;
+	}
+}
+
+int spp_dense_posv_masked(spp_ctx *ctx, double *d_A, int64_t n, int64_t ld, double *d_b, const uint64_t *words, int64_t nwords)
+{
+	if(!ctx || !d_A || !d_b || n <= 0 || ld < n || nwords < 0 || (nwords && !words))
+		return SPP_E_BADARG;
+	SPP_TRY(ctx)
+	SPP_HIP_CHECK(hipSetDevice(ctx->device));
+	std::vector<uint64_t> mask(words, words + nwords);
+	if(nwords) {
+		SPP_REQUIRE(nwords == (n + DENSE_NB - 1) / DENSE_NB, SPP_E_BADARG, "posv: one mask word per tile row of 128");
+		tile_mask_close(n, true, true, mask);
+	}
+	TileMaskGuard guard(ctx->dense, &mask);
 	const int64_t ldp = ((n + 1 + DENSE_NB - 1) / DENSE_NB) * DENSE_NB;
 	DevBuf<double> tmp;
 	tmp.reserve((size_t)ldp * ldp);
diff --git a/slam_plus_plus_amd/csrc/spp_dense.hip b/slam_plus_plus_amd/csrc/spp_dense.hip
--- a/slam_plus_plus_amd/csrc/spp_dense.hip
+++ b/slam_plus_plus_amd/csrc/spp_dense.hip
@@ -1324,9 +1324,23 @@
 	if(!enabled || dw.tail_disabled || k + 1 >= nsteps || nsteps * NB < rows || (dw.ident_from >= 0 && dw.ident_from < rows))
 		return false;
 	const int Tr = (int)(nsteps - (k + 1)), Tc = (int)((ncols - c1 + NB - 1) / NB);
-	if(Tr < 1 || Tc < Tr || Tc > Tr + 1)
+	if(Tr < 1 || Tc < Tr || Tc > Tr + 1 || Tc > TAIL_MAX_ROWS)
 		return false;
-	const int ntile = Tr * Tc - Tr * (Tr - 1) / 2;
+	static int use_mask = -1;
+	if(use_mask < 0) {
+		const char *e = getenv("SPP_TAIL_MASK");
+		use_mask = e ? atoi(e) : 1;
+	}
+	const std::vector<uint64_t> *mask = (use_mask && dw.tile_mask && (int64_t)dw.tile_mask->size() == nsteps) ? dw.tile_mask : nullptr;
+	std::vector<uint64_t> bits((size_t)Tr + 1);
+	const uint64_t all_cols = Tc == 64 ? ~0ull : (1ull << Tc) - 1;
+	for(int i = -1; i < Tr; ++ i) {
+		const int64_t g = k + 1 + i;
+		uint64_t w = (mask && g >= 0) ? ((*mask)[(size_t)g] >> (k + 1)) : all_cols;
+		if(i >= 0)
+			w = (w | (1ull << i)) & ~((1ull << i) - 1);
+		bits[(size_t)i + 1] = w & all_cols;
+	}
 	static int max_rows = -1;
 	if(max_rows < 0) {
 		const char *e = getenv("SPP_TAIL_ROWS");
@@ -1350,7 +1364,9 @@
 		SPP_HIP_CHECK(hipMemsetAsync(dw.tail_pub.p, 0, dw.tail_pub.cap * sizeof(int), s));
 		dw.tail_epoch = 1;
 	}
-	if(dw.tail_order_tr != Tr || dw.tail_order_tc != Tc) {
+	if(dw.tail_order_tr != Tr || dw.tail_order_tc != Tc || dw.tail_order_bits != bits) {
+		if(!dw.tail_order_host.empty())
+			SPP_HIP_CHECK(hipStreamSynchronize(s));
 		static double beta = -1;
 		if(beta < 0) {
 			const char *e = getenv("SPP_TAIL_ORDER_BETA");
@@ -1359,7 +1375,8 @@
 		std::vector<std::pair<double, int> > key;
 		for(int i = 0; i < Tr; ++ i)
 			for(int j = i; j < Tc; ++ j)
-				key.push_back(std::make_pair((double)i + beta * (double)j, (i << 16) | j));
+				if((bits[(size_t)i + 1] >> j) & 1)
+					key.push_back(std::make_pair((double)i + beta * (double)j, (i << 16) | j));
 		std::stable_sort(key.begin(), key.end(), [](const std::pair<double, int> &x, const std::pair<double, int> &y) { return x.first < y.first; });
 		std::vector<int> &order = dw.tail_order_host;
 		order.resize(key.size());
@@ -1368,9 +1385,14 @@
 		dw.tail_order.upload(order, s);
 		dw.tail_order_tr = Tr;
 		dw.tail_order_tc = Tc;
-	}
+		dw.tail_order_bits = bits;
+	}
+	const int ntile = (int)dw.tail_order_host.size();
 	TailArgs a;
 	a.order = dw.tail_order.p;
+	memset(a.rowbits, 0, sizeof(a.rowbits));
+	for(size_t q = 0; q < bits.size(); ++ q)
+		a.rowbits[q] = bits[q];
 	a.A = d_A;
 	a.ld = ld;
 	a.rows = rows;
@@ -1417,7 +1439,7 @@
 		std::vector<long long> h((size_t)Tr * 8);
 		SPP_HIP_CHECK(hipStreamSynchronize(s));
 		SPP_HIP_CHECK(hipMemcpy(h.data(), trace.p, h.size() * sizeof(long long), hipMemcpyDeviceToHost));
-		fprintf(stderr, "[spp] streamed tail, %d tile rows (us from the launch's first stamp): diagonal tile: updates complete / factored+inverted | first panel tile: first row tile seen / last seen / last published\n", Tr);
+		fprintf(stderr, "[spp] streamed tail, %d tile rows, %d of %d tiles launched (us from the launch's first stamp): diagonal tile: updates complete / factored+inverted | first panel tile: first row tile seen / last seen / last published\n", Tr, ntile, Tr * Tc - Tr * (Tr - 1) / 2);
 		const long long t0 = h[0];
 		for(int i = 0; i < Tr; ++ i)
 			fprintf(stderr, "  row %2d  start %7.1f  updated %7.1f  done %7.1f | %7.1f %7.1f %7.1f\n", i, (h[8 * i] - t0) * 0.01, (h[8 * i + 1] - t0) * 0.01,
diff --git a/slam_plus_plus_amd/csrc/spp_dense_tail.h b/slam_plus_plus_amd/csrc/spp_dense_tail.h
--- a/slam_plus_plus_amd/csrc/spp_dense_tail.h
+++ b/slam_plus_plus_amd/csrc/spp_dense_tail.h
@@ -2,6 +2,8 @@
 #include "spp_dense_dev.h"
 
 namespace spp {
+
+constexpr int TAIL_MAX_ROWS = 64;
 
 struct TailArgs {
 	double *A;
@@ -20,6 +22,7 @@
 	long long timeout_ticks;
 	long long *trace;
 	const int *order;
+	unsigned long long rowbits[TAIL_MAX_ROWS + 1];
 };
 
 constexpr int TAIL_ABORT_TIMEOUT = 2;
@@ -139,10 +142,16 @@
 		const int ek = tid & 15, ec = tid >> 4;
 		constexpr int PS = 18;
 		const int ekp = 4 * (ek & 3) + (ek >> 2);
-		const int kfirst = a.have_pre ? -1 : 0, nst = 8 * (ti - kfirst);
+		const int kfirst = a.have_pre ? -1 : 0;
+		unsigned long long steps = 0;
+		for(int k = kfirst; k < ti; ++ k) {
+			const unsigned long long w = a.rowbits[k + 1];
+			if(((w >> ti) & (w >> tj) & 1) != 0)
+				steps |= 1ull << (k - kfirst);
+		}
+		const int nst = 8 * __builtin_popcountll(steps);
 		double va[2], vb[2];
-		auto fetch = [&](const int sidx) {
-			const int k = kfirst + (sidx >> 3), J = sidx & 7;
+		auto fetch = [&](const int k, const int J) {
 			const double *rowp = a.A + (a.c0 + (int64_t)NB * k) + 16 * J + ek;
 #pragma unroll
 			for(int h = 0; h < 2; ++ h) {
@@ -154,8 +163,13 @@
 		int avail = a.have_pre ? 8 : 0;
 		pre_first = diag && nst > 0 && (nst & 1) == 0 && a.rows - i0 >= 16;
 		bool inflight = false;
+		int k = kfirst;
 		for(int sidx = 0; sidx < nst; ++ sidx) {
-			const int k = kfirst + (sidx >> 3), J = sidx & 7;
+			const int J = sidx & 7;
+			if(J == 0) {
+				k = kfirst + __builtin_ctzll(steps);
+				steps &= steps - 1;
+			}
 			if(J == 0 && k >= 0)
 				avail = 0;
 			if(!inflight) {
@@ -164,7 +178,7 @@
 					if(avail < 0)
 						return;
 				}
-				fetch(sidx);
+				fetch(k, J);
 			}
 			int pk = -1;
 			if(tid == 0 && k >= 0 && J + 1 < 8 && J + 1 >= avail)
@@ -187,7 +201,7 @@
 			}
 			inflight = (sidx + 1 < nst) && (J + 1 < 8) && (J + 1 < avail);
 			if(inflight)
-				fetch(sidx + 1);
+				fetch(k, J + 1);
 			double fa[4];
 #pragma unroll
 			for(int u = 0; u < 4; ++ u) {
diff --git a/slam_plus_plus_amd/csrc/spp_internal.h b/slam_plus_plus_amd/csrc/spp_internal.h
--- a/slam_plus_plus_amd/csrc/spp_internal.h
+++ b/slam_plus_plus_amd/csrc/spp_internal.h
@@ -199,6 +199,7 @@
 	std::vector<int64_t> pose_block;
 	std::vector<int64_t> lm_block;
 	std::vector<uint8_t> is_lm;
+	std::vector<uint64_t> tile_mask;
 	DevBuf<int32_t> lm_ptr;
 	DevBuf<int32_t> bs_ptr;
 	int64_t n_bs = 0;
@@ -242,6 +243,8 @@
 	DevBuf<int> tail_order;
 	std::vector<int> tail_order_host;
 	int tail_order_tr = 0, tail_order_tc = 0;
+	std::vector<uint64_t> tail_order_bits;
+	const std::vector<uint64_t> *tile_mask = nullptr;
 	int tail_rows_last = 0;
 	bool tail_disabled = false;
 	DevBuf<double> trsv_m;
@@ -354,6 +357,14 @@
 
 void dense_chain_check(spp_ctx *ctx);
 void dense_set_padding(spp_ctx *ctx, double *d_A, int64_t ld, int64_t n);
+struct TileMaskGuard {
+	DenseWork &d;
+	TileMaskGuard(DenseWork &dw, const std::vector<uint64_t> *m) : d(dw) { d.tile_mask = (m && !m->empty()) ? m : nullptr; }
+	~TileMaskGuard() { d.tile_mask = nullptr; }
+};
+void tile_mask_mark(int64_t n, int bs, int64_t nblk, const int32_t *i1, const int32_t *i2, std::vector<uint64_t> &words);
+int64_t tile_mask_close(int64_t n, bool has_rhs, bool fill, std::vector<uint64_t> &words);
+void schur_tile_mask_host_probe(const Structure &st, int shard_rank, int shard_world, std::vector<uint64_t> &words);
 int dense_front_factor(spp_ctx *ctx, double *d_F, int64_t ld, int64_t w, int64_t h, double *d_image);
 bool dense_gemm_tn_sub(spp_ctx *ctx, int64_t m, int64_t n, int64_t k, const double *A, int64_t lda,
 	const double *B, int64_t ldb, double *C, int64_t ldc, bool upper_only);
diff --git a/slam_plus_plus_amd/csrc/spp_schur.hip b/slam_plus_plus_amd/csrc/spp_schur.hip
--- a/slam_plus_plus_amd/csrc/spp_schur.hip
+++ b/slam_plus_plus_amd/csrc/spp_schur.hip
@@ -860,7 +860,10 @@
 	} else {
 		phase_begin(ctx, SPP_PHASE_FACTOR);
 		dense_set_padding(ctx, S, ld, sp.n_red);
-		dense_potrf_upper_enqueue(ctx, S, sp.n_red, ld);
+		{
+			TileMaskGuard guard(ctx->dense, &sp.tile_mask);
+			dense_potrf_upper_enqueue(ctx, S, sp.n_red, ld);
+		}
 		phase_end(ctx, SPP_PHASE_FACTOR);
 		xcol = S + sp.n_red * ld;
 		phase_begin(ctx, SPP_PHASE_TRISOLVE);
diff --git a/slam_plus_plus_amd/csrc/spp_symbolic.cpp b/slam_plus_plus_amd/csrc/spp_symbolic.cpp
--- a/slam_plus_plus_amd/csrc/spp_symbolic.cpp
+++ b/slam_plus_plus_amd/csrc/spp_symbolic.cpp
@@ -22,7 +22,7 @@
 	sblk_voff.release(); s_st = Structure(); sparse_S = false; mis = false;
 	pair_a.release(); pair_b.release(); multi_blk.release(); multi_ptr.release(); cinv.release(); lfac.release();
 	W.release(); Up.release(); xw.release(); partial.release(); S.release();
-	pose_block.clear(); lm_block.clear(); is_lm.clear();
+	pose_block.clear(); lm_block.clear(); is_lm.clear(); tile_mask.clear();
 }
 
 bool schur_applicable(const Structure &st, int *dp_out, int *dl_out)
@@ -136,6 +136,88 @@
 	const T &operator[](size_t i) const { return p[i]; }
 };
 
+void tile_mask_mark(int64_t n, int bs, int64_t nblk, const int32_t *i1, const int32_t *i2, std::vector<uint64_t> &words)
+{
+	words.clear();
+	const int64_t Tr = (n + DENSE_NB - 1) / DENSE_NB, Tc = n / DENSE_NB + 1;
+	if(Tr < 1 || Tc > 64)
+		return;
+	words.assign((size_t)Tr, 0);
+	for(int64_t q = 0; q < nblk; ++ q) {
+		const int64_t a = std::min(i1[q], i2[q]), b = std::max(i1[q], i2[q]);
+		const int64_t r0 = a * bs / DENSE_NB, r1 = std::min<int64_t>(a * bs + bs - 1, n - 1) / DENSE_NB;
+		const int64_t c0 = b * bs / DENSE_NB, c1 = std::min<int64_t>(b * bs + bs - 1, n - 1) / DENSE_NB;
+		if(a < 0 || r0 >= Tr || c0 >= Tr)
+			continue;
+		words[r0] |= (1ull << c0) | (1ull << c1);
+		words[r1] |= (1ull << c0) | (1ull << c1);
+	}
+}
+
+int64_t tile_mask_close(int64_t n, bool has_rhs, bool fill, std::vector<uint64_t> &words)
+{
+	const int64_t Tr = (n + DENSE_NB - 1) / DENSE_NB, Tc = has_rhs ? n / DENSE_NB + 1 : Tr;
+	if(Tr < 1 || Tc > 64 || (int64_t)words.size() != Tr) {
+		words.clear();
+		return -1;
+	}
+	const uint64_t cols = Tc == 64 ? ~0ull : (1ull << Tc) - 1;
+	for(int64_t i = 0; i < Tr; ++ i) {
+		words[i] |= 1ull << i;
+		if(has_rhs)
+			words[i] |= 1ull << (n / DENSE_NB);
+		words[i] &= cols & ~((1ull << i) - 1);
+	}
+	int64_t updates = 0;
+	for(int64_t k = 0; k < Tr; ++ k) {
+		const uint64_t r = words[k] & ~((2ull << k) - 1);
+		for(uint64_t m = r; m; m &= m - 1) {
+			const int a = __builtin_ctzll(m);
+			if(a >= Tr)
+				break;
+			const uint64_t f = r & ~((1ull << a) - 1);
+			if(fill)
+				words[a] |= f;
+			updates += __builtin_popcountll(words[a] & f);
+		}
+	}
+	return updates;
+}
+
+static void schur_tile_mask(const Structure &st, const std::vector<uint8_t> &is_lm, const std::vector<int32_t> &pose_of,
+	int dp, int64_t n_red, std::vector<uint64_t> &words)
+{
+	tile_mask_mark(n_red, dp, 0, nullptr, nullptr, words);
+	if(words.empty())
+		return;
+	const int64_t Tr = (int64_t)words.size();
+	auto tiles_of = [&](int32_t pose) -> uint64_t {
+		return (1ull << ((int64_t)pose * dp / DENSE_NB)) | (1ull << (((int64_t)pose * dp + dp - 1) / DENSE_NB));
+	};
+	auto mark = [&](uint64_t rows, const uint64_t cols) {
+		for(; rows; rows &= rows - 1) {
+			const int a = __builtin_ctzll(rows);
+			if(a < Tr)
+				words[a] |= cols;
+		}
+	};
+	std::vector<uint64_t> seen(st.nb, 0);
+	for(int64_t j = 0; j < st.nb; ++ j)
+		for(int64_t p = st.col_ptr[j]; p < st.col_ptr[j + 1]; ++ p) {
+			const int64_t i = st.row_idx[p];
+			if(!is_lm[i] && !is_lm[j])
+				mark(tiles_of(pose_of[i]), tiles_of(pose_of[j]));
+			else if(!is_lm[i])
+				seen[j] |= tiles_of(pose_of[i]);
+			else if(!is_lm[j])
+				seen[i] |= tiles_of(pose_of[j]);
+		}
+	for(int64_t j = 0; j < st.nb; ++ j)
+		if(seen[j])
+			mark(seen[j], seen[j]);
+	tile_mask_close(n_red, true, true, words);
+}
+
 struct SchurPlanHost {
 	int dp = 0, dl = 0;
 	int64_t nc = 0, nl = 0, nl_total = 0, no = 0, n_red = 0, ld = 0, n_sblk = 0, n_pairs = 0, n_items = 0, n_multi = 0, n_ablk = 0;
@@ -151,6 +233,7 @@
 	std::vector<int64_t> sblk_aoff, sblk_voff, pose_rbase;
 	std::vector<SaccItem> recs;
 	Structure s_st;
+	std::vector<uint64_t> tile_mask;
 };
 
 static void schur_plan_host(const Structure &st, int shard_rank, int shard_world, bool sparse_S, bool mis, SchurPlanHost &h)
@@ -194,6 +277,8 @@
 	h.ld = ((h.n_red + 1 + DENSE_NB - 1) / DENSE_NB) * DENSE_NB;
 	SPP_REQUIRE(sparse_S || h.ld <= 65536, SPP_E_UNSUPPORTED,
 		"reduced camera system too large for the dense path (use SPP_MODE_SCHUR_SPARSE)");
+	if(!sparse_S)
+		schur_tile_mask(st, is_lm, pose_of, dp, h.n_red, h.tile_mask);
 
 	struct Obs { int32_t lm, pose; int64_t off; };
 	HVec<int64_t> &lm_coff = h.lm_coff;
@@ -742,6 +827,7 @@
 	sp.add_A = (ctx->shard_rank == 0);
 	sp.n_red = h.n_red;
 	sp.ld = h.ld;
+	sp.tile_mask.swap(h.tile_mask);
 	sp.no = no;
 	sp.n_pairs = h.n_pairs;
 	sp.n_sblk = h.n_sblk;
@@ -843,6 +929,13 @@
 	return sec;
 }
 
+void schur_tile_mask_host_probe(const Structure &st, int shard_rank, int shard_world, std::vector<uint64_t> &words)
+{
+	SchurPlanHost h;
+	schur_plan_host(st, shard_rank, shard_world, false, false, h);
+	words.swap(h.tile_mask);
+}
+
 void min_degree_order(int64_t nb, const int64_t *col_ptr, const int64_t *row_idx, std::vector<int64_t> &order)
 {
 	order.clear();
```

Measured after the change: 1.141 billion block-nnz/s, median of 6. 1.02x the previous value.
